# jingsenzhu/i2-sdf

Measured on AMD Instinct MI355X. Metric: ray-samples/sec (fwd+bwd), higher is better.
Workload: dtype f32 (bf16x3 split MFMA: fp32 operands as 3 bf16 terms, fp32 accumulate; the 256x256 weight-gradient GEMM blocks and the sampler's depth-choosing sdf-only passes: 2 bf16 terms per operand, 3 products, fp32 accumulate; the saved SDF tensors abar / G(hbar) / G(a) -- operands of those GEMMs and of the s

## Files before the change

### i2sdf_amd/csrc/pack.hip

```cpp
#include "plan.h"

using namespace i2sdf;

int i2sdf_hip_check(hipError_t e, const char* what);

namespace {

struct RowTab {
  int32_t n;
  int32_t rows[3 * I2SDF_MAX_LAYERS], cols[3 * I2SDF_MAX_LAYERS], scale_off[3 * I2SDF_MAX_LAYERS];
  int64_t off_v[3 * I2SDF_MAX_LAYERS], off_g[3 * I2SDF_MAX_LAYERS];
};

__global__ __launch_bounds__(256) void rowscale_kernel(RowTab tab, const float* __restrict__ params, float* __restrict__ scale,
                                                        int n_rows) {
  const int row = blockIdx.x * 4 + (threadIdx.x >> 6);
  const int lane = threadIdx.x & 63;
  if (row >= n_rows) return;
  int e = 0;
  while (e + 1 < tab.n && row >= tab.scale_off[e + 1]) ++e;
  const int r = row - tab.scale_off[e];
  const int cols = tab.cols[e];
  const float* v = params + tab.off_v[e] + (int64_t)r * cols;
  float s = 0.f;
  for (int c = lane; c < cols; c += 64) { float x = v[c]; s = fmaf(x, x, s); }
#pragma unroll
  for (int o = 32; o > 0; o >>= 1) s += __shfl_xor(s, o);
  if (lane == 0) scale[row] = params[tab.off_g[e] + r] / sqrtf(s);
}

__device__ __forceinline__ int map_col(const ColMap& cm, int kp) {
  if (kp < cm.split) return kp < cm.valid0 ? cm.base0 + kp : -1;
  const int j = kp - cm.split;
  return j < cm.valid1 ? cm.base1 + j : -1;
}

__global__ __launch_bounds__(256) void pack_kernel(const Seg* __restrict__ segs, int n_segs, const float* __restrict__ params,
                                                    const float* __restrict__ scale, float* __restrict__ chunks,
                                                    int64_t total_chunks) {
  const int64_t gid = (int64_t)blockIdx.x * 256 + threadIdx.x;
  const int64_t chunk = gid >> 6;
  const int lane = (int)(gid & 63);
  if (chunk >= total_chunks) return;
  int lo = 0, hi_ = n_segs - 1;
  while (lo < hi_) {
    const int mid = (lo + hi_ + 1) >> 1;
    if (segs[mid].chunk0 <= chunk) lo = mid; else hi_ = mid - 1;
  }
  const Seg s = segs[lo];
  const int c = (int)(chunk - s.chunk0);
  const int i32 = lane & 31, hi = lane >> 5;
  f32x4 out = {0.f, 0.f, 0.f, 0.f};
  if (c < s.used) {
    if (s.type == SEG_BIAS) {
      const int nt = c / 4, q = c % 4;
#pragma unroll
      for (int t = 0; t < 4; ++t) {
        const int r = 32 * nt + 8 * q + 4 * hi + t;
        out[t] = (r < s.nrows) ? params[s.off_bias + s.row_off + r] : 0.f;
      }
    } else if (s.type == SEG_WFWD) {
      const int nt = c / s.KC, kc = c % s.KC;
      const int r = 32 * nt + i32;
      if (r < s.nrows) {
        const int row = s.row_off + r;
        const float sc = scale[s.scale_off + row] * s.mult;
        const float* v = params + s.off_v + (int64_t)row * s.cols;
#pragma unroll
        for (int t = 0; t < 4; ++t) {
          const int col = map_col(s.cm, 8 * kc + 4 * hi + t);
          out[t] = col >= 0 ? v[col] * sc : 0.f;
        }
      }
    } else if (s.type == SEG_WFWD3) {
      const int G = s.NT / 2, w = c >> 1, e = c & 1;
      const int kc = w / (3 * G), g = (w / 3) % G, sp = w % 3;
      const int r = 32 * (2 * g + e) + i32;
      unsigned q[4] = {0u, 0u, 0u, 0u};
      if (r < s.nrows) {
        const int row = s.row_off + r;
        const float sc = scale[s.scale_off + row] * s.mult;
        const float* v = params + s.off_v + (int64_t)row * s.cols;
#pragma unroll
        for (int i = 0; i < 4; ++i) {
          float x[2];
#pragma unroll
          for (int h2 = 0; h2 < 2; ++h2) {
            const int j = 2 * i + h2;
            const int col = map_col(s.cm, 16 * kc + (j & 3) + 8 * (j >> 2) + 4 * hi);
            x[h2] = col >= 0 ? v[col] * sc : 0.f;
          }
          unsigned p0, p1, p2;
          split3_pair(x[0], x[1], p0, p1, p2);
          q[i] = sp == 0 ? p0 : (sp == 1 ? p1 : p2);
        }
      }
      out = __builtin_bit_cast(f32x4, u32x4{q[0], q[1], q[2], q[3]});
    } else if (s.type == SEG_WBWD3) {
      const int G = s.NT / 2, w = c >> 1, e = c & 1;
      const int kc = w / (3 * G), g = (w / 3) % G, sp = w % 3;
      const int col = map_col(s.cm, 32 * (2 * g + e) + i32);
      unsigned q[4] = {0u, 0u, 0u, 0u};
      if (col >= 0) {
#pragma unroll
        for (int i = 0; i < 4; ++i) {
          float x[2];
#pragma unroll
          for (int h2 = 0; h2 < 2; ++h2) {
            const int j = 2 * i + h2;
            const int r = 16 * kc + (j & 3) + 8 * (j >> 2) + 4 * hi;
            x[h2] = 0.f;
            if (r < s.nrows) {
              const int row = s.row_off + r;
              x[h2] = params[s.off_v + (int64_t)row * s.cols + col] * scale[s.scale_off + row] * s.mult;
            }
          }
          unsigned p0, p1, p2;
          split3_pair(x[0], x[1], p0, p1, p2);
          q[i] = sp == 0 ? p0 : (sp == 1 ? p1 : p2);
        }
      }
      out = __builtin_bit_cast(f32x4, u32x4{q[0], q[1], q[2], q[3]});
    } else if (s.type == SEG_BIAS_H) {
      const int kg = lane >> 4;
#pragma unroll
      for (int t = 0; t < 4; ++t) {
        const int r = 16 * c + 4 * kg + t;
        out[t] = (r < s.nrows) ? params[s.off_bias + s.row_off + r] : 0.f;
      }
    } else if (s.type == SEG_WFWD3H || s.type == SEG_WBWD3H || s.type == SEG_WFWD2H) {
      const int G = s.NT / 2, w = c >> 1, e = c & 1, PL = s.type == SEG_WFWD2H ? 2 : 3;
      const int kc = w / (PL * G), g = (w / PL) % G, sp = w % PL;
      const int i16 = lane & 15, kg = lane >> 4;
      const int arow = 16 * (2 * g + e) + i16;
      const bool fwd = s.type != SEG_WBWD3H;
      const int acol = fwd ? -1 : map_col(s.cm, arow);
      unsigned q[4] = {0u, 0u, 0u, 0u};
      if (fwd ? (arow < s.nrows) : (acol >= 0)) {
#pragma unroll
        for (int i = 0; i < 4; ++i) {
          float x[2];
#pragma unroll
          for (int h2 = 0; h2 < 2; ++h2) {
            const int j = 2 * i + h2;
            const int k = 32 * kc + 16 * (j >> 2) + 4 * kg + (j & 3);
            x[h2] = 0.f;
            if (fwd) {
              const int row = s.row_off + arow, col = map_col(s.cm, k);
              if (col >= 0) x[h2] = params[s.off_v + (int64_t)row * s.cols + col] * (scale[s.scale_off + row] * s.mult);
            } else if (k < s.nrows) {
              const int row = s.row_off + k;
              x[h2] = params[s.off_v + (int64_t)row * s.cols + acol] * scale[s.scale_off + row] * s.mult;
            }
          }
          unsigned p0, p1, p2;
          split3_pair(x[0], x[1], p0, p1, p2);
          q[i] = sp == 0 ? p0 : (sp == 1 ? p1 : p2);
        }
      }
      out = __builtin_bit_cast(f32x4, u32x4{q[0], q[1], q[2], q[3]});
    } else if (s.type == SEG_ROWVEC_H) {
      const int rr = c / s.KC, nt = c % s.KC, kg = lane >> 4;
      const int row = s.row_off + rr;
      const float sc = scale[s.scale_off + row] * s.mult;
#pragma unroll
      for (int t = 0; t < 4; ++t) {
        const int col = map_col(s.cm, 16 * nt + 4 * kg + t);
        out[t] = col >= 0 ? params[s.off_v + (int64_t)row * s.cols + col] * sc : 0.f;
      }
    } else if (s.type == SEG_WBWD) {
      const int kt = c / s.KC, nc = c % s.KC;
      const int col = map_col(s.cm, 32 * kt + i32);
      if (col >= 0) {
#pragma unroll
        for (int t = 0; t < 4; ++t) {
          const int r = 8 * nc + 4 * hi + t;
          if (r < s.nrows) {
            const int row = s.row_off + r;
            out[t] = params[s.off_v + (int64_t)row * s.cols + col] * scale[s.scale_off + row] * s.mult;
          }
        }
      }
    } else if (s.type == SEG_ROWVEC) {
      const int rr = c / s.KC, kc = c % s.KC;
      const int row = s.row_off + rr;
      const float sc = scale[s.scale_off + row] * s.mult;
#pragma unroll
      for (int t = 0; t < 4; ++t) {
        const int col = map_col(s.cm, 8 * kc + 4 * hi + t);
        out[t] = col >= 0 ? params[s.off_v + (int64_t)row * s.cols + col] * sc : 0.f;
      }
    } else if (s.type == SEG_SCALAR) {
#pragma unroll
      for (int t = 0; t < 4; ++t) out[t] = (t < s.nrows) ? params[s.off_bias + s.row_off + t] : 0.f;
    }
  }
  reinterpret_cast<f32x4*>(chunks)[chunk * 64 + lane] = out;
}

void fill_tab(RowTab& tab, const NetPlan& np) {
  for (int l = 0; l < np.d.n_lin; ++l) {
    const int e = tab.n++;
    tab.rows[e] = np.d.out_dim[l]; tab.cols[e] = np.d.in_dim[l]; tab.scale_off[e] = np.scale_off[l];
    tab.off_v[e] = np.d.off_v[l]; tab.off_g[e] = np.d.off_g[l];
  }
}

}

extern "C" int i2sdf_pack_weights(const i2sdf_plan* p, const float* params, float* packed, void* stream) {
  if (!p || !params || !packed) return I2SDF_EINVAL;
  if (!p->d_segs) return I2SDF_EHIP;
  hipStream_t st = (hipStream_t)stream;
  RowTab tab{};
  fill_tab(tab, p->sdf); fill_tab(tab, p->rgb);
  if (p->light.d.n_lin) fill_tab(tab, p->light);
  rowscale_kernel<<<cdiv(p->n_scale, 4), 256, 0, st>>>(tab, params, packed, p->n_scale);
  const int64_t threads = p->total_chunks * 64;
  pack_kernel<<<(unsigned)((threads + 255) / 256), 256, 0, st>>>(p->d_segs, p->n_segs, params, packed, packed + p->scale_floats,
                                                                 p->total_chunks);
  return i2sdf_hip_check(hipGetLastError(), "pack_weights launch");
}
```

### i2sdf_amd/csrc/plan.cpp

```cpp
#include <hip/hip_runtime.h>
#include <string.h>
#include <initializer_list>
#include <string>
#include "plan.h"
#include <stdlib.h>

using namespace i2sdf;

static thread_local std::string g_hip_err;

int i2sdf_hip_check(hipError_t e, const char* what) {
  if (e == hipSuccess) return I2SDF_OK;
  g_hip_err = std::string(what) + ": " + hipGetErrorString(e);
  return I2SDF_EHIP;
}

int i2sdf_refuse(const char* why) {
  g_hip_err = why;
  return I2SDF_EINVAL;
}

extern "C" int i2sdf_version(void) { return I2SDF_VERSION; }
extern "C" const char* i2sdf_last_hip_error(void) { return g_hip_err.c_str(); }
extern "C" const char* i2sdf_strerror(int code) {
  switch (code) {
    case I2SDF_OK: return "ok";
    case I2SDF_EINVAL: return "invalid argument or unsupported network shape";
    case I2SDF_EHIP: return "HIP runtime error";
    case I2SDF_ESPHERE: return "ray misses the scene bounding sphere";
    case I2SDF_EWORKSPACE: return "workspace too small";
    case I2SDF_ECOMM: return "RCCL error";
    default: return "unknown error";
  }
}

namespace {

constexpr int32_t HUGE_SPLIT = 1 << 30;
constexpr float RS2 = 0.70710678118654752440f;

struct Builder {
  std::vector<Seg>& segs;
  int64_t chunk;
  void add(Seg s) { s.chunk0 = chunk; chunk += s.nchunks; segs.push_back(s); }
  void pad_to_stage() {
    int64_t r = chunk % SC;
    if (r) { Seg z{}; z.type = SEG_ZERO; z.nchunks = (int32_t)(SC - r); add(z); }
  }
};

Seg base_seg(const NetPlan& np, int l, int type) {
  Seg s{};
  s.type = type;
  s.off_v = np.d.off_v[l]; s.off_bias = np.d.off_bias[l];
  s.scale_off = np.scale_off[l];
  s.rows = np.d.out_dim[l]; s.cols = np.d.in_dim[l];
  s.row_off = 0; s.nrows = s.rows;
  s.mult = 1.0f;
  s.cm = ColMap{HUGE_SPLIT, 0, s.cols, 0, 0};
  return s;
}

int pe_dim(const i2sdf_mlp_desc& d) { return side_dim(d); }
int pe_chunks(const i2sdf_mlp_desc& d) { return side_chunks(d); }

ColMap cols(int n) { return ColMap{HUGE_SPLIT, 0, n, 0, 0}; }

struct Family {
  int32_t bias_type, w_type, rowvec_type;
  int tile_rows;
  int k_width;
  int rv_width;
  int bias_chunks;
  int planes;
  bool fold_skip;
};
constexpr Family FP32{SEG_BIAS, SEG_WFWD, SEG_ROWVEC, 32, 8, 8, 4, 1, false};
constexpr Family X3{SEG_BIAS, SEG_WFWD3, SEG_ROWVEC, 32, 16, 8, 4, 3, true};
constexpr Family X3H{SEG_BIAS_H, SEG_WFWD3H, SEG_ROWVEC_H, 16, 32, 16, 1, 3, true};
constexpr Family X2H{SEG_BIAS_H, SEG_WFWD2H, SEG_ROWVEC_H, 16, 32, 16, 1, 2, true};

void emit_dense(Builder& b, const NetPlan& np, int l, const Family& f, int NT, int KC, ColMap cm, float mult, int row_off, int nrows) {
  Seg sb = base_seg(np, l, f.bias_type);
  sb.NT = NT; sb.KC = f.bias_chunks; sb.nchunks = sb.used = NT * f.bias_chunks; sb.row_off = row_off; sb.nrows = nrows;
  b.add(sb);
  Seg sw = base_seg(np, l, f.w_type);
  sw.NT = NT; sw.KC = KC; sw.used = NT * KC * f.planes; sw.cm = cm; sw.mult = mult; sw.row_off = row_off; sw.nrows = nrows;
  sw.nchunks = (f.w_type == SEG_WFWD ? op_chunks(NT, KC) : f.w_type == SEG_WFWD3 ? x3_op_chunks(NT, KC) : x3h_op_chunks(NT, KC, f.planes)) - sb.nchunks;
  b.add(sw);
}
void emit_dense_bwd(Builder& b, const NetPlan& np, int l, int type, int KT, int KC, ColMap cm, int row_off, int nrows, float mult = 1.0f) {
  Seg sw = base_seg(np, l, type);
  sw.NT = KT; sw.KC = KC; sw.used = KT * KC * (type == SEG_WBWD ? 1 : 3); sw.cm = cm; sw.mult = mult; sw.row_off = row_off; sw.nrows = nrows;
  sw.nchunks = type == SEG_WBWD ? bwd_op_chunks(KT, KC) : type == SEG_WBWD3 ? x3_bwd_chunks(KT, KC) : x3h_bwd_chunks(KT, KC);
  b.add(sw);
}
void emit_rowvec(Builder& b, const NetPlan& np, int l, const Family& f, int nrows) {
  const int KC = np.d.hidden / f.rv_width;
  Seg sw = base_seg(np, l, f.rowvec_type);
  sw.NT = nrows; sw.KC = KC; sw.used = nrows * KC; sw.nchunks = nrows * KC; sw.cm = cols(np.d.hidden); sw.nrows = nrows;
  b.add(sw);
  Seg sc = base_seg(np, l, SEG_SCALAR);
  sc.nchunks = (f.rowvec_type == SEG_ROWVEC ? rowvec_chunks(KC, nrows) : rowvec_h_chunks(KC, nrows)) - nrows * KC; sc.used = 1; sc.nrows = nrows;
  b.add(sc);
}
void emit_sdf_hidden(Builder& b, const NetPlan& np, const Family& f) {
  const i2sdf_mlp_desc& d = np.d;
  const int H = d.hidden, PED = pe_dim(d), PEK = cdiv(PED, f.k_width);
  for (int l = 0; l < d.n_lin - 1; ++l) {
    ColMap cm = cols(d.in_dim[l]);
    int KC = (l == 0) ? PEK : H / f.k_width;
    float mult = 1.0f;
    if (l == d.skip_layer) {
      cm = ColMap{H, 0, d.in_dim[l] - PED, d.in_dim[l] - PED, PED}; KC += PEK;
      if (f.fold_skip) mult = RS2;
    }
    emit_dense(b, np, l, f, H / f.tile_rows, KC, cm, mult, 0, d.out_dim[l]);
  }
}

int check_mlp(const i2sdf_mlp_desc& d) {
  if (d.n_lin < 2 || d.n_lin > I2SDF_MAX_LAYERS) return I2SDF_EINVAL;
  if (d.hidden % 32 || d.hidden < 32 || d.hidden > 256) return I2SDF_EINVAL;
  return I2SDF_OK;
}

void mark_here(NetPlan& np, const Builder& b, std::initializer_list<Mark> ms) {
  for (Mark k : ms) np.mark[k] = b.chunk;
}

int build_sdf(i2sdf_plan* p, Builder& b) {
  NetPlan& np = p->sdf;
  const i2sdf_mlp_desc& d = np.d;
  const int L = d.n_lin, H = d.hidden, PEC = pe_chunks(d), PED = pe_dim(d);
  const int F = d.d_out - 1;
  if (check_mlp(d)) return I2SDF_EINVAL;
  if (d.multires <= 0 || d.d_in != 3 || d.in0 != PED) return I2SDF_EINVAL;
  if (F < 0 || F % 32 || F > 256) return I2SDF_EINVAL;
  if (d.skip_layer == 0 || d.skip_layer >= L - 1) return I2SDF_EINVAL;
  for (int l = 0; l < L - 1; ++l) {
    const int want_out = (l + 1 == d.skip_layer) ? H - PED : H;
    const int want_in = (l == 0) ? PED : H;
    if (d.out_dim[l] != want_out || d.in_dim[l] != want_in) return I2SDF_EINVAL;
  }
  if (d.in_dim[L - 1] != H) return I2SDF_EINVAL;
  p->H = H; p->F = F;
  const bool even_tiles = (H / 32) % 2 == 0, wide = H == 256 && F == 256;
  const int PT = cdiv(PEC * 8, 32);
  mark_here(np, b, {FWD});
  emit_sdf_hidden(b, np, FP32);
  mark_here(np, b, {FWD_HIDDEN_END});
  emit_rowvec(b, np, L - 1, FP32, 1);
  mark_here(np, b, {FWD_SDF_END});
  if (F > 0) emit_dense(b, np, L - 1, FP32, F / 32, H / 8, cols(H), 1.0f, 1, F);
  mark_here(np, b, {FWD_END});
  mark_here(np, b, {REV});
  emit_rowvec(b, np, L - 1, FP32, 1);
  if (F > 0) emit_dense_bwd(b, np, L - 1, SEG_WBWD, H / 32, F / 8, cols(H), 1, F);
  mark_here(np, b, {REV_CHAIN});
  emit_rowvec(b, np, L - 1, FP32, 1);
  for (int l = L - 2; l >= 0; --l) {
    ColMap cm = cols(d.in_dim[l]);
    int KT = (l == 0) ? PT : H / 32;
    if (l == d.skip_layer) { cm = ColMap{H, 0, d.in_dim[l] - PED, d.in_dim[l] - PED, PED}; KT += PT; }
    if (l == 0) mark_here(np, b, {REV_W0});
    emit_dense_bwd(b, np, l, SEG_WBWD, KT, H / 8, cm, 0, d.out_dim[l]);
  }
  mark_here(np, b, {REV_END});
  mark_here(np, b, {FWD3, FWD3_HIDDEN_END, FWD3_END});
  if (even_tiles) {
    emit_sdf_hidden(b, np, X3);
    mark_here(np, b, {FWD3_HIDDEN_END});
    emit_rowvec(b, np, L - 1, X3, 1);
    mark_here(np, b, {FWD3_END});
  }
  mark_here(np, b, {REV3, REV3_CHAIN, REV3_W0, REV3_END});
  if (even_tiles) {
    emit_rowvec(b, np, L - 1, X3, 1);
    if (F > 0 && F % 16 == 0) emit_dense_bwd(b, np, L - 1, SEG_WBWD3, H / 32, F / 16, cols(H), 1, F);
    mark_here(np, b, {REV3_CHAIN});
    emit_rowvec(b, np, L - 1, X3, 1);
    for (int l = L - 2; l >= 0; --l) {
      if (l == 0) mark_here(np, b, {REV3_W0});
      if (l == d.skip_layer) {
        emit_dense_bwd(b, np, l, SEG_WBWD3, H / 32, H / 16, cols(d.in_dim[l] - PED), 0, d.out_dim[l], RS2);
        emit_dense_bwd(b, np, l, SEG_WBWD3, PT, H / 16, ColMap{HUGE_SPLIT, d.in_dim[l] - PED, PED, 0, 0}, 0, d.out_dim[l], RS2);
      } else {
        emit_dense_bwd(b, np, l, SEG_WBWD3, (l == 0) ? PT : H / 32, H / 16, cols(d.in_dim[l]), 0, d.out_dim[l]);
      }
    }
    mark_here(np, b, {REV3_END});
  }
  mark_here(np, b, {FWD3H, FWD3H_SDF_END, FWD3H_END});
  if (wide) {
    emit_sdf_hidden(b, np, X3H);
    emit_rowvec(b, np, L - 1, X3H, 1);
    mark_here(np, b, {FWD3H_SDF_END});
    emit_dense(b, np, L - 1, X3H, F / 16, H / 32, cols(H), 1.0f, 1, F);
    mark_here(np, b, {FWD3H_END});
  }
  mark_here(np, b, {FWD2H, FWD2H_END});
  if (wide) {
    emit_sdf_hidden(b, np, X2H);
    emit_rowvec(b, np, L - 1, X2H, 1);
    mark_here(np, b, {FWD2H_END});
  }
  return I2SDF_OK;
}

int build_rgb(i2sdf_plan* p, Builder& b) {
  NetPlan& np = p->rgb;
  const i2sdf_mlp_desc& d = np.d;
  const bool idr = rgb_idr(d);
  const int L = d.n_lin, H = d.hidden, PED = pe_dim(d), PEC = pe_chunks(d), F = p->F;
  if (check_mlp(d)) return I2SDF_EINVAL;
  if ((rgb_mode(d) != I2SDF_RGB_MODE_NERF && !idr) || (idr && d.d_in != 9)) return I2SDF_EINVAL;
  if (rgb_act(d) > I2SDF_RGB_ACT_SOFTPLUS || (d.reserved & 0xf0ff0000) || rgb_embed(d) > I2SDF_RGB_EMBED_FOURIER) return I2SDF_EINVAL;
  const ColMap rev0 = idr ? ColMap{F, PED, F, PED - 3, 3} : ColMap{HUGE_SPLIT, PED, F, 0, 0};
  if (d.skip_layer >= 0 || d.d_out != 3 || (d.multires <= 0 && !idr) || d.in0 != PED + F || F <= 0) return I2SDF_EINVAL;
  for (int l = 0; l < L - 1; ++l)
    if (d.out_dim[l] != H || d.in_dim[l] != (l == 0 ? PED + F : H)) return I2SDF_EINVAL;
  const bool wide = H == 256 && F == 256 && L >= 3;
  mark_here(np, b, {FWD});
  emit_dense(b, np, 0, FP32, H / 32, PEC + F / 8, ColMap{PEC * 8, 0, PED, PED, F}, 1.0f, 0, H);
  for (int l = 1; l < L - 1; ++l) emit_dense(b, np, l, FP32, H / 32, H / 8, cols(H), 1.0f, 0, H);
  emit_rowvec(b, np, L - 1, FP32, 3);
  mark_here(np, b, {FWD_END, REV});
  emit_rowvec(b, np, L - 1, FP32, 3);
  for (int l = L - 2; l >= 1; --l) emit_dense_bwd(b, np, l, SEG_WBWD, H / 32, H / 8, cols(H), 0, H);
  emit_dense_bwd(b, np, 0, SEG_WBWD, F / 32 + (idr ? 1 : 0), H / 8, rev0, 0, H);
  mark_here(np, b, {REV_END});
  mark_here(np, b, {FWD3H, FWD3H_END, REV3H, REV3H_END});
  if (wide) {
    const int PV32 = cdiv(PEC * 8, 32);
    emit_dense(b, np, 0, X3H, H / 16, PV32 + F / 32, ColMap{PV32 * 32, 0, PED, PED, F}, 1.0f, 0, H);
    for (int l = 1; l < L - 1; ++l) emit_dense(b, np, l, X3H, H / 16, H / 32, cols(H), 1.0f, 0, H);
    emit_rowvec(b, np, L - 1, X3H, 3);
    mark_here(np, b, {FWD3H_END, REV3H});
    emit_rowvec(b, np, L - 1, X3H, 3);
    for (int l = L - 2; l >= 1; --l) emit_dense_bwd(b, np, l, SEG_WBWD3H, H / 16, H / 32, cols(H), 0, H);
    emit_dense_bwd(b, np, 0, SEG_WBWD3H, F / 16 + (idr ? 2 : 0), H / 32, rev0, 0, H);
    mark_here(np, b, {REV3H_END});
  }
  return I2SDF_OK;
}

int build_light(i2sdf_plan* p, Builder& b) {
  NetPlan& np = p->light;
  const i2sdf_mlp_desc& d = np.d;
  if (d.n_lin == 0) return I2SDF_OK;
  const int H = d.hidden, F = p->F;
  if (d.n_lin != 2 || H % 32 || H > 256 || d.d_out != 1 || d.in0 != F || d.multires != 0) return I2SDF_EINVAL;
  if (d.out_dim[0] != H || d.in_dim[0] != F || d.in_dim[1] != H) return I2SDF_EINVAL;
  mark_here(np, b, {FWD});
  emit_dense(b, np, 0, FP32, H / 32, F / 8, cols(F), 1.0f, 0, H);
  emit_rowvec(b, np, 1, FP32, 1);
  mark_here(np, b, {FWD_END, REV});
  emit_rowvec(b, np, 1, FP32, 1);
  mark_here(np, b, {REV_END});
  mark_here(np, b, {FWD3H, FWD3H_END});
  if (H == 128 && F == 256) {
    emit_dense(b, np, 0, X3H, H / 16, F / 32, cols(F), 1.0f, 0, H);
    emit_rowvec(b, np, 1, X3H, 1);
    mark_here(np, b, {FWD3H_END});
  }
  return I2SDF_OK;
}

void assign_scales_and_wgrad(i2sdf_plan* p, NetPlan& np, int kind) {
  const i2sdf_mlp_desc& d = np.d;
  const int side = pe_dim(d), PEC8 = pe_chunks(d) * 8;
  for (int l = 0; l < d.n_lin; ++l) {
    np.scale_off[l] = p->n_scale;
    p->n_scale += d.out_dim[l];
    const bool last = (l == d.n_lin - 1);
    int rowsP = d.hidden, colsP = d.hidden;
    if (kind == 0) {
      if (l == 0) colsP = PEC8;
      else if (l == d.skip_layer) colsP = d.hidden + PEC8;
      if (last) rowsP = 32 + (d.d_out - 1);
    } else if (kind == 1) {
      if (l == 0) colsP = PEC8 + (d.in0 - side);
      if (last) rowsP = 32;
    } else {
      if (l == 0) colsP = d.in0;
      if (last) rowsP = 32;
    }
    np.wg_rows[l] = rowsP; np.wg_cols[l] = colsP;
    np.wgrad_off[l] = p->wgrad_floats;
    p->wgrad_floats += (int64_t)rowsP * colsP + rowsP;
  }
}

}

extern "C" int i2sdf_plan_create(const i2sdf_net_desc* desc, i2sdf_plan** out) {
  if (!desc || !out) return I2SDF_EINVAL;
  {
    if (rgb_act(desc->rgb) > I2SDF_RGB_ACT_SOFTPLUS || (desc->rgb.reserved & 0x00ff0000)) {
      g_hip_err = "i2sdf_plan_create: rgb.reserved " + std::to_string(desc->rgb.reserved) + ": output activation " + std::to_string(rgb_act(desc->rgb)) +
                  " of the radiance net is not one of I2SDF_RGB_ACT_SIGMOID (0), I2SDF_RGB_ACT_RELU (1), I2SDF_RGB_ACT_SOFTPLUS (2) in bits 8..15"
                  " (bits 16..23 must be zero)";
      return I2SDF_EINVAL;
    }
    const int emb = rgb_embed(desc->rgb), n_emb = desc->rgb.multires;
    if (emb > I2SDF_RGB_EMBED_FOURIER || (desc->rgb.reserved & 0xf0000000)) {
      g_hip_err = "i2sdf_plan_create: rgb.reserved " + std::to_string(desc->rgb.reserved) + ": view embedder " + std::to_string(emb) +
                  " of the radiance net is not one of I2SDF_RGB_EMBED_POSITIONAL (0), I2SDF_RGB_EMBED_SH (1), I2SDF_RGB_EMBED_FOURIER (2) in bits 24..27"
                  " (bits 28..31 must be zero)";
      return I2SDF_EINVAL;
    }
    if (emb == I2SDF_RGB_EMBED_SH && (n_emb < 1 || n_emb > 5)) {
      g_hip_err = "i2sdf_plan_create: spherical-harmonics view embedder of degree " + std::to_string(n_emb) +
                  " (rgb.multires): the reference's SHEncoder and the kernels have degrees 1..5";
      return I2SDF_EINVAL;
    }
    if (emb == I2SDF_RGB_EMBED_FOURIER && (n_emb < 1 || n_emb > I2SDF_RGB_EMBED_MAX_CHANNELS)) {
      g_hip_err = "i2sdf_plan_create: Fourier view embedder with " + std::to_string(n_emb) + " channels (rgb.multires): 1..12 fit the 27 view "
                  "columns of the radiance net's side row (width 2 c + 3); more need wider rows";
      return I2SDF_EINVAL;
    }
    const int H = desc->sdf.hidden, Hr = desc->rgb.hidden;
    int F = 0;
    if (desc->rgb.n_lin > 0) {
      if (emb != I2SDF_RGB_EMBED_POSITIONAL) {
        F = desc->sdf.d_out - 1;
        if (desc->rgb.in0 != side_dim(desc->rgb) + F) {
          g_hip_err = "i2sdf_plan_create: rgb.in0 " + std::to_string(desc->rgb.in0) + " disagrees with the view embedder: " +
                      (emb == I2SDF_RGB_EMBED_SH ? "spherical harmonics of degree " : "Fourier features with channels ") + std::to_string(n_emb) +
                      " are " + std::to_string(embed_dim(desc->rgb)) + " wide, the side row " + std::to_string(side_dim(desc->rgb)) +
                      ", so lin0 has " + std::to_string(side_dim(desc->rgb) + F) + " columns with feature size " + std::to_string(F);
          return I2SDF_EINVAL;
        }
      } else {
        F = desc->rgb.in0 - (rgb_idr(desc->rgb) ? side_dim(desc->rgb) : (desc->rgb.multires > 0 ? 3 + 6 * desc->rgb.multires : 3));
      }
    }
    const bool ok = (H == 256 && Hr == 256 && F == 256) || (H == 64 && Hr == 64 && F == 64);
    if (!ok || desc->sdf.multires != 6 || (emb == I2SDF_RGB_EMBED_POSITIONAL && desc->rgb.multires != 4 && desc->rgb.multires != 0)) {
      g_hip_err = "i2sdf_plan_create: SDF width " + std::to_string(H) + " / radiance width " + std::to_string(Hr) + " / feature size " + std::to_string(F) +
                  " / multires " + std::to_string(desc->sdf.multires) + "," + std::to_string(desc->rgb.multires) +
                  ": the MLP kernels are instantiated for 256/256/256 and 64/64/64 with multires 6 (points) and 4 (view directions) only";
      return I2SDF_EINVAL;
    }
    if (rgb_idr(desc->rgb) && desc->rgb.d_in != 9) {
      g_hip_err = "i2sdf_plan_create: the radiance net's 'idr' mode needs d_in 9 (points, view directions, normals)";
      return I2SDF_EINVAL;
    }
  }
  i2sdf_plan* p = new i2sdf_plan();
  p->desc = *desc;
  p->sdf.d = desc->sdf; p->rgb.d = desc->rgb; p->light.d = desc->light;
  assign_scales_and_wgrad(p, p->sdf, 0);
  assign_scales_and_wgrad(p, p->rgb, 1);
  if (desc->light.n_lin) assign_scales_and_wgrad(p, p->light, 2);
  p->scale_floats = round_up(p->n_scale, CHUNK_FLOATS);
  Builder b{p->segs, 0};
  int rc = build_sdf(p, b);
  if (!rc) rc = build_rgb(p, b);
  if (!rc) rc = build_light(p, b);
  if (rc) { delete p; return rc; }
  { Seg z{}; z.type = SEG_ZERO; z.nchunks = SC > SCH ? SC : SCH; b.add(z); }
  p->total_chunks = b.chunk;
  p->n_segs = (int32_t)p->segs.size();
  hipError_t e = hipMalloc((void**)&p->d_segs, sizeof(Seg) * p->segs.size());
  if (e == hipSuccess) e = hipMemcpy(p->d_segs, p->segs.data(), sizeof(Seg) * p->segs.size(), hipMemcpyHostToDevice);
  if (e != hipSuccess) {
    (void)i2sdf_hip_check(e, "plan table upload");
    if (p->d_segs) (void)hipFree(p->d_segs);
    p->d_segs = nullptr;
    (void)hipGetLastError();
  }
  {
    int dev = 0, n = 0;
    if (hipGetDevice(&dev) == hipSuccess && hipDeviceGetAttribute(&n, hipDeviceAttributeMultiprocessorCount, dev) == hipSuccess && n > 0) p->n_cu = n;
    else (void)hipGetLastError();
  }
  if (p->H == 256 && p->F == 256)
    for (int32_t opt : {I2SDF_OPT_SDF_FWD_BF16X3, I2SDF_OPT_WGRAD_BF16X3, I2SDF_OPT_TRAIN_FWD_BF16X3, I2SDF_OPT_SDF_BWD_BF16X3, I2SDF_OPT_RGB_BF16X3,
                        I2SDF_OPT_BLOCKED_SAVES, I2SDF_OPT_TAIL_OVERLAP})
      (void)i2sdf_plan_set_option(p, opt, 1);
  *out = p;
  return I2SDF_OK;
}

extern "C" void i2sdf_plan_destroy(i2sdf_plan* p) {
  if (!p) return;
  if (p->d_segs) (void)hipFree(p->d_segs);
  if (p->ev_fork) (void)hipEventDestroy(p->ev_fork);
  if (p->ev_join) (void)hipEventDestroy(p->ev_join);
  if (p->side) (void)hipStreamDestroy(p->side);
  for (hipEvent_t e : p->part_ev) if (e) (void)hipEventDestroy(e);
  for (hipStream_t s : p->part_st) if (s) (void)hipStreamDestroy(s);
  delete p;
}

hipStream_t i2sdf_tail_fork(const i2sdf_plan* p, hipStream_t st) {
  if (!p->tail_overlap) return st;
  if (!p->side) {
    if (hipStreamCreateWithFlags(&p->side, hipStreamNonBlocking) != hipSuccess) { p->side = nullptr; (void)hipGetLastError(); return st; }
    if (hipEventCreateWithFlags(&p->ev_fork, hipEventDisableTiming) != hipSuccess ||
        hipEventCreateWithFlags(&p->ev_join, hipEventDisableTiming) != hipSuccess) {
      (void)hipGetLastError();
      (void)hipStreamDestroy(p->side); p->side = nullptr;
      return st;
    }
  }
  if (hipEventRecord(p->ev_fork, st) != hipSuccess || hipStreamWaitEvent(p->side, p->ev_fork, 0) != hipSuccess) {
    (void)hipGetLastError();
    return st;
  }
  return p->side;
}

void i2sdf_tail_join(const i2sdf_plan* p, hipStream_t st, hipStream_t side) {
  if (side == st) return;
  (void)hipEventRecord(p->ev_join, side);
  (void)hipStreamWaitEvent(st, p->ev_join, 0);
}

namespace {
constexpr int64_t PART_ALIGN = I2SDF_WG_CH;

bool parts_resources(const i2sdf_plan* p) {
  for (int q = 0; q < I2SDF_MAX_PARTS; ++q)
    if (!p->part_ev[q] && hipEventCreateWithFlags(&p->part_ev[q], hipEventDisableTiming) != hipSuccess) { (void)hipGetLastError(); return false; }
  for (int q = 0; q + 1 < p->parts; ++q)
    if (!p->part_st[q] && hipStreamCreateWithFlags(&p->part_st[q], hipStreamNonBlocking) != hipSuccess) { (void)hipGetLastError(); return false; }
  return true;
}
void part_bounds(int64_t M, int n, int64_t (&b)[I2SDF_MAX_PARTS + 1]) {
  static double w[I2SDF_MAX_PARTS] = {0, 0, 0, 0};
  static int nw = -1;
  if (nw < 0) {
    nw = 0;
    if (const char* e = getenv("I2SDF_PART_WEIGHTS")) {
      while (*e && nw < I2SDF_MAX_PARTS) {
        char* end = nullptr;
        const double v = strtod(e, &end);
        if (end == e) break;
        w[nw++] = v > 0 ? v : 0;
        e = (*end == ',') ? end + 1 : end;
      }
    }
  }
  const int64_t nch = (M + PART_ALIGN - 1) / PART_ALIGN;
  double tot = 0, acc = 0;
  for (int q = 0; q < n; ++q) tot += (nw == n) ? w[q] : 1.0;
  b[0] = 0;
  for (int q = 1; q <= n; ++q) {
    acc += (nw == n) ? w[q - 1] : 1.0;
    int64_t c = tot > 0 ? (int64_t)(nch * (acc / tot) + 0.5) : nch * q / n;
    if (c < b[q - 1] / PART_ALIGN) c = b[q - 1] / PART_ALIGN;
    b[q] = (c > nch ? nch : c) * PART_ALIGN;
  }
  b[n] = nch * PART_ALIGN;
}
}

void i2sdf_parts_fence(const i2sdf_plan* p, hipStream_t st) {
  (void)hipEventRecord(p->part_ev[0], st);
  for (int q = 0; q + 1 < p->parts; ++q) (void)hipStreamWaitEvent(p->part_st[q], p->part_ev[0], 0);
}
void i2sdf_parts_join_all(const i2sdf_plan* p, hipStream_t st) {
  for (int q = 0; q + 1 < p->parts; ++q) {
    if (!p->part_st[q] || !p->part_ev[q + 1]) continue;
    (void)hipEventRecord(p->part_ev[q + 1], p->part_st[q]);
    (void)hipStreamWaitEvent(st, p->part_ev[q + 1], 0);
  }
}
bool i2sdf_parts_begin(const i2sdf_plan* p, hipStream_t st, int64_t M, PartRun* pr) {
  pr->n = 1; pr->st[0] = st; pr->lo[0] = 0; pr->hi[0] = M; pr->own = false;
  if (!i2sdf_parts_on(p) || M <= 0) return false;
  const bool chain = p->chain_active != 0;
  const int64_t Mref = chain ? (p->chain_M > M ? p->chain_M : M) : M;
  if ((Mref + PART_ALIGN - 1) / PART_ALIGN < p->parts) return false;
  if (!parts_resources(p)) return false;
  int64_t b[I2SDF_MAX_PARTS + 1];
  part_bounds(Mref, p->parts, b);
  pr->n = p->parts;
  for (int q = 0; q < pr->n; ++q) {
    pr->st[q] = q == 0 ? st : p->part_st[q - 1];
    pr->lo[q] = b[q] < M ? b[q] : M;
    pr->hi[q] = b[q + 1] < M ? b[q + 1] : M;
  }
  if (!chain) { i2sdf_parts_fence(p, st); pr->own = true; }
  return true;
}
void i2sdf_parts_end(const i2sdf_plan* p, hipStream_t st, PartRun* pr) {
  if (pr->own) i2sdf_parts_join_all(p, st);
  pr->own = false;
}

extern "C" int i2sdf_chain_begin(const i2sdf_plan* p, int64_t M, void* stream) {
  if (!p || M < 0) return I2SDF_EINVAL;
  if (!i2sdf_parts_on(p) || M == 0) return I2SDF_OK;
  if (p->chain_active) return I2SDF_EINVAL;
  if (!parts_resources(p)) return i2sdf_hip_check(hipErrorOutOfMemory, "chain_begin: streams / events");
  i2sdf_parts_fence(p, (hipStream_t)stream);
  p->chain_active = 1;
  p->chain_M = M;
  return i2sdf_hip_check(hipGetLastError(), "chain_begin");
}
extern "C" int i2sdf_chain_fence(const i2sdf_plan* p, void* stream) {
  if (!p) return I2SDF_EINVAL;
  if (!p->chain_active) return I2SDF_OK;
  i2sdf_parts_fence(p, (hipStream_t)stream);
  return i2sdf_hip_check(hipGetLastError(), "chain_fence");
}
extern "C" int i2sdf_chain_end(const i2sdf_plan* p, void* stream) {
  if (!p) return I2SDF_EINVAL;
  if (!p->chain_active) return I2SDF_OK;
  i2sdf_parts_join_all(p, (hipStream_t)stream);
  p->chain_active = 0;
  p->chain_M = 0;
  return i2sdf_hip_check(hipGetLastError(), "chain_end");
}

extern "C" int i2sdf_plan_set_option(i2sdf_plan* p, int32_t option, int32_t value) {
  if (!p) return I2SDF_EINVAL;
  if (option == I2SDF_OPT_PARTS) {
    if (value < 0 || value > I2SDF_MAX_PARTS || p->chain_active) return I2SDF_EINVAL;
    p->parts = value >= 2 ? value : 0;
    return I2SDF_OK;
  }
  if (option == I2SDF_OPT_SDF_FWD_BF16X3) {
    const bool runs = (p->H == 256 && p->F == 256 && span_chunks(p->sdf, SPAN_FWD3H) > 0) || (p->H == 64 && p->F == 64 && span_chunks(p->sdf, SPAN_FWD3) > 0);
    if (value && !runs) return I2SDF_EINVAL;
    p->sdf_fwd_bf16x3 = value ? 1 : 0;
    return I2SDF_OK;
  }
  if (option == I2SDF_OPT_SAMPLER_BF16X2) {
    if (value && (span_chunks(p->sdf, SPAN_FWD2H) == 0 || p->H != 256 || p->F != 256)) return I2SDF_EINVAL;
    p->sampler_bf16x2 = value ? 1 : 0;
    return I2SDF_OK;
  }
  if (option == I2SDF_OPT_TRAIN_FWD_BF16X3) {
    if (value && (span_chunks(p->sdf, SPAN_REV3_CHAIN) == 0 || span_chunks(p->sdf, SPAN_FWD3H) == 0 || p->H != 256 || p->F != 256)) return I2SDF_EINVAL;
    p->train_fwd_bf16x3 = value ? 1 : 0;
    return I2SDF_OK;
  }
  if (option == I2SDF_OPT_SDF_BWD_BF16X3) {
    if (value && (span_chunks(p->sdf, SPAN_REV3_CHAIN) == 0 || p->H != 256 || p->F != 256)) return I2SDF_EINVAL;
    p->sdf_bwd_bf16x3 = value ? 1 : 0;
    return I2SDF_OK;
  }
  if (option == I2SDF_OPT_RGB_BF16X3) {
    if (value && (span_chunks(p->rgb, SPAN_REV3H) == 0 || p->rgb.d.hidden != 256 || p->F != 256 || p->rgb.d.n_lin < 3)) return I2SDF_EINVAL;
    p->rgb_bf16x3 = value ? 1 : 0;
    return I2SDF_OK;
  }
  if (option == I2SDF_OPT_WGRAD_BF16X3) {
    p->wgrad_bf16x3 = value ? 1 : 0;
    return I2SDF_OK;
  }
  if (option == I2SDF_OPT_WGRAD_BF16X2) {
    p->wgrad_bf16x2 = value ? 1 : 0;
    return I2SDF_OK;
  }
  if (option == I2SDF_OPT_BLOCKED_SAVES) {
    p->blocked_saves = value ? 1 : 0;
    return I2SDF_OK;
  }
  if (option == I2SDF_OPT_SAVES24) {
    if (value && (p->H != 256 || p->F != 256 || span_chunks(p->sdf, SPAN_REV3_CHAIN) == 0)) return I2SDF_EINVAL;
    if (p->chain_active) return I2SDF_EINVAL;
    p->saves24 = value ? 1 : 0;
    return I2SDF_OK;
  }
  if (option == I2SDF_OPT_TAIL_OVERLAP) {
    p->tail_overlap = value ? 1 : 0;
    return I2SDF_OK;
  }
  return I2SDF_EINVAL;
}

extern "C" int i2sdf_plan_set_view_embed(i2sdf_plan* p, const float* B_host, int32_t rows, int32_t cols) {
  if (!p) return I2SDF_EINVAL;
  const auto refuse = [](const std::string& why) { g_hip_err = "i2sdf_plan_set_view_embed: " + why; return I2SDF_EINVAL; };
  if (rgb_embed(p->rgb.d) != I2SDF_RGB_EMBED_FOURIER) return refuse("the plan's radiance net has no Fourier view embedder (rgb.reserved bits 24..27)");
  if (!B_host) return refuse("B_host is NULL");
  if (rows != 3 || cols != p->rgb.d.multires)
    return refuse("B is (" + std::to_string(rows) + ", " + std::to_string(cols) + "), the plan's embedder takes (3, " + std::to_string(p->rgb.d.multires) + ")");
  for (int i = 0; i < 3 * cols; ++i)
    if (!(B_host[i] - B_host[i] == 0.0f)) return refuse("B[" + std::to_string(i / cols) + "][" + std::to_string(i % cols) + "] is not finite");
  for (int r = 0; r < 3; ++r)
    for (int c = 0; c < I2SDF_RGB_EMBED_MAX_CHANNELS; ++c) p->view_B[r * I2SDF_RGB_EMBED_MAX_CHANNELS + c] = c < cols ? B_host[r * cols + c] : 0.0f;
  p->view_B_set = 1;
  return I2SDF_OK;
}

extern "C" int i2sdf_plan_set_exchange(i2sdf_plan* p, const i2sdf_exchange* ex, int32_t flags) {
  if (!p || (flags & ~I2SDF_DP_GLOBAL_SAMPLER) || (ex && !ex->allreduce)) return I2SDF_EINVAL;
  p->exchange = ex ? *ex : i2sdf_exchange{nullptr, nullptr};
  p->dp_flags = ex ? flags : 0;
  return I2SDF_OK;
}

extern "C" int64_t i2sdf_plan_pack_floats(const i2sdf_plan* p) {
  return p ? p->scale_floats + p->total_chunks * CHUNK_FLOATS : 0;
}
extern "C" int64_t i2sdf_plan_wgrad_floats(const i2sdf_plan* p) { return p ? p->wgrad_floats : 0; }
```

### i2sdf_amd/csrc/plan.h

```cpp
#pragma once
#include <stdint.h>
#include <vector>
#include "../../include/i2sdf.h"
#include "x3h.h"

namespace i2sdf {

enum SegType : int32_t { SEG_ZERO = 0, SEG_BIAS = 1, SEG_WFWD = 2, SEG_WBWD = 3, SEG_ROWVEC = 4, SEG_SCALAR = 5,
                         SEG_WFWD3 = 6 ,
                         SEG_WBWD3 = 7 ,
                         SEG_BIAS_H = 8, SEG_WFWD3H = 9, SEG_WBWD3H = 10, SEG_ROWVEC_H = 11,
                         SEG_WFWD2H = 12  };

struct ColMap { int32_t split, base0, valid0, base1, valid1; };

struct Seg {
  int64_t chunk0;
  int32_t nchunks;
  int32_t type;
  int64_t off_v, off_bias;
  int32_t scale_off;
  int32_t rows, cols;
  int32_t row_off;
  int32_t nrows;
  int32_t NT, KC;
  int32_t used;
  ColMap cm;
  float mult;
};

enum Mark : int {
  FWD, FWD_HIDDEN_END, FWD_SDF_END, FWD_END,
  REV, REV_CHAIN, REV_W0, REV_END,
  FWD3, FWD3_HIDDEN_END, FWD3_END,
  REV3, REV3_CHAIN, REV3_W0, REV3_END,
  FWD3H, FWD3H_SDF_END, FWD3H_END,
  REV3H, REV3H_END,
  FWD2H, FWD2H_END,
  N_MARKS
};
struct SpanId { Mark from, to; int stage_chunks; };
constexpr SpanId SPAN_FWD_HIDDEN{FWD, FWD_HIDDEN_END, SC};
constexpr SpanId SPAN_FWD_SDF{FWD, FWD_SDF_END, SC};
constexpr SpanId SPAN_FWD{FWD, FWD_END, SC};
constexpr SpanId SPAN_REV_SWEEP2{REV, REV_W0, SC};
constexpr SpanId SPAN_REV_CHAIN{REV_CHAIN, REV_END, SC};
constexpr SpanId SPAN_REV{REV, REV_END, SC};
constexpr SpanId SPAN_FWD3_HIDDEN{FWD3, FWD3_HIDDEN_END, SC};
constexpr SpanId SPAN_FWD3{FWD3, FWD3_END, SC};
constexpr SpanId SPAN_REV3_SWEEP2{REV3, REV3_W0, SC};
constexpr SpanId SPAN_REV3_CHAIN{REV3_CHAIN, REV3_END, SC};
constexpr SpanId SPAN_FWD3H_SDF{FWD3H, FWD3H_SDF_END, SCH};
constexpr SpanId SPAN_FWD3H{FWD3H, FWD3H_END, SCH};
constexpr SpanId SPAN_REV3H{REV3H, REV3H_END, SCH};
constexpr SpanId SPAN_FWD2H{FWD2H, FWD2H_END, SCH};

inline int rgb_mode(const i2sdf_mlp_desc& d) { return d.reserved & 0xff; }
inline int rgb_act(const i2sdf_mlp_desc& d) { return (d.reserved >> 8) & 0xff; }
inline int rgb_embed(const i2sdf_mlp_desc& d) { return (d.reserved >> 24) & 0xf; }
inline bool rgb_idr(const i2sdf_mlp_desc& d) { return rgb_mode(d) == I2SDF_RGB_MODE_IDR; }
inline int embed_dim(const i2sdf_mlp_desc& d) { return rgb_embed(d) == I2SDF_RGB_EMBED_SH ? d.multires * d.multires : 2 * d.multires + 3; }
inline int side_dim(const i2sdf_mlp_desc& d) {
  if (rgb_embed(d) != I2SDF_RGB_EMBED_POSITIONAL) return embed_dim(d) + (rgb_idr(d) ? 6 : 0);
  const int raw = rgb_idr(d) ? 3 : d.d_in;
  return (d.multires > 0 ? raw + 2 * raw * d.multires : raw) + (rgb_idr(d) ? 6 : 0);
}
inline int side_chunks(const i2sdf_mlp_desc& d) {
  if (rgb_embed(d) != I2SDF_RGB_EMBED_POSITIONAL) return rgb_idr(d) ? 5 : 4;
  return (side_dim(d) + 7) / 8;
}

struct NetPlan {
  i2sdf_mlp_desc d;
  int32_t scale_off[I2SDF_MAX_LAYERS];
  int64_t mark[N_MARKS] = {};
  int64_t wgrad_off[I2SDF_MAX_LAYERS];
  int32_t wg_rows[I2SDF_MAX_LAYERS], wg_cols[I2SDF_MAX_LAYERS];
};

}

struct i2sdf_plan {
  i2sdf_net_desc desc;
  i2sdf::NetPlan sdf, rgb, light;
  std::vector<i2sdf::Seg> segs;
  i2sdf::Seg* d_segs = nullptr;
  int32_t n_segs = 0;
  int32_t n_scale = 0;
  int64_t scale_floats = 0;
  int64_t total_chunks = 0;
  int64_t wgrad_floats = 0;
  int32_t H = 0, F = 0;
  int32_t n_cu = 256;
  int32_t rgb_bf16x3 = 0;
  int32_t sdf_bwd_bf16x3 = 0;
  int32_t train_fwd_bf16x3 = 0;
  int32_t wgrad_bf16x3 = 0;
  int32_t sdf_fwd_bf16x3 = 0;
  int32_t sampler_bf16x2 = 0;
  i2sdf_exchange exchange{nullptr, nullptr};
  int32_t dp_flags = 0;
  int32_t wgrad_bf16x2 = 0;
  int32_t blocked_saves = 0;
  int32_t saves24 = 0;
  int32_t tail_overlap = 0;
  mutable hipStream_t side = nullptr;
  mutable hipEvent_t ev_fork = nullptr, ev_join = nullptr;
  int32_t parts = 0;
  mutable hipStream_t part_st[I2SDF_MAX_PARTS - 1] = {nullptr, nullptr, nullptr};
  mutable hipEvent_t part_ev[I2SDF_MAX_PARTS] = {nullptr, nullptr, nullptr, nullptr};
  mutable int32_t chain_active = 0;
  float view_B[3 * I2SDF_RGB_EMBED_MAX_CHANNELS] = {};
  int32_t view_B_set = 0;
  mutable int64_t chain_M = 0;
};

int i2sdf_refuse(const char* why);
int i2sdf_hip_check(hipError_t e, const char* what);

namespace i2sdf {
struct Span { const float* w = nullptr; int n_stages = 0; };
inline int64_t span_chunks(const NetPlan& np, SpanId id) { return np.mark[id.to] - np.mark[id.from]; }
inline Span span(const i2sdf_plan* p, const float* packed, const NetPlan& np, SpanId id) {
  const int64_t n = span_chunks(np, id);
  if (n <= 0 || n % id.stage_chunks) return Span{};
  return Span{packed + p->scale_floats + np.mark[id.from] * CHUNK_FLOATS, (int)(n / id.stage_chunks)};
}
}

struct PartRun {
  int n = 1;
  hipStream_t st[I2SDF_MAX_PARTS];
  int64_t lo[I2SDF_MAX_PARTS], hi[I2SDF_MAX_PARTS];
  bool own = false;
};
bool i2sdf_parts_begin(const i2sdf_plan* p, hipStream_t st, int64_t M, PartRun* pr);
void i2sdf_parts_end(const i2sdf_plan* p, hipStream_t st, PartRun* pr);
void i2sdf_parts_join_all(const i2sdf_plan* p, hipStream_t st);
void i2sdf_parts_fence(const i2sdf_plan* p, hipStream_t st);
#ifndef I2SDF_WG_CH
#define I2SDF_WG_CH 2048
#endif
inline bool i2sdf_parts_on(const i2sdf_plan* p) { return p->parts >= 2; }
struct ChainGuard {
  const i2sdf_plan* p; hipStream_t st; bool on;
  ChainGuard(const i2sdf_plan* p_, hipStream_t st_, bool ranged) : p(p_), st(st_), on(!ranged && p_->chain_active != 0) {
    if (on) i2sdf_parts_join_all(p, st);
  }
  ~ChainGuard() { if (on) i2sdf_parts_fence(p, st); }
};

hipStream_t i2sdf_tail_fork(const i2sdf_plan* p, hipStream_t st);
void i2sdf_tail_join(const i2sdf_plan* p, hipStream_t st, hipStream_t side);

inline int64_t split_bulk_points(int64_t M, int n_cu) {
  const int64_t n_wg = (M + i2sdf::PTS_PER_WG - 1) / i2sdf::PTS_PER_WG;
  const int64_t full = (n_wg / n_cu) * n_cu, rem = n_wg - full;
  if (full == 0 || rem == 0 || rem * 4 > n_cu) return 0;
  if ((full * i2sdf::PTS_PER_WG) % I2SDF_WG_CH != 0) return 0;
  return full * i2sdf::PTS_PER_WG;
}

enum TailOrder { TAIL_FORKED, TAIL_BEHIND };
template <class Full, class Tail>
inline void i2sdf_dispatch_points(const i2sdf_plan* p, hipStream_t st, int64_t M, bool ranged, bool may_split, TailOrder order, Full full, Tail tail) {
  constexpr int64_t WG = i2sdf::PTS_PER_WG;
  if (ranged) {
    PartRun pr;
    i2sdf_parts_begin(p, st, M, &pr);
    for (int q = 0; q < pr.n; ++q)
      if (pr.hi[q] > pr.lo[q]) full(pr.st[q], (int)(pr.lo[q] / WG), (unsigned)((pr.hi[q] - pr.lo[q] + WG - 1) / WG), M);
    i2sdf_parts_end(p, st, &pr);
    return;
  }
  const int64_t bulk = may_split ? split_bulk_points(M, p->n_cu) : 0;
  if (bulk == 0) {
    full(st, 0, (unsigned)((M + WG - 1) / WG), M);
  } else if (order == TAIL_FORKED) {
    hipStream_t ts = i2sdf_tail_fork(p, st);
    tail(ts, bulk);
    full(st, 0, (unsigned)(bulk / WG), bulk);
    i2sdf_tail_join(p, st, ts);
  } else {
    full(st, 0, (unsigned)(bulk / WG), bulk);
    tail(st, bulk);
  }
}
```

### i2sdf_amd/csrc/sampler.hip

```cpp
#include "mlp_args.h"

using namespace i2sdf;

namespace {

constexpr int NMAX = 640;
constexpr int NNEW = 128;
constexpr int EMAX = NMAX / 64;

enum { ST_DONE = 0, ST_ITERS = 1, ST_FLAG0 = 2 , ST_CNT0 = 16 , ST_WORDS = 32 };

#ifndef SAMPLER_DPP
#define SAMPLER_DPP 1
#endif
template <int CTRL, int ROW_MASK>
__device__ __forceinline__ float dpp_mov(float old, float v) {
  return __builtin_bit_cast(float, __builtin_amdgcn_update_dpp(__builtin_bit_cast(int, old), __builtin_bit_cast(int, v), CTRL, ROW_MASK, 0xf, false));
}
constexpr int DPP_ROW_SHR1 = 0x111, DPP_ROW_SHR2 = 0x112, DPP_ROW_SHR4 = 0x114, DPP_ROW_SHR8 = 0x118, DPP_ROW_BCAST15 = 0x142, DPP_ROW_BCAST31 = 0x143;
__device__ __forceinline__ float wscan_incl(float v, int lane) {
#if SAMPLER_DPP
  (void)lane;
  v += dpp_mov<DPP_ROW_SHR1, 0xf>(0.f, v);
  v += dpp_mov<DPP_ROW_SHR2, 0xf>(0.f, v);
  v += dpp_mov<DPP_ROW_SHR4, 0xf>(0.f, v);
  v += dpp_mov<DPP_ROW_SHR8, 0xf>(0.f, v);
  v += dpp_mov<DPP_ROW_BCAST15, 0xa>(0.f, v);
  v += dpp_mov<DPP_ROW_BCAST31, 0xc>(0.f, v);
  return v;
#else
#pragma unroll
  for (int o = 1; o < 64; o <<= 1) {
    const float t = __shfl_up(v, o);
    if (lane >= o) v += t;
  }
  return v;
#endif
}
__device__ __forceinline__ float wsum(float v) {
#if SAMPLER_DPP
  return __builtin_bit_cast(float, __builtin_amdgcn_readlane(__builtin_bit_cast(int, wscan_incl(v, 0)), 63));
#else
#pragma unroll
  for (int o = 32; o > 0; o >>= 1) v += __shfl_xor(v, o);
  return v;
#endif
}
__device__ __forceinline__ float wmax(float v) {
#if SAMPLER_DPP
  const float lo = -3.4028234663852886e38f;
  v = fmaxf(v, dpp_mov<DPP_ROW_SHR1, 0xf>(lo, v));
  v = fmaxf(v, dpp_mov<DPP_ROW_SHR2, 0xf>(lo, v));
  v = fmaxf(v, dpp_mov<DPP_ROW_SHR4, 0xf>(lo, v));
  v = fmaxf(v, dpp_mov<DPP_ROW_SHR8, 0xf>(lo, v));
  v = fmaxf(v, dpp_mov<DPP_ROW_BCAST15, 0xa>(lo, v));
  v = fmaxf(v, dpp_mov<DPP_ROW_BCAST31, 0xc>(lo, v));
  return __builtin_bit_cast(float, __builtin_amdgcn_readlane(__builtin_bit_cast(int, v), 63));
#else
#pragma unroll
  for (int o = 32; o > 0; o >>= 1) v = fmaxf(v, __shfl_xor(v, o));
  return v;
#endif
}
template <int E>
__device__ __forceinline__ void row_scan_incl(float (&v)[E], int lane) {
#pragma unroll
  for (int e = 1; e < E; ++e) v[e] += v[e - 1];
  const float tot = v[E - 1];
  const float pre = wscan_incl(tot, lane) - tot;
#pragma unroll
  for (int e = 0; e < E; ++e) v[e] += pre;
}

__device__ __forceinline__ float laplace_density(float s, float inv_beta) {
  const float e = expm1f(-fabsf(s) * inv_beta);
  const float sg = (s > 0.f) ? 1.f : ((s < 0.f) ? -1.f : 0.f);
  return inv_beta * (0.5f + 0.5f * sg * e);
}

template <int E>
struct Row {
  float z[E], s[E];
  float a[E], ds[E];
  int n;
};

template <int E>
__device__ __forceinline__ void row_intervals(Row<E>& r, int lane) {
  const float zn_next = __shfl_down(r.z[0], 1), sn_next = __shfl_down(r.s[0], 1);
#pragma unroll
  for (int e = 0; e < E; ++e) {
    const int j = lane * E + e;
    const float z1 = (e + 1 < E) ? r.z[(e + 1 < E) ? e + 1 : e] : zn_next;
    const float s1 = (e + 1 < E) ? r.s[(e + 1 < E) ? e + 1 : e] : sn_next;
    float a = 0.f, d = 0.f;
    if (j < r.n - 1) {
      a = z1 - r.z[e];
      const float b = fabsf(r.s[e]), c = fabsf(s1);
      const bool first = a * a + b * b <= c * c;
      const bool second = a * a + c * c <= b * b;
      const float sp = (a + b + c) / 2.0f;
      const float area = sp * (sp - a) * (sp - b) * (sp - c);
      const bool mask = !first && !second && (b + c - a > 0.f);
      float h = (2.0f * sqrtf(area)) / a;
      if (!(h == h)) h = 0.f;
      else if (h > 3.4028234663852886e38f) h = 3.4028234663852886e38f;
      else if (h < -3.4028234663852886e38f) h = -3.4028234663852886e38f;
      d = ((first && !second) ? b : 0.f) + (second ? c : 0.f) + (mask ? h : 0.f);
      const float sg0 = (r.s[e] > 0.f) ? 1.f : ((r.s[e] < 0.f) ? -1.f : 0.f);
      const float sg1 = (s1 > 0.f) ? 1.f : ((s1 < 0.f) ? -1.f : 0.f);
      if (!(sg0 * sg1 == 1.f)) d = 0.f;
    }
    r.a[e] = a; r.ds[e] = d;
  }
}

template <int E>
__device__ __forceinline__ float row_error_bound(const Row<E>& r, float beta, int lane) {
  const float ib = 1.0f / beta;
  float fe[E], er[E];
#pragma unroll
  for (int e = 0; e < E; ++e) {
    const int j = lane * E + e;
    const bool ok = j < r.n - 1;
    fe[e] = ok ? r.a[e] * laplace_density(r.s[e], ib) : 0.f;
    er[e] = ok ? expf(-r.ds[e] / beta) * (r.a[e] * r.a[e]) / (4.0f * beta * beta) : 0.f;
  }
  float fi[E], ei[E];
#pragma unroll
  for (int e = 0; e < E; ++e) { fi[e] = fe[e]; ei[e] = er[e]; }
  row_scan_incl<E>(fi, lane);
  row_scan_incl<E>(ei, lane);
  float mx = -3.4e38f;
#pragma unroll
  for (int e = 0; e < E; ++e) {
    const int j = lane * E + e;
    if (j < r.n - 1) {
      const float integ = fi[e] - fe[e];
      const float bo = (fminf(expf(ei[e]), 1.0e6f) - 1.0f) * expf(-integ);
      mx = fmaxf(mx, bo);
    }
  }
  return wmax(mx);
}

struct SamplerArgs {
  int64_t B;
  int it, n, n_new;
  int N_eval, N_final, max_iters, beta_iters, force_iters;
  float eps, add_tiny, near, far;
  const float* beta_param; float beta_min;
  int* state;
  float* z_cur; float* z_nxt;
  float* sdf_prev; float* sdf_cur;
  const int* idx;
  int* idx_nxt;
  const float* sdf_new;
  float* samples;
  float* beta;
  const float* u_more; const float* u_final; int64_t ldu_final;
};

template <int E>
__device__ __forceinline__ void load_row(Row<E>& r, const float* z, const float* s, int n, int lane) {
  r.n = n;
#pragma unroll
  for (int e = 0; e < E; ++e) {
    const int j = lane * E + e;
    r.z[e] = (j < n) ? z[j] : 3.0e38f;
    r.s[e] = (j < n) ? s[j] : 0.f;
  }
}

template <int E>
__device__ __forceinline__ float beta_step(const SamplerArgs& a, Row<E>& r, int64_t rc, bool active, int lane) {
  const float beta0 = fabsf(a.beta_param[0]) + a.beta_min;
  const int n = a.n;
  float* sc = a.sdf_cur + rc * NMAX;
  const float* zc = a.z_cur + rc * NMAX;
  r.n = n;
  {
    const int n_old = n - a.n_new;
    const int* ix = a.idx + rc * NMAX;
    const float* sp = a.sdf_prev + rc * NMAX;
    const float* sn = a.sdf_new + rc * a.n_new;
#pragma unroll
    for (int e = 0; e < E; ++e) {
      const int j = lane * E + e;
      float sv = 0.f, zv = 3.0e38f;
      if (j < n) {
        zv = zc[j];
        if (a.it == 0) sv = sn[j];
        else { const int k = ix[j]; sv = (k < n_old) ? sp[k] : sn[k - n_old]; }
        if (active) sc[j] = sv;
      }
      r.z[e] = zv; r.s[e] = sv;
    }
  }
  row_intervals<E>(r, lane);
  float beta = a.beta[rc];
  const float err0 = row_error_bound<E>(r, beta0, lane);
  if (err0 <= a.eps) beta = beta0;
  float bmin = beta0, bmax = beta;
  for (int k = 0; k < a.beta_iters; ++k) {
    const float bmid = (bmin + bmax) / 2.0f;
    const float err = row_error_bound<E>(r, bmid, lane);
    if (err <= a.eps) bmax = bmid; else bmin = bmid;
  }
  return bmax;
}
template <int E>
__global__ __launch_bounds__(256) void sampler_beta_kernel(SamplerArgs a) {
  if (a.state[ST_DONE]) return;
  const int lane = threadIdx.x & 63;
  const int64_t ray = (int64_t)blockIdx.x * 4 + (threadIdx.x >> 6);
  if (ray >= a.B) return;
  Row<E> r;
  const float beta = beta_step<E>(a, r, ray, true, lane);
  if (lane == 0) {
    a.beta[ray] = beta;
    if (beta > fabsf(a.beta_param[0]) + a.beta_min) atomicOr(&a.state[ST_FLAG0 + a.it], 1);
  }
}

template <int E>
__device__ __forceinline__ void resample_step(const SamplerArgs& a, const Row<E>& r, float beta, bool more, int64_t ray, int64_t rc, bool active,
                                              float (&s_cdf)[4][NMAX + 1], float (&s_z)[4][NMAX], float (&s_new)[4][NNEW], int lane, int wv) {
  const int n = a.n;
  const float ib = 1.0f / beta;
  float fe[E], cum[E];
#pragma unroll
  for (int e = 0; e < E; ++e) {
    const int j = lane * E + e;
    const float dist = (j < n - 1) ? r.a[e] : 1.0e10f;
    fe[e] = (j < n) ? dist * laplace_density(r.s[e], ib) : 0.f;
    cum[e] = (j < n - 1) ? fe[e] : 0.f;
  }
  row_scan_incl<E>(cum, lane);
  float pdf[E];
  if (more) {
    float er[E];
#pragma unroll
    for (int e = 0; e < E; ++e) {
      const int j = lane * E + e;
      er[e] = (j < n - 1) ? expf(-r.ds[e] / beta) * (r.a[e] * r.a[e]) / (4.0f * beta * beta) : 0.f;
    }
    row_scan_incl<E>(er, lane);
#pragma unroll
    for (int e = 0; e < E; ++e) {
      const int j = lane * E + e;
      const float T = expf(-(cum[e] - ((j < n - 1) ? fe[e] : 0.f)));
      pdf[e] = (j < n - 1) ? (fminf(expf(er[e]), 1.0e6f) - 1.0f) * T + a.add_tiny : 0.f;
    }
  } else {
#pragma unroll
    for (int e = 0; e < E; ++e) {
      const int j = lane * E + e;
      const float T = expf(-(cum[e] - ((j < n - 1) ? fe[e] : 0.f)));
      const float w = (1.0f - expf(-fe[e])) * T;
      pdf[e] = (j < n - 1) ? w + 1e-5f : 0.f;
    }
  }
  float tot = 0.f;
#pragma unroll
  for (int e = 0; e < E; ++e) tot += pdf[e];
  tot = wsum(tot);
  float cd[E];
#pragma unroll
  for (int e = 0; e < E; ++e) { pdf[e] = pdf[e] / tot; cd[e] = pdf[e]; }
  row_scan_incl<E>(cd, lane);
#pragma unroll
  for (int e = 0; e < E; ++e) {
    const int j = lane * E + e;
    if (j < n) { s_cdf[wv][j] = cd[e] - pdf[e]; s_z[wv][j] = r.z[e]; }
  }
  __syncthreads();
  const int N = more ? a.N_eval : a.N_final;
  for (int k = lane; k < N; k += 64) {
    float u;
    if (more) u = a.u_more[k];
    else u = a.u_final[rc * a.ldu_final + k];
    int lo = 0, hi = n;
    while (lo < hi) {
      const int mid = (lo + hi) >> 1;
      if (s_cdf[wv][mid] <= u) lo = mid + 1; else hi = mid;
    }
    const int below = (lo - 1 > 0) ? lo - 1 : 0;
    const int above = (lo < n - 1) ? lo : n - 1;
    const float c0 = s_cdf[wv][below], c1 = s_cdf[wv][above];
    const float b0 = s_z[wv][below], b1 = s_z[wv][above];
    float denom = c1 - c0;
    if (denom < 1e-5f) denom = 1.0f;
    const float t = (u - c0) / denom;
    const float smp = b0 + t * (b1 - b0);
    s_new[wv][k] = smp;
    if (active) a.samples[ray * NNEW + k] = smp;
  }
  __syncthreads();
  if (!more) return;
  if (active) {
    float* zn = a.z_nxt + ray * NMAX;
    int* ixn = a.idx_nxt + ray * NMAX;
    for (int j = lane; j < n; j += 64) {
      const float v = s_z[wv][j];
      int lo = 0, hi = N;
      while (lo < hi) { const int mid = (lo + hi) >> 1; if (s_new[wv][mid] < v) lo = mid + 1; else hi = mid; }
      zn[j + lo] = v; ixn[j + lo] = j;
    }
    for (int k = lane; k < N; k += 64) {
      const float v = s_new[wv][k];
      int lo = 0, hi = n;
      while (lo < hi) { const int mid = (lo + hi) >> 1; if (s_z[wv][mid] <= v) lo = mid + 1; else hi = mid; }
      zn[k + lo] = v; ixn[k + lo] = n + k;
    }
  }
}

__device__ __forceinline__ void iteration_done(const SamplerArgs& a, bool more) {
  __syncthreads();
  if (threadIdx.x == 0) {
    __threadfence();
    const int c = atomicAdd(&a.state[ST_CNT0 + a.it], 1);
    if (c == (int)gridDim.x - 1 && !more) { a.state[ST_ITERS] = a.it + 1; __threadfence(); a.state[ST_DONE] = 1; }
  }
}

template <int E>
__global__ __launch_bounds__(256) void sampler_resample_kernel(SamplerArgs a) {
  __shared__ float s_cdf[4][NMAX + 1];
  __shared__ float s_z[4][NMAX];
  __shared__ float s_new[4][NNEW];
  if (a.state[ST_DONE]) return;
  const int lane = threadIdx.x & 63, wv = threadIdx.x >> 6;
  const int64_t ray = (int64_t)blockIdx.x * 4 + wv;
  const bool active = ray < a.B;
  const int64_t rc = active ? ray : a.B - 1;
  bool not_conv = a.state[ST_FLAG0 + a.it] != 0;
  if (a.force_iters > 0) not_conv = (a.it + 1) < a.force_iters;
  const bool more = not_conv && (a.it + 1 < a.max_iters);
  Row<E> r;
  load_row<E>(r, a.z_cur + rc * NMAX, a.sdf_cur + rc * NMAX, a.n, lane);
  row_intervals<E>(r, lane);
  resample_step<E>(a, r, a.beta[rc], more, ray, rc, active, s_cdf, s_z, s_new, lane, wv);
  iteration_done(a, more);
}

template <int E>
__global__ __launch_bounds__(256) void sampler_iter_fixed_kernel(SamplerArgs a) {
  __shared__ float s_cdf[4][NMAX + 1];
  __shared__ float s_z[4][NMAX];
  __shared__ float s_new[4][NNEW];
  const int lane = threadIdx.x & 63, wv = threadIdx.x >> 6;
  const int64_t ray = (int64_t)blockIdx.x * 4 + wv;
  const bool active = ray < a.B;
  const int64_t rc = active ? ray : a.B - 1;
  const bool more = ((a.it + 1) < a.force_iters) && (a.it + 1 < a.max_iters);
  Row<E> r;
  const float beta = beta_step<E>(a, r, rc, active, lane);
  if (active && lane == 0) a.beta[ray] = beta;
  resample_step<E>(a, r, beta, more, ray, rc, active, s_cdf, s_z, s_new, lane, wv);
  iteration_done(a, more);
}

__global__ __launch_bounds__(256) void sampler_init_kernel(int64_t B, int N, const float* __restrict__ t_lin, const float* __restrict__ strat_u,
                                                            float near, float far, float eps, float* __restrict__ z_cur,
                                                            float* __restrict__ samples, float* __restrict__ beta, int* __restrict__ state) {
  const int lane = threadIdx.x & 63;
  const int64_t ray = (int64_t)blockIdx.x * 4 + (threadIdx.x >> 6);
  if (blockIdx.x == 0 && threadIdx.x < ST_WORDS) state[threadIdx.x] = 0;
  if (ray >= B) return;
  float acc = 0.f, carry = 0.f;
  for (int base = 0; base < N; base += 64) {
    const int j = base + lane;
    float z = 0.f;
    if (j < N) {
      const float t = t_lin[j];
      z = near * (1.0f - t) + far * t;
      if (strat_u) {
        const float tm = t_lin[j > 0 ? j - 1 : 0], tp = t_lin[j < N - 1 ? j + 1 : N - 1];
        const float zm = near * (1.0f - tm) + far * tm, zq = near * (1.0f - tp) + far * tp;
        const float lower = (j > 0) ? 0.5f * (z + zm) : z;
        const float upper = (j < N - 1) ? 0.5f * (zq + z) : z;
        z = lower + (upper - lower) * strat_u[ray * N + j];
      }
      z_cur[ray * NMAX + j] = z;
      samples[ray * NNEW + j] = z;
    }
    float zp = __shfl_up(z, 1);
    if (lane == 0) zp = carry;
    if (j < N && j > 0) { const float d = z - zp; acc = fmaf(d, d, acc); }
    carry = __shfl(z, 63);
  }
  acc = wsum(acc);
  if (lane == 0) beta[ray] = sqrtf((1.0f / (4.0f * logf(eps + 1.0f))) * acc);
}

__global__ __launch_bounds__(256) void sampler_final_kernel(int64_t B, const int* __restrict__ state, int N_eval, const float* z_a,
                                                             const float* z_b, const float* __restrict__ samples, int N_final, int N_extra,
                                                             const int* __restrict__ extra_idx, const int* __restrict__ extra_tab,
                                                             float near, float far, const int* __restrict__ eik_idx, float* __restrict__ z_out,
                                                             int64_t ldz, float* __restrict__ z_eik, int* __restrict__ iters_out) {
  __shared__ float buf[4][256];
  const int lane = threadIdx.x & 63, wv = threadIdx.x >> 6;
  const int64_t ray = (int64_t)blockIdx.x * 4 + wv;
  const bool active = ray < B;
  const int64_t rc = active ? ray : B - 1;
  const int iters = state[ST_ITERS];
  if (iters_out != nullptr && blockIdx.x == 0 && threadIdx.x == 0) iters_out[0] = iters;
  const int n_row = N_eval * iters;
  const float* zr = ((iters & 1) ? z_a : z_b) + rc * NMAX;
  const int total = N_final + 2 + N_extra;
  for (int k = lane; k < 256; k += 64) {
    float v = 3.0e38f;
    if (k < N_final) v = samples[rc * NNEW + k];
    else if (k == N_final) v = near;
    else if (k == N_final + 1) v = far;
    else if (k < total) {
      const int e = k - N_final - 2;
      int id;
      if (extra_idx) id = extra_idx[(iters - 1) * N_extra + e];
      else id = extra_tab[(iters - 1) * N_extra + e];
      id = id < 0 ? 0 : (id > n_row - 1 ? n_row - 1 : id);
      v = zr[id];
    }
    buf[wv][k] = v;
  }
  __syncthreads();
  for (int k = 2; k <= 256; k <<= 1) {
    for (int j = k >> 1; j > 0; j >>= 1) {
      for (int i = lane; i < 256; i += 64) {
        const int l = i ^ j;
        if (l > i) {
          const float x = buf[wv][i], y = buf[wv][l];
          const bool up = (i & k) == 0;
          if ((x > y) == up) { buf[wv][i] = y; buf[wv][l] = x; }
        }
      }
      __syncthreads();
    }
  }
  if (active) {
    for (int k = lane; k < total; k += 64) z_out[ray * ldz + k] = buf[wv][k];
    if (lane == 0 && z_eik) {
      int id = eik_idx ? eik_idx[ray] : 0;
      id = id < 0 ? 0 : (id > total - 1 ? total - 1 : id);
      z_eik[ray] = buf[wv][id];
    }
  }
}

template <int E>
__global__ __launch_bounds__(256) void error_bound_kernel(int64_t B, int n, const float* __restrict__ z, const float* __restrict__ sdf,
                                                           const float* __restrict__ beta, int64_t ldbeta, const float* __restrict__ d_star_in,
                                                           float* __restrict__ d_star_out, float* __restrict__ bound) {
  const int lane = threadIdx.x & 63;
  const int64_t ray = (int64_t)blockIdx.x * 4 + (threadIdx.x >> 6);
  if (ray >= B) return;
  Row<E> r;
  load_row<E>(r, z + ray * n, sdf + ray * n, n, lane);
  row_intervals<E>(r, lane);
#pragma unroll
  for (int e = 0; e < E; ++e) {
    const int j = lane * E + e;
    if (j < n - 1) {
      if (d_star_in) r.ds[e] = d_star_in[ray * (n - 1) + j];
      if (d_star_out) d_star_out[ray * (n - 1) + j] = r.ds[e];
    }
  }
  if (bound) {
    const float eb = row_error_bound<E>(r, beta[ray * ldbeta], lane);
    if (lane == 0) bound[ray] = eb;
  }
}

template <int E>
int launch_iter(const SamplerArgs& a, hipStream_t st, const i2sdf_exchange* ex) {
  const unsigned grid = (unsigned)((a.B + 3) / 4);
  if (a.force_iters > 0 && !ex) {
    sampler_iter_fixed_kernel<E><<<grid, 256, 0, st>>>(a);
    return I2SDF_OK;
  }
  sampler_beta_kernel<E><<<grid, 256, 0, st>>>(a);
  if (ex) {
    const int rc = ex->allreduce(ex->ctx, a.state + ST_FLAG0 + a.it, 1, I2SDF_XCHG_I32, I2SDF_XCHG_MAX, (void*)st);
    if (rc) return rc;
  }
  sampler_resample_kernel<E><<<grid, 256, 0, st>>>(a);
  return I2SDF_OK;
}

}

extern "C" int64_t i2sdf_sampler_workspace_floats(int64_t B) {
  return B * (int64_t)(NMAX * 6 + NNEW * 2 + 1) + ST_WORDS + 64;
}

extern "C" int i2sdf_error_bound(const float* z, const float* sdf, int64_t B, int32_t n, const float* beta, int64_t ldbeta,
                                 const float* d_star_in, float* d_star_out, float* bound, void* stream) {
  if (B == 0) return I2SDF_OK;
  if (!z || !sdf || B < 0 || n < 2 || n > NMAX || (bound && !beta) || (!bound && !d_star_out) || (ldbeta != 0 && ldbeta != 1)) return I2SDF_EINVAL;
  hipStream_t st = (hipStream_t)stream;
  const unsigned grid = (unsigned)((B + 3) / 4);
#define I2SDF_EB(E_) error_bound_kernel<E_><<<grid, 256, 0, st>>>(B, n, z, sdf, beta, ldbeta, d_star_in, d_star_out, bound)
  switch (cdiv(n, 64)) {
    case 1: I2SDF_EB(1); break;
    case 2: I2SDF_EB(2); break;
    case 3: I2SDF_EB(3); break;
    case 4: I2SDF_EB(4); break;
    case 5: I2SDF_EB(5); break;
    case 6: I2SDF_EB(6); break;
    case 7: I2SDF_EB(7); break;
    case 8: I2SDF_EB(8); break;
    case 9: I2SDF_EB(9); break;
    default: I2SDF_EB(10); break;
  }
#undef I2SDF_EB
  return i2sdf_hip_check(hipGetLastError(), "error_bound launch");
}


extern "C" int i2sdf_sample_rays(const i2sdf_plan* p, const float* packed, const float* params, const i2sdf_sampler_cfg* sc,
                                 const float* cam, const float* dirs, int64_t B, int32_t training, const float* t_lin, const float* u_more,
                                 const float* u_final, int64_t ldu_final, const int32_t* extra_tab, const float* strat_u,
                                 const int32_t* extra_idx, const int32_t* eik_idx, int32_t force_iters, float* workspace, float* z_out,
                                 int64_t ldz, float* z_eik, int32_t* iters_out, void* stream) {
  if (B == 0) return I2SDF_OK;
  if (!p || !packed || !params || !sc || !cam || !dirs || !t_lin || !u_more || !u_final || !workspace || !z_out || B < 0) return I2SDF_EINVAL;
  if (sc->N_samples_eval > NNEW || sc->N_samples > NNEW || sc->N_samples_eval * sc->max_total_iters > NMAX || sc->max_total_iters > 12)
    return I2SDF_EINVAL;
  if (sc->N_samples + 2 + sc->N_samples_extra > 256 || ldz < sc->N_samples + 2 + sc->N_samples_extra) return I2SDF_EINVAL;
  if (training && (!strat_u || (sc->N_samples_extra > 0 && !extra_idx))) return I2SDF_EINVAL;
  if (!training && sc->N_samples_extra > 0 && !extra_tab) return I2SDF_EINVAL;
  hipStream_t st = (hipStream_t)stream;
  float* w = workspace;
  float* zA = w; w += B * NMAX;
  float* zB = w; w += B * NMAX;
  float* sA = w; w += B * NMAX;
  float* sB = w; w += B * NMAX;
  int* iA = (int*)w; w += B * NMAX;
  int* iB = (int*)w; w += B * NMAX;
  float* samples = w; w += B * NNEW;
  float* sdf_new = w; w += B * NNEW;
  float* beta = w; w += B;
  int* state = (int*)w;
  const float near = sc->near, far = 2.0f * p->desc.scene_bounding_sphere;
  const unsigned grid = (unsigned)((B + 3) / 4);
  const i2sdf_exchange* gcomm = (training && p->exchange.allreduce && (p->dp_flags & I2SDF_DP_GLOBAL_SAMPLER) && force_iters <= 0) ? &p->exchange : nullptr;
  sampler_init_kernel<<<grid, 256, 0, st>>>(B, sc->N_samples_eval, t_lin, training ? strat_u : nullptr, near, far, sc->eps, zA, samples, beta, state);
  const int n_it = (force_iters > 0 && force_iters < sc->max_total_iters) ? force_iters : sc->max_total_iters;
  for (int it = 0; it < n_it; ++it) {
    const int n_new = sc->N_samples_eval;
    int rc = i2sdf_sdf_forward_rays_flagged(p, packed, cam, dirs, samples, NNEW, n_new, B, sdf_new, state + ST_DONE, true, stream);
    if (rc) return rc;
    SamplerArgs a{};
    a.B = B; a.it = it; a.n = sc->N_samples_eval * (it + 1); a.n_new = n_new;
    a.N_eval = sc->N_samples_eval; a.N_final = sc->N_samples; a.max_iters = sc->max_total_iters; a.beta_iters = sc->beta_iters;
    a.force_iters = force_iters;
    a.eps = sc->eps; a.add_tiny = sc->add_tiny; a.near = near; a.far = far;
    a.beta_param = params + p->desc.off_beta; a.beta_min = p->desc.beta_min;
    a.state = state;
    const bool even = (it & 1) == 0;
    a.z_cur = even ? zA : zB; a.z_nxt = even ? zB : zA;
    a.sdf_cur = even ? sA : sB; a.sdf_prev = even ? sB : sA;
    a.idx = even ? iB : iA; a.idx_nxt = even ? iA : iB;
    a.sdf_new = sdf_new; a.samples = samples; a.beta = beta;
    a.u_more = u_more; a.u_final = u_final; a.ldu_final = ldu_final;
    const int E = cdiv(a.n, 64);
    int xrc = I2SDF_OK;
    switch (E) {
      case 1: xrc = launch_iter<1>(a, st, gcomm); break;
      case 2: xrc = launch_iter<2>(a, st, gcomm); break;
      case 3: xrc = launch_iter<3>(a, st, gcomm); break;
      case 4: xrc = launch_iter<4>(a, st, gcomm); break;
      case 5: xrc = launch_iter<5>(a, st, gcomm); break;
      case 6: xrc = launch_iter<6>(a, st, gcomm); break;
      case 7: xrc = launch_iter<7>(a, st, gcomm); break;
      case 8: xrc = launch_iter<8>(a, st, gcomm); break;
      case 9: xrc = launch_iter<9>(a, st, gcomm); break;
      default: xrc = launch_iter<10>(a, st, gcomm); break;
    }
    if (xrc) return xrc;
  }
  sampler_final_kernel<<<grid, 256, 0, st>>>(B, state, sc->N_samples_eval, zA, zB, samples, sc->N_samples, sc->N_samples_extra,
                                             training ? (const int*)extra_idx : nullptr, (const int*)extra_tab, near, far, (const int*)eik_idx, z_out, ldz,
                                             z_eik, iters_out);
  return i2sdf_hip_check(hipGetLastError(), "sample_rays launch");
}
```

### i2sdf_amd/engine.py

```python
from __future__ import annotations

import ctypes as C
from typing import Optional

import os

import torch

from . import lib as L
from .config import NetConfig
from .params import ParamLayout


class RenderEngine:
    def __init__(self, cfg: NetConfig, device="cuda"):
        self.cfg = cfg
        self.layout = ParamLayout(cfg)
        self.device = torch.device(device)
        self._lib = L.load()
        self._desc = self.layout.net_desc()
        plan = C.c_void_p()
        L.check(self._lib.i2sdf_plan_create(C.byref(self._desc), C.byref(plan)), "i2sdf_plan_create")
        self._plan = plan
        self.pack_floats = int(self._lib.i2sdf_plan_pack_floats(plan))
        self.wgrad_floats = int(self._lib.i2sdf_plan_wgrad_floats(plan))
        self.packed = torch.zeros(self.pack_floats, dtype=torch.float32, device=self.device)
        self._pack_stream, self._pack_event, self._pack_readers = None, None, {}
        self.F = cfg.feature_size
        wide = cfg.sdf.hidden == 256 and cfg.feature_size == 256
        self.set_sdf_forward_bf16x3(bool(cfg.bf16x3 and cfg.sdf.hidden % 64 == 0))
        self.set_wgrad_bf16x3(bool(cfg.bf16x3))
        self.set_train_forward_bf16x3(bool(cfg.bf16x3 and wide))
        self.set_sdf_backward_bf16x3(bool(cfg.bf16x3 and wide))
        self.set_rgb_bf16x3(bool(cfg.bf16x3 and cfg.rgb.hidden == 256 and cfg.feature_size == 256 and cfg.rgb.n_lin >= 3))
        self.wgrad_bf16x2 = False
        x2 = os.environ.get("I2SDF_WGRAD_BF16X2", "")
        self.set_wgrad_bf16x2(bool(cfg.bf16x3 and ((x2 != "0") if x2 != "" else cfg.wgrad_bf16x2)))
        self.sampler_bf16x2 = False
        sx2 = os.environ.get("I2SDF_SAMPLER_BF16X2", "")
        if wide:
            self.set_sampler_bf16x2(bool(self.sdf_forward_bf16x3 and ((sx2 != "0") if sx2 != "" else getattr(cfg, "sampler_bf16x2", False))))
        self.set_blocked_saves(bool(cfg.bf16x3 and os.environ.get("I2SDF_BLOCKED_SAVES", "1") != "0"))
        self.saves24 = False
        s24 = os.environ.get("I2SDF_SAVES24", "")
        if wide:
            self.set_saves24(bool(cfg.bf16x3 and ((s24 != "0") if s24 != "" else getattr(cfg, "saves24", True))))
        self.set_tail_overlap(os.environ.get("I2SDF_TAIL_OVERLAP", "1") != "0")
        self.parts = 0
        n_parts = int(os.environ.get("I2SDF_PARTS", "2"))
        self._parts_wanted = n_parts if (cfg.bf16x3 and n_parts >= 2) else 0
        self._sync_parts()
        sc = cfg.sampler
        self._scfg = L.SamplerCfg(near=sc.near, eps=sc.eps, add_tiny=sc.add_tiny, N_samples=sc.N_samples, N_samples_eval=sc.N_samples_eval,
                                  N_samples_extra=sc.N_samples_extra, beta_iters=sc.beta_iters, max_total_iters=sc.max_total_iters)
        dev = self.device
        self.t_lin = torch.linspace(0.0, 1.0, steps=sc.N_samples_eval, device=dev)
        self.u_more = torch.linspace(0.0, 1.0, steps=sc.N_samples_eval, device=dev)
        self.u_final = torch.linspace(0.0, 1.0, steps=sc.N_samples, device=dev)
        if sc.N_samples_extra > 0:
            self.extra_tab = torch.stack([torch.linspace(0, sc.N_samples_eval * (it + 1) - 1, sc.N_samples_extra).long()
                                          for it in range(sc.max_total_iters)]).to(torch.int32).to(dev).contiguous()
        else:
            self.extra_tab = None
        self.n_z = sc.N_samples + sc.N_samples_extra + 2

    def start_timing(self):
        self._timing = []
        eng = self

        class _Timed:
            def __init__(self, fn, name):
                self.fn, self.name = fn, name

            def __call__(self, *a):
                e0, e1 = torch.cuda.Event(enable_timing=True), torch.cuda.Event(enable_timing=True)
                e0.record()
                rc = self.fn(*a)
                e1.record()
                eng._timing.append((self.name, e0, e1))
                return rc

        self._timed_lib = type("TimedLib", (), {})()
        for name in L.SIGNATURES:
            fn = getattr(self._lib, name)
            if name in ("i2sdf_sdf_forward", "i2sdf_sdf_forward_grad", "i2sdf_rgb_forward", "i2sdf_rgb_backward", "i2sdf_rgb_forward_idr", "i2sdf_rgb_backward_idr",
                        "i2sdf_sdf_backward",
                        "i2sdf_weight_grads", "i2sdf_sample_rays", "i2sdf_composite_forward", "i2sdf_composite_backward", "i2sdf_pack_weights",
                        "i2sdf_ray_setup", "i2sdf_light_forward", "i2sdf_light_backward"):
                fn = _Timed(fn, name)
            setattr(self._timed_lib, name, fn)
        self._real_lib, self._lib = self._lib, self._timed_lib

    def stop_timing(self):
        self._lib = self._real_lib
        out = {}
        for name, e0, e1 in self._timing:
            tot, cnt = out.get(name, (0.0, 0))
            out[name] = (tot + e0.elapsed_time(e1), cnt + 1)
        self._timing = []
        return out

    def __del__(self):
        try:
            if getattr(self, "_plan", None):
                self._lib.i2sdf_plan_destroy(self._plan)
                self._plan = None
        except Exception:
            pass

    def pack(self, flat_params: torch.Tensor):
        assert flat_params.is_cuda and flat_params.dtype == torch.float32 and flat_params.numel() == self.layout.n_params
        if os.environ.get("I2SDF_PACK_ASYNC", "1") == "0":
            L.check(self._lib.i2sdf_pack_weights(self._plan, L.ptr(flat_params), L.ptr(self.packed), L.stream_ptr()), "i2sdf_pack_weights")
            return
        dev = flat_params.device
        side = self._pack_stream
        if side is None:
            side = self._pack_stream = torch.cuda.Stream(device=dev)
        cur = torch.cuda.current_stream(dev)
        side.wait_stream(cur)
        for st in getattr(self, "_pack_readers", {}):
            if st != cur:
                side.wait_stream(st)
        with torch.cuda.stream(side):
            L.check(self._lib.i2sdf_pack_weights(self._plan, L.ptr(flat_params), L.ptr(self.packed), L.stream_ptr()), "i2sdf_pack_weights")
            self._pack_event = side.record_event()
        flat_params.record_stream(side)
        self._pack_readers = {}

    def _pk(self):
        ev = self._pack_event
        if ev is not None:
            cur = torch.cuda.current_stream(self.packed.device)
            readers = self.__dict__.setdefault("_pack_readers", {})
            if cur not in readers:
                cur.wait_event(ev)
                readers[cur] = True
        return L.ptr(self.packed)

    def set_sdf_forward_bf16x3(self, on: bool):
        L.check(self._lib.i2sdf_plan_set_option(self._plan, L.OPT_SDF_FWD_BF16X3, int(bool(on))), "i2sdf_plan_set_option")
        self.sdf_forward_bf16x3 = bool(on)

    def set_train_forward_bf16x3(self, on: bool):
        L.check(self._lib.i2sdf_plan_set_option(self._plan, L.OPT_TRAIN_FWD_BF16X3, int(bool(on))), "i2sdf_plan_set_option")
        self.train_forward_bf16x3 = bool(on)
        if hasattr(self, "_parts_wanted"):
            self._sync_parts()

    def set_sdf_backward_bf16x3(self, on: bool):
        L.check(self._lib.i2sdf_plan_set_option(self._plan, L.OPT_SDF_BWD_BF16X3, int(bool(on))), "i2sdf_plan_set_option")
        self.sdf_backward_bf16x3 = bool(on)
        if hasattr(self, "_parts_wanted"):
            self._sync_parts()

    def set_rgb_bf16x3(self, on: bool):
        L.check(self._lib.i2sdf_plan_set_option(self._plan, L.OPT_RGB_BF16X3, int(bool(on))), "i2sdf_plan_set_option")
        self.rgb_bf16x3 = bool(on)
        if hasattr(self, "_parts_wanted"):
            self._sync_parts()

    def set_wgrad_bf16x2(self, on: bool):
        L.check(self._lib.i2sdf_plan_set_option(self._plan, L.OPT_WGRAD_BF16X2, int(bool(on))), "i2sdf_plan_set_option")
        self.wgrad_bf16x2 = bool(on)

    def set_sampler_bf16x2(self, on: bool):
        rc = self._lib.i2sdf_plan_set_option(self._plan, L.OPT_SAMPLER_BF16X2, int(bool(on)))
        if on or rc == 0:
            L.check(rc, "i2sdf_plan_set_option")
        self.sampler_bf16x2 = bool(on) and rc == 0

    def set_blocked_saves(self, on: bool):
        L.check(self._lib.i2sdf_plan_set_option(self._plan, L.OPT_BLOCKED_SAVES, int(bool(on))), "i2sdf_plan_set_option")
        self.blocked_saves = bool(on)

    def set_saves24(self, on: bool):
        rc = self._lib.i2sdf_plan_set_option(self._plan, L.OPT_SAVES24, int(bool(on)))
        if on or rc == 0:
            L.check(rc, "i2sdf_plan_set_option")
        self.saves24 = bool(on) and rc == 0

    def blocked_points(self, which: int, M: int, Mp: int, has_feat: bool = True) -> int:
        return int(self._lib.i2sdf_blocked_points(self._plan, which, M, Mp, int(has_feat)))

    def saves24_points(self, M: int, Mp: int, has_feat: bool = True) -> int:
        return int(self._lib.i2sdf_blocked_points(self._plan, 2, M, Mp, int(has_feat))) if self.saves24 else 0

    @staticmethod
    def saved_to_point_major(t: torch.Tensor, n_blocked: int, p24_layers=None) -> torch.Tensor:
        if n_blocked <= 0:
            return t.clone()
        Lr, Mp, H = t.shape
        assert H == 256 and n_blocked % 32 == 0
        out = t.clone()
        out[:, :n_blocked] = t[:, :n_blocked].reshape(Lr, n_blocked // 32, 16, 32, 16).permute(0, 1, 3, 2, 4).reshape(Lr, n_blocked, 256)
        if p24_layers is not None and any(p24_layers):
            assert n_blocked == Mp, "packed records: every point is blocked"
            nb = Mp // 32
            for l in range(Lr):
                if not p24_layers[l]:
                    continue
                raw = t[l].reshape(-1)[: nb * 6144].view(torch.int32).reshape(nb, 16, 384)
                hi16 = raw[:, :, :256].contiguous().view(torch.int16).reshape(nb, 16, 32, 2, 8).to(torch.int32) & 0xFFFF
                mid = raw[:, :, 256:].contiguous().view(torch.uint8).reshape(nb, 16, 32, 2, 8).to(torch.int32)
                val = ((hi16 << 16) | (mid << 8)).view(torch.float32)
                v = val.reshape(nb, 16, 32, 2, 2, 4).permute(0, 2, 1, 4, 3, 5)
                out[l] = v.reshape(Mp, 256)
        return out

    def saved_pm(self, name: str, t: torch.Tensor, M: int, has_feat: bool = True) -> torch.Tensor:
        Mp = t.shape[1]
        if name in ("rs", "gar"):
            return self.saved_to_point_major(t, self.blocked_points(1, M, Mp))[:, :M]
        nb = self.blocked_points(0, M, Mp, has_feat)
        p24 = None
        if name in ("abars", "gus", "gas") and self.saves24_points(M, Mp, has_feat) == Mp:
            p24 = [True] * t.shape[0]
            if name == "gus":
                p24[-1] = False
                p24[0] = False
        return self.saved_to_point_major(t, nb, p24)[:, :M]

    def set_tail_overlap(self, on: bool):
        L.check(self._lib.i2sdf_plan_set_option(self._plan, L.OPT_TAIL_OVERLAP, int(bool(on))), "i2sdf_plan_set_option")
        self.tail_overlap = bool(on)

    def _sync_parts(self):
        want = self._parts_wanted if (self.train_forward_bf16x3 and self.sdf_backward_bf16x3 and self.rgb_bf16x3) else 0
        if want != self.parts:
            n = int(want) if int(want) >= 2 else 0
            L.check(self._lib.i2sdf_plan_set_option(self._plan, L.OPT_PARTS, n), "i2sdf_plan_set_option")
            self.parts = n

    def set_parts(self, n: int):
        self._parts_wanted = int(n) if int(n) >= 2 else 0
        self._sync_parts()

    def chain(self, M: int):
        eng = self
        if not getattr(self, "use_chain", True) or not self.parts:
            import contextlib
            return contextlib.nullcontext()

        class _Chain:
            def __enter__(self_):
                L.check(eng._lib.i2sdf_chain_begin(eng._plan, int(M), L.stream_ptr()), "i2sdf_chain_begin")
                return self_

            def __exit__(self_, *exc):
                L.check(eng._lib.i2sdf_chain_end(eng._plan, L.stream_ptr()), "i2sdf_chain_end")
                return False

            def fence(self_):
                L.check(eng._lib.i2sdf_chain_fence(eng._plan, L.stream_ptr()), "i2sdf_chain_fence")

        return _Chain()

    def set_exchange(self, ex, flags: int = 0):
        self._exchange = ex
        L.check(self._lib.i2sdf_plan_set_exchange(self._plan, C.byref(ex) if ex is not None else None, int(flags)), "i2sdf_plan_set_exchange")

    def set_wgrad_bf16x3(self, on: bool):
        L.check(self._lib.i2sdf_plan_set_option(self._plan, L.OPT_WGRAD_BF16X3, int(bool(on))), "i2sdf_plan_set_option")
        self.wgrad_bf16x3 = bool(on)

    def sdf_forward(self, points: torch.Tensor, want_features: bool = False):
        pts = points.detach().to(torch.float32).contiguous()
        M = pts.shape[0]
        sdf = torch.empty(M, 1, dtype=torch.float32, device=pts.device)
        feat = torch.empty(M, self.F, dtype=torch.float32, device=pts.device) if want_features else None
        L.check(self._lib.i2sdf_sdf_forward(self._plan, self._pk(), L.ptr(pts), M, L.ptr(sdf), L.ptr(feat), self.F,
                                            L.stream_ptr()), "i2sdf_sdf_forward")
        return (sdf, feat) if want_features else sdf

    @staticmethod
    def pad_rows(M: int) -> int:
        return (M + 127) // 128 * 128

    def _ws(self, *shape, device=None):
        return torch.empty(*shape, dtype=torch.float32, device=device)

    def sdf_forward_grad(self, points=None, rays=None, want_grad=True, save=True, want_feat=True):
        cfgs = self.cfg.sdf
        H, NL = cfgs.hidden, cfgs.n_lin
        pts = cam = dirs = z = None
        n_ray, ldz, npr = 0, 0, 1
        if rays is not None:
            cam, dirs, z = (t.detach().to(torch.float32).contiguous() for t in rays[:3])
            npr = rays[3] if len(rays) > 3 else z.shape[1]
            n_ray, ldz = z.shape[0] * npr, z.shape[1]
            dev = z.device
        if points is not None:
            pts = points.detach().to(torch.float32).contiguous()
            dev = pts.device
        M = n_ray + (pts.shape[0] if pts is not None else 0)
        Mp = self.pad_rows(M)
        out = {"Mp": Mp, "M": M, "n_ray_pts": n_ray, "pts": pts, "rays": (cam, dirs, z, npr), "sdf": torch.empty(M, 1, dtype=torch.float32, device=dev),
               "blk": self.blocked_points(0, M, Mp, want_feat)}
        out["feat"] = self._ws(Mp, self.F, device=dev) if want_feat else None
        out["grad"] = torch.empty(M, 3, dtype=torch.float32, device=dev) if want_grad else None
        out["hs"] = self._ws(NL - 1, Mp, H, device=dev) if (save or want_grad) else None
        out["abars"] = self._ws(NL - 1, Mp, H, device=dev) if (save and want_grad) else None
        out["pe"] = self._ws(Mp, 40, device=dev) if save else None
        L.check(self._lib.i2sdf_sdf_forward_grad(self._plan, self._pk(), L.ptr(pts), L.ptr(cam), L.ptr(dirs), L.ptr(z),
                                                  ldz, npr, n_ray, M, Mp, L.ptr(out["sdf"]), L.ptr(out["feat"]), L.ptr(out["grad"]),
                                                  L.ptr(out["hs"]), L.ptr(out["abars"]), L.ptr(out["pe"]), L.stream_ptr()),
                 "i2sdf_sdf_forward_grad")
        return out

    @property
    def idr(self) -> bool:
        return self.cfg.rgb_mode == "idr"

    @property
    def rgb_act(self) -> str:
        return self.cfg.rgb_act

    def set_view_embed(self, B: torch.Tensor):
        B = B.detach().to("cpu", torch.float32).contiguous()
        if B.dim() != 2:
            raise ValueError(f"set_view_embed: B must be (3, channels); got {tuple(B.shape)}")
        L.check(self._lib.i2sdf_plan_set_view_embed(self._plan, C.c_void_p(B.data_ptr()), B.shape[0], B.shape[1]), "i2sdf_plan_set_view_embed")
        self.view_embed_B = B

    def rgb_forward(self, dirs, n_per_ray, feat, M, save=True, fw=None, points=None, normals=None):
        Mp = feat.shape[0]
        rgb = torch.empty(M, 3, dtype=torch.float32, device=feat.device)
        Lr, Hr = self.cfg.rgb.n_lin, self.cfg.rgb.hidden
        rs = self._ws(Lr - 1, Mp, Hr, device=feat.device) if save else None
        side = (40 if self.idr else 32) if self.cfg.rgb.embed != "positional" else ((self.cfg.rgb.pe_dim + 7) // 8 * 8 if self.idr else 32)
        pev = self._ws(Mp, side, device=feat.device) if save else None
        no_B = self.cfg.rgb.embed == "fourier" and getattr(self, "view_embed_B", None) is None
        if self.idr:
            cam = z = pts = None
            ldz = 0
            if points is not None:
                pts = points.detach().to(torch.float32).contiguous()
                if pts.shape[0] < M:
                    raise ValueError(f"rgb_forward: {pts.shape[0]} points for {M} radiance samples")
            else:
                if fw is None or fw["rays"][2] is None or fw["n_ray_pts"] < M or fw["rays"][3] != n_per_ray:
                    raise ValueError("rgb_forward ('idr' mode): needs the sdf_forward_grad result whose leading ray samples are the M points, or `points`")
                cam, _, z, _ = fw["rays"]
                ldz = z.shape[1]
            nrm = normals if normals is not None else (fw["grad"] if fw is not None else None)
            if nrm is None or nrm.shape[0] < M:
                raise ValueError("rgb_forward ('idr' mode): needs the normals (d sdf/dx) of the M points")
            nrm = nrm.detach().to(torch.float32).contiguous()
            dirs = dirs.contiguous()
            if dirs.shape[0] * n_per_ray < M:
                raise ValueError(f"rgb_forward: {dirs.shape[0]} view directions x {n_per_ray} samples for {M} points")
            L.check(self._lib.i2sdf_rgb_forward_idr(self._plan, self._pk(), L.ptr(pts), L.ptr(cam), L.ptr(dirs), L.ptr(z), ldz, n_per_ray,
                                                    L.ptr(nrm), L.ptr(feat), M, Mp, L.ptr(rgb), L.ptr(rs), L.ptr(pev), L.stream_ptr()),
                    "i2sdf_rgb_forward_idr", reason=no_B)
            return rgb, rs, pev
        L.check(self._lib.i2sdf_rgb_forward(self._plan, self._pk(), L.ptr(dirs.contiguous()), n_per_ray, L.ptr(feat), M, Mp,
                                             L.ptr(rgb), L.ptr(rs), L.ptr(pev), L.stream_ptr()), "i2sdf_rgb_forward", reason=no_B)
        return rgb, rs, pev

    def rgb_backward(self, rgb, rgb_bar, rs, M, nbar=None, accumulate=True):
        Mp, dev = rs.shape[1], rs.device
        Lr, Hr = self.cfg.rgb.n_lin, self.cfg.rgb.hidden
        gar = self._ws(Lr - 1, Mp, Hr, device=dev)
        ga_last = self._ws(Mp, 4, device=dev)
        fbar = self._ws(Mp, self.F, device=dev)
        if self.idr:
            if nbar is None or nbar.shape[0] < M or nbar.dtype != torch.float32 or not nbar.is_contiguous():
                raise ValueError("rgb_backward ('idr' mode): needs a contiguous fp32 `nbar` of at least M rows")
            L.check(self._lib.i2sdf_rgb_backward_idr(self._plan, self._pk(), L.ptr(rgb), L.ptr(rgb_bar.contiguous()), L.ptr(rs), M, Mp,
                                                     L.ptr(gar), L.ptr(ga_last), L.ptr(fbar), L.ptr(nbar), int(bool(accumulate)), L.stream_ptr()),
                    "i2sdf_rgb_backward_idr")
            return gar, ga_last, fbar
        L.check(self._lib.i2sdf_rgb_backward(self._plan, self._pk(), L.ptr(rgb), L.ptr(rgb_bar.contiguous()), L.ptr(rs), M, Mp,
                                              L.ptr(gar), L.ptr(ga_last), L.ptr(fbar), L.stream_ptr()), "i2sdf_rgb_backward")
        return gar, ga_last, fbar

    def sdf_backward(self, fw, sbar=None, fbar=None, m_fbar=0, nbar=None):
        cfgs = self.cfg.sdf
        H, NL = cfgs.hidden, cfgs.n_lin
        Mp, M, dev = fw["Mp"], fw["M"], fw["hs"].device
        cam, dirs, z, npr = fw["rays"]
        o = {"gus": self._ws(NL, Mp, H, device=dev), "gpbar": self._ws(Mp, 40, device=dev), "gas": self._ws(NL - 1, Mp, H, device=dev),
             "ga_last4": self._ws(Mp, 4, device=dev), "ones4": self._ws(Mp, 4, device=dev)}
        c = lambda t: None if t is None else t.contiguous()
        L.check(self._lib.i2sdf_sdf_backward(self._plan, self._pk(), L.ptr(fw["pts"]), L.ptr(cam), L.ptr(dirs), L.ptr(z),
                                              z.shape[1] if z is not None else 0, npr, fw["n_ray_pts"], M, Mp,
                                              L.ptr(fw["hs"]), L.ptr(fw["abars"]), L.ptr(c(sbar)), L.ptr(c(fbar)), m_fbar, L.ptr(c(nbar)),
                                              L.ptr(o["gus"]), L.ptr(o["gpbar"]), L.ptr(o["gas"]), L.ptr(o["ga_last4"]), L.ptr(o["ones4"]),
                                              L.stream_ptr()), "i2sdf_sdf_backward")
        return o

    def weight_grads(self, flat_params, grad_flat, fw, bw, M_main=0, fbar=None, rgb_fw=None, rgb_bw=None, light=None):
        tb = L.TrainBuffers()
        tb.M_sdf, tb.M_main, tb.Mp = fw["M"], M_main, fw["Mp"]
        P = lambda t: None if t is None else t.data_ptr()
        tb.pe, tb.hs, tb.abars = P(fw["pe"]), P(fw["hs"]), P(fw["abars"])
        tb.gus, tb.gpbar, tb.gas, tb.ga_last4, tb.ones4 = P(bw["gus"]), P(bw["gpbar"]), P(bw["gas"]), P(bw["ga_last4"]), P(bw["ones4"])
        tb.fbar = P(fbar)
        tb.feat = P(fw["feat"])
        if rgb_fw is not None:
            tb.pev, tb.rs = P(rgb_fw["pev"]), P(rgb_fw["rs"])
            tb.gar, tb.ga_last_rgb = P(rgb_bw["gar"]), P(rgb_bw["ga_last"])
        if light is not None:
            tb.hl, tb.gal0, tb.gal_last = P(light["hl"]), P(light["gal0"]), P(light["gal_last"])
        ch = int(self._lib.i2sdf_wgrad_chunk_points())
        n_chunks = (fw["M"] + ch - 1) // ch
        partials = torch.empty(n_chunks * self.wgrad_floats, dtype=torch.float32, device=flat_params.device)
        L.check(self._lib.i2sdf_weight_grads(self._plan, C.byref(tb), L.ptr(flat_params), L.ptr(partials), n_chunks, L.ptr(grad_flat),
                                              L.stream_ptr()), "i2sdf_weight_grads")
        return partials

    def ray_setup(self, uv, pose, intrinsics):
        uv, pose, intrinsics = (t.detach().to(torch.float32).contiguous() for t in (uv, pose, intrinsics))
        quat = pose.dim() == 2 and pose.shape[1] == 7
        if not quat and tuple(pose.shape[1:]) != (4, 4):
            raise ValueError(f"pose must be (batch,4,4) or (batch,7), got {tuple(pose.shape)}")
        batch, pixels = uv.shape[0], uv.shape[1]
        N = batch * pixels
        cam = torch.empty(N, 3, dtype=torch.float32, device=uv.device)
        dirs = torch.empty_like(cam)
        dnorm = torch.empty(N, dtype=torch.float32, device=uv.device)
        L.check(self._lib.i2sdf_ray_setup_ex(L.ptr(uv), L.ptr(pose), int(quat), L.ptr(intrinsics), batch, pixels, L.ptr(cam),
                                              L.ptr(dirs), L.ptr(dnorm), L.stream_ptr()), "i2sdf_ray_setup_ex")
        return cam, dirs, dnorm

    def sphere_intersections(self, cam_loc, dirs, radius):
        cam_loc, dirs = cam_loc.detach().float().contiguous(), dirs.detach().float().contiguous()
        N = cam_loc.shape[0]
        out = torch.empty(N, 2, dtype=torch.float32, device=cam_loc.device)
        miss = torch.zeros(1, dtype=torch.int32, device=cam_loc.device)
        L.check(self._lib.i2sdf_sphere_intersections(L.ptr(cam_loc), L.ptr(dirs), N, float(radius), L.ptr(out), L.ptr(miss),
                                                      L.stream_ptr()), "i2sdf_sphere_intersections")
        if int(miss.item()) > 0:
            raise ValueError(f"BOUNDING SPHERE PROBLEM: {int(miss.item())} rays do not intersect the sphere of radius {radius}")
        return out

    def composite_forward(self, beta_param, z_all, sdf, rgb, grad, lmask, dnorm, want_normal, save=True, eik_grad=None):
        B, n = z_all.shape[0], z_all.shape[1] - 1
        dev = z_all.device
        o = {"rgb": torch.empty(B, 3, device=dev), "depth": torch.empty(B, device=dev), "wsum": torch.empty(B, 1, device=dev)}
        o["normal"] = torch.empty(B, 3, device=dev) if want_normal else None
        o["lmask"] = torch.empty(B, 1, device=dev) if lmask is not None else None
        o["w"] = torch.empty(B, n, device=dev) if save else None
        o["nsum"] = torch.empty(B, 3, device=dev) if (save and want_normal) else None
        if eik_grad is not None and eik_grad.shape[0] == 3 * B and B > 0:
            o["grad_theta"], o["diff_norm"] = torch.empty(2 * B, 3, device=dev), torch.empty(B, device=dev)
            L.check(self._lib.i2sdf_composite_forward_eik(L.ptr(beta_param), self.cfg.beta_min, L.ptr(z_all), z_all.shape[1], L.ptr(sdf),
                                                           L.ptr(rgb), L.ptr(grad) if want_normal else None, L.ptr(lmask), L.ptr(dnorm), B, n,
                                                           L.ptr(o["rgb"]), L.ptr(o["depth"]), L.ptr(o["wsum"]), L.ptr(o["normal"]),
                                                           L.ptr(o["lmask"]), L.ptr(o["w"]), L.ptr(o["nsum"]), L.ptr(eik_grad.contiguous()),
                                                           L.ptr(o["grad_theta"]), L.ptr(o["diff_norm"]), L.stream_ptr()), "i2sdf_composite_forward_eik")
            return o
        L.check(self._lib.i2sdf_composite_forward(L.ptr(beta_param), self.cfg.beta_min, L.ptr(z_all), z_all.shape[1], L.ptr(sdf),
                                                   L.ptr(rgb), L.ptr(grad) if want_normal else None, L.ptr(lmask), L.ptr(dnorm), B, n,
                                                   L.ptr(o["rgb"]), L.ptr(o["depth"]), L.ptr(o["wsum"]), L.ptr(o["normal"]),
                                                   L.ptr(o["lmask"]), L.ptr(o["w"]), L.ptr(o["nsum"]), L.stream_ptr()),
                 "i2sdf_composite_forward")
        return o

    def composite_backward(self, beta_param, z_all, sdf, rgb, grad, dnorm, nsum, g_rgb, g_depth, g_wsum, g_normal, g_lmask,
                           beta_grad_accum=None, sdf_bar_out=None, grad_bar_out=None):
        B, n = z_all.shape[0], z_all.shape[1] - 1
        dev = z_all.device
        M = B * n
        o = {"sdf_bar": sdf_bar_out if sdf_bar_out is not None else torch.empty(M, device=dev), "rgb_bar": torch.empty(M, 3, device=dev)}
        o["grad_bar"] = grad_bar_out if grad_bar_out is not None else (torch.empty(M, 3, device=dev) if g_normal is not None else None)
        o["lmask_bar"] = torch.empty(M, device=dev) if g_lmask is not None else None
        part = torch.empty(B, device=dev)
        c = lambda t: None if t is None else t.contiguous()
        L.check(self._lib.i2sdf_composite_backward(L.ptr(beta_param), self.cfg.beta_min, L.ptr(z_all), z_all.shape[1], L.ptr(sdf),
                                                    L.ptr(rgb), L.ptr(grad), L.ptr(dnorm), L.ptr(nsum), B, n, L.ptr(c(g_rgb)),
                                                    L.ptr(c(g_depth)), L.ptr(c(g_wsum)), L.ptr(c(g_normal)), L.ptr(c(g_lmask)),
                                                    L.ptr(o["sdf_bar"]), L.ptr(o["rgb_bar"]), L.ptr(o["grad_bar"]), L.ptr(o["lmask_bar"]),
                                                    L.ptr(part), L.ptr(beta_grad_accum), L.stream_ptr()), "i2sdf_composite_backward")
        o["beta_partial"] = part
        return o

    def training_draws(self, B: int, seed: int, device, eik_radius: float = 0.0, want_eik: bool = True):
        sc = self.cfg.sampler
        e = lambda *s, dt=torch.float32: torch.empty(*s, dtype=dt, device=device)
        d = {"strat_u": e(B, sc.N_samples_eval), "cdf_u": e(B, sc.N_samples),
             "extra_idx": e(sc.max_total_iters, sc.N_samples_extra, dt=torch.int32) if sc.N_samples_extra > 0 else None,
             "eik_idx": e(B, dt=torch.int32), "eik_pts": e(B, 3) if want_eik else None, "nbr_off": e(B, 3) if want_eik else None}
        L.check(self._lib.i2sdf_training_draws(int(seed) & (2 ** 64 - 1), B, sc.N_samples_eval, sc.N_samples, sc.N_samples_extra, sc.max_total_iters,
                                               self.n_z, float(eik_radius), 0.005, L.ptr(d["strat_u"]), L.ptr(d["cdf_u"]), L.ptr(d["extra_idx"]),
                                               L.ptr(d["eik_idx"]), L.ptr(d["eik_pts"]), L.ptr(d["nbr_off"]), L.stream_ptr()), "i2sdf_training_draws")
        return d

    def sample_rays(self, flat_params, cam, dirs, training=False, strat_u=None, cdf_u=None, extra_idx=None, eik_idx=None, force_iters=0,
                    workspace=None):
        B, dev = cam.shape[0], cam.device
        n_ws = int(self._lib.i2sdf_sampler_workspace_floats(B))
        if workspace is None:
            ws = torch.empty(n_ws, dtype=torch.float32, device=dev)
        else:
            ws = workspace
            if not (ws.is_cuda and ws.device == dev and ws.dtype == torch.float32 and ws.is_contiguous() and ws.numel() >= n_ws):
                raise ValueError(f"workspace must be a contiguous fp32 tensor of at least {n_ws} elements on {dev}")
        z_out = torch.empty(B, self.n_z, dtype=torch.float32, device=dev)
        z_eik = torch.empty(B, 1, dtype=torch.float32, device=dev)
        iters = torch.empty(1, dtype=torch.int32, device=dev) if B > 0 else torch.zeros(1, dtype=torch.int32, device=dev)
        i32 = lambda t: None if t is None else t.to(torch.int32).contiguous()
        if training:
            u_final, ldu = cdf_u.contiguous(), cdf_u.shape[1]
        else:
            u_final, ldu = self.u_final, 0
        ex, ek = i32(extra_idx), i32(eik_idx)
        su = None if strat_u is None else strat_u.contiguous()
        L.check(self._lib.i2sdf_sample_rays(self._plan, self._pk(), L.ptr(flat_params), C.byref(self._scfg), L.ptr(cam.contiguous()),
                                             L.ptr(dirs.contiguous()), B, 1 if training else 0, L.ptr(self.t_lin), L.ptr(self.u_more),
                                             L.ptr(u_final), ldu, L.ptr(self.extra_tab), L.ptr(su), L.ptr(ex), L.ptr(ek), force_iters,
                                             L.ptr(ws), L.ptr(z_out), self.n_z, L.ptr(z_eik), L.ptr(iters), L.stream_ptr()),
                 "i2sdf_sample_rays")
        self._last_sampler_ws = ws
        return z_out, z_eik, iters

    def trace_rays(self, cam_loc, dirs, t_min=None, t_max=None, *, eps=1e-4, max_steps=64, step_scale=1.0, route="auto", return_f=False,
                   workspace=None, out=None):
        from . import trace as T
        cfg = T.check_trace_cfg(eps, max_steps, step_scale, route)
        cam, dirs, t0, t1 = T.check_trace_rays(cam_loc, dirs, self.cfg.sampler.near if t_min is None else t_min,
                                               2.0 * self.cfg.scene_bounding_sphere if t_max is None else t_max)
        N, dev = cam.shape[0], cam.device
        if dev.type != self.device.type or (self.device.index is not None and dev.index != self.device.index):
            raise ValueError(f"trace_rays: the rays are on {dev}, the engine on {self.device}")
        out = dict(out or {})
        shapes = {"t": ((N,), torch.float32), "status": ((N,), torch.int32), "steps": ((N,), torch.int32), "f_trace": ((max_steps, N), torch.float32)}
        for k, b in out.items():
            if k not in shapes:
                raise ValueError(f"trace_rays: out has no entry {k!r}")
            shp, dt = shapes[k]
            if not (isinstance(b, torch.Tensor) and tuple(b.shape) == shp and b.dtype == dt and b.device == dev and b.is_contiguous()):
                raise ValueError(f"trace_rays: out[{k!r}] must be a contiguous {dt} tensor {shp} on {dev}")
        t = out["t"] if "t" in out else torch.empty(N, dtype=torch.float32, device=dev)
        status = out["status"] if "status" in out else torch.empty(N, dtype=torch.int32, device=dev)
        steps = out["steps"] if "steps" in out else torch.empty(N, dtype=torch.int32, device=dev)
        f_trace = None
        if return_f:
            f_trace = out["f_trace"] if "f_trace" in out else torch.full((max_steps, N), float("nan"), dtype=torch.float32, device=dev)
        n_ws = int(self._lib.i2sdf_trace_workspace_floats(N))
        if workspace is None:
            ws = torch.empty(max(n_ws, 1), dtype=torch.float32, device=dev)
        else:
            ws = workspace
            if not (ws.device == dev and ws.dtype == torch.float32 and ws.is_contiguous() and ws.numel() >= n_ws):
                raise ValueError(f"trace_rays: workspace must be a contiguous fp32 tensor of at least {n_ws} elements on {dev}")
        if N > 0:
            L.check(self._lib.i2sdf_trace_rays(self._plan, self._pk(), C.byref(cfg), L.ptr(cam), L.ptr(dirs), L.ptr(t0), L.ptr(t1), N, L.ptr(t),
                                               L.ptr(status), L.ptr(steps), L.ptr(f_trace), L.ptr(ws), L.stream_ptr()), "i2sdf_trace_rays", reason=True)
        elif cfg.route == L.TRACE_ROUTES["fused"]:
            L.check(self._lib.i2sdf_trace_rays(self._plan, None, C.byref(cfg), None, None, None, None, 0, None, None, None, None, None, None),
                    "i2sdf_trace_rays", reason=True)
        return T.TraceResultF(t, status, steps, f_trace) if return_f else T.TraceResult(t, status, steps)

    def error_bound(self, z, sdf, beta, d_star=None, want_d_star=False):
        z, sdf = z.detach().float().contiguous(), sdf.detach().float().reshape(z.shape).contiguous()
        B, n = z.shape
        beta = beta.detach().float().reshape(-1).contiguous().to(z.device)
        if beta.numel() not in (1, B):
            raise ValueError("beta must be a scalar or one value per ray")
        bound = torch.empty(B, dtype=torch.float32, device=z.device)
        ds_out = torch.empty(B, n - 1, dtype=torch.float32, device=z.device) if want_d_star else None
        ds_in = None if d_star is None else d_star.detach().float().contiguous()
        L.check(self._lib.i2sdf_error_bound(L.ptr(z), L.ptr(sdf), B, n, L.ptr(beta), 0 if beta.numel() == 1 else 1, L.ptr(ds_in),
                                            L.ptr(ds_out), L.ptr(bound), L.stream_ptr()), "i2sdf_error_bound")
        return (bound, ds_out) if want_d_star else bound

    def render_image(self, flat_params, uv, pose, intrinsics, chunk, want_normal=True, want_z=False, out=None):
        uv = uv.detach().to(torch.float32).reshape(-1, 2).contiguous()
        pose = pose.detach().to(torch.float32).contiguous()
        intrinsics = intrinsics.detach().to(torch.float32).reshape(4, 4).contiguous()
        quat = pose.numel() == 7
        if not quat and pose.numel() != 16:
            raise ValueError(f"one view: pose must be (4,4) or (7,), got {tuple(pose.shape)}")
        P, dev = uv.shape[0], uv.device
        chunk = int(max(1, min(chunk, max(P, 1))))
        n_ws = int(self._lib.i2sdf_render_image_workspace_floats(self._plan, C.byref(self._scfg), chunk))
        ws = getattr(self, "_img_ws", None)
        if ws is None or ws.numel() < n_ws or ws.device != dev:
            ws = torch.empty(n_ws, dtype=torch.float32, device=dev)
            self._img_ws = ws
        e = lambda *s: torch.empty(*s, dtype=torch.float32, device=dev)
        o = {"rgb": e(P, 3), "depth": e(P), "wsum": e(P, 1), "normal": e(P, 3) if want_normal else None,
             "lmask": e(P, 1) if self.cfg.light is not None else None, "z": e(P, self.n_z) if want_z else None,
             "iters": torch.zeros((P + chunk - 1) // chunk, dtype=torch.int32, device=dev)}
        for k, t in (out or {}).items():
            if o.get(k) is None or t.shape != o[k].shape or t.dtype != o[k].dtype or t.device != dev or not t.is_contiguous():
                raise ValueError(f"render_image: out[{k!r}] does not fit (want {None if o.get(k) is None else tuple(o[k].shape)})")
            o[k] = t.zero_() if k == "iters" else t
        L.check(self._lib.i2sdf_render_image(self._plan, self._pk(), L.ptr(flat_params), C.byref(self._scfg), L.ptr(uv), L.ptr(pose),
                                             int(quat), L.ptr(intrinsics), P, chunk, L.ptr(self.t_lin), L.ptr(self.u_more), L.ptr(self.u_final),
                                             L.ptr(self.extra_tab), L.ptr(ws), L.ptr(o["rgb"]), L.ptr(o["depth"]), L.ptr(o["wsum"]),
                                             L.ptr(o["normal"]), L.ptr(o["lmask"]), L.ptr(o["z"]), L.ptr(o["iters"]), L.stream_ptr()),
                "i2sdf_render_image")
        return o

    def sdf_grid(self, x, y, z, rot=None, trans=None, order: int = L.GRID_ORDER_VOLUME, first: int = 0, count: Optional[int] = None,
                 chunk: int = 1 << 21):
        x, y, z = (t.detach().to(torch.float32).contiguous() for t in (x, y, z))
        dev = x.device
        nx, ny, nz = x.numel(), y.numel(), z.numel()
        total = nx * ny * nz
        count = total - first if count is None else count
        chunk = int(max(128, min(chunk, max(count, 128))))
        ws = getattr(self, "_grid_ws", None)
        n_ws = int(self._lib.i2sdf_sdf_grid_workspace_floats(chunk))
        if ws is None or ws.numel() < n_ws or ws.device != dev:
            ws = torch.empty(n_ws, dtype=torch.float32, device=dev)
            self._grid_ws = ws
        out = torch.empty(count, dtype=torch.float32, device=dev)
        host = lambda v, n: None if v is None else (C.c_float * n)(*[float(a) for a in torch.as_tensor(v, dtype=torch.float32).reshape(-1).tolist()])
        r, t = host(rot, 9), host(trans, 3)
        L.check(self._lib.i2sdf_sdf_grid(self._plan, self._pk(), L.ptr(x), L.ptr(y), L.ptr(z), nx, ny, nz, int(order),
                                         C.cast(r, C.c_void_p) if r is not None else None, C.cast(t, C.c_void_p) if t is not None else None,
                                         int(first), int(count), L.ptr(out), L.ptr(ws), chunk, L.stream_ptr()), "i2sdf_sdf_grid")
        return out

    def light_forward(self, feat, M, save=True):
        Mp, dev = feat.shape[0], feat.device
        HL = self.cfg.light.hidden
        lm = torch.empty(M, dtype=torch.float32, device=dev)
        hl = self._ws(Mp, HL, device=dev) if save else None
        L.check(self._lib.i2sdf_light_forward(self._plan, self._pk(), L.ptr(feat), M, Mp, L.ptr(lm), L.ptr(hl), L.stream_ptr()),
                 "i2sdf_light_forward")
        return lm, hl

    def light_backward(self, lm, lm_bar, hl, M):
        Mp, dev = hl.shape[0], hl.device
        gal0 = self._ws(Mp, hl.shape[1], device=dev)
        gal_last = self._ws(Mp, 4, device=dev)
        L.check(self._lib.i2sdf_light_backward(self._plan, self._pk(), L.ptr(lm), L.ptr(lm_bar.contiguous()), L.ptr(hl), M, Mp,
                                                L.ptr(gal0), L.ptr(gal_last), L.stream_ptr()), "i2sdf_light_backward")
        return gal0, gal_last
```

### i2sdf_amd/lib.py

```python
from __future__ import annotations

import ctypes as C
import os

MAX_LAYERS = 12
_HERE = os.path.dirname(os.path.abspath(__file__))
LIB_PATH = os.environ.get("I2SDF_LIB_PATH") or os.path.join(_HERE, "lib", "libi2sdf_hip.so")


class MlpDesc(C.Structure):
    _fields_ = [("n_lin", C.c_int32), ("hidden", C.c_int32), ("d_in", C.c_int32), ("in0", C.c_int32), ("d_out", C.c_int32),
                ("multires", C.c_int32), ("skip_layer", C.c_int32), ("reserved", C.c_int32),
                ("out_dim", C.c_int32 * MAX_LAYERS), ("in_dim", C.c_int32 * MAX_LAYERS),
                ("off_bias", C.c_int64 * MAX_LAYERS), ("off_g", C.c_int64 * MAX_LAYERS), ("off_v", C.c_int64 * MAX_LAYERS)]


class NetDesc(C.Structure):
    _fields_ = [("sdf", MlpDesc), ("rgb", MlpDesc), ("light", MlpDesc), ("off_beta", C.c_int64), ("n_params", C.c_int64),
                ("beta_min", C.c_float), ("scene_bounding_sphere", C.c_float)]


class TrainBuffers(C.Structure):
    _fields_ = [("M_sdf", C.c_int64), ("M_main", C.c_int64), ("Mp", C.c_int64)] + [(n, C.c_void_p) for n in (
        "pe", "hs", "abars", "gus", "gpbar", "gas", "ga_last4", "ones4", "fbar", "pev", "feat", "rs", "gar", "ga_last_rgb",
        "hl", "gal0", "gal_last")]


class SamplerCfg(C.Structure):
    _fields_ = [("near", C.c_float), ("eps", C.c_float), ("add_tiny", C.c_float), ("N_samples", C.c_int32), ("N_samples_eval", C.c_int32),
                ("N_samples_extra", C.c_int32), ("beta_iters", C.c_int32), ("max_total_iters", C.c_int32)]


EXCHANGE_FN = C.CFUNCTYPE(C.c_int, C.c_void_p, C.c_void_p, C.c_int64, C.c_int32, C.c_int32, C.c_void_p)


class Exchange(C.Structure):
    _fields_ = [("allreduce", EXCHANGE_FN), ("ctx", C.c_void_p)]


class TraceCfg(C.Structure):
    _fields_ = [("eps", C.c_float), ("step_scale", C.c_float), ("max_steps", C.c_int32), ("route", C.c_int32)]


class LossCfg(C.Structure):
    _fields_ = [(n, C.c_float) for n in ("eikonal_w", "smooth_w", "mask_w", "depth_w", "normal_w", "angular_w", "bubble_w", "light_w")] + \
               [("smooth_on", C.c_int32), ("reserved", C.c_int32), ("exchange", C.POINTER(Exchange))]


XCHG_F32, XCHG_I32 = 0, 1
XCHG_SUM, XCHG_AVG, XCHG_MAX = 0, 1, 2
DP_GLOBAL_SAMPLER = 1
COMM_UNIQUE_ID_BYTES = 128


class RayTables(C.Structure):
    _fields_ = [("intrinsics", C.c_void_p), ("pose", C.c_void_p), ("pose_is_quat", C.c_int32), ("n_images", C.c_int32),
                ("height", C.c_int32), ("width", C.c_int32)] + \
               [(n, C.c_void_p) for n in ("rgb", "depth", "normal", "mask", "light_mask", "depth_mask", "normal_mask")]


class RayBatch(C.Structure):
    _fields_ = [(n, C.c_void_p) for n in ("image_idx", "uv", "cam_loc", "dirs", "dnorm", "rgb", "depth", "normal", "mask", "light_mask",
                                          "depth_mask", "normal_mask", "n_bad")]


OPT_SDF_FWD_BF16X3 = 1
OPT_WGRAD_BF16X3 = 2
OPT_TRAIN_FWD_BF16X3 = 4
OPT_SDF_BWD_BF16X3 = 8
OPT_RGB_BF16X3 = 16
OPT_TAIL_OVERLAP = 32
OPT_BLOCKED_SAVES = 128
OPT_WGRAD_BF16X2 = 256
OPT_PARTS = 512
OPT_SAMPLER_BF16X2 = 1024
OPT_SAVES24 = 2048
MAX_PARTS = 4
GRID_ORDER_MESHGRID, GRID_ORDER_VOLUME = 0, 1
RGB_MODE_NERF, RGB_MODE_IDR = 0, 1
RGB_ACTS = {"sigmoid": 0, "relu": 1, "softplus": 2}
RGB_EMBEDS = {"positional": 0, "spherical_harmonics": 1, "fourier": 2}
RGB_EMBED_MAX_CHANNELS = 12
RASTER_SMALL_MAX = 64
TSDF_MAX_CELLS = 1 << 24
IMAGE_STATS = 8
SSIM_TILE_X, SSIM_TILE_Y = 32, 16
BUBBLE_MAX_K = 4096
BUBBLE_WS_PASSES_OFFSET = 24
KMEANS_MAX_K = 256
DBSCAN_NONFINITE, DBSCAN_CELLS = 1, 2
TRACE_HIT, TRACE_MISS, TRACE_UNRESOLVED, TRACE_INSIDE = 1, 2, 3, 4
TRACE_ROUTES = {"auto": 0, "stepwise": 1, "fused": 2}
TRACE_MAX_STEPS = 1024


class I2SDFError(RuntimeError):
    pass


_lib = None

_P, _I64, _I32, _F, _D = C.c_void_p, C.c_int64, C.c_int32, C.c_float, C.c_double
SIGNATURES = {
    "i2sdf_version": (C.c_int, []),
    "i2sdf_strerror": (C.c_char_p, [C.c_int]),
    "i2sdf_last_hip_error": (C.c_char_p, []),
    "i2sdf_plan_create": (C.c_int, [C.POINTER(NetDesc), C.POINTER(_P)]),
    "i2sdf_plan_destroy": (None, [_P]),
    "i2sdf_plan_set_option": (C.c_int, [_P, _I32, _I32]),
    "i2sdf_chain_begin": (C.c_int, [_P, _I64, _P]),
    "i2sdf_chain_fence": (C.c_int, [_P, _P]),
    "i2sdf_chain_end": (C.c_int, [_P, _P]),
    "i2sdf_blocked_points": (_I64, [_P, _I32, _I64, _I64, _I32]),
    "i2sdf_plan_pack_floats": (_I64, [_P]),
    "i2sdf_plan_wgrad_floats": (_I64, [_P]),
    "i2sdf_pack_weights": (C.c_int, [_P, _P, _P, _P]),
    "i2sdf_sdf_forward": (C.c_int, [_P, _P, _P, _I64, _P, _P, _I64, _P]),
    "i2sdf_sdf_forward_grad": (C.c_int, [_P] * 6 + [_I64, _I32, _I64, _I64, _I64] + [_P] * 7),
    "i2sdf_plan_set_view_embed": (C.c_int, [_P, _P, _I32, _I32]),
    "i2sdf_rgb_forward": (C.c_int, [_P, _P, _P, _I32, _P, _I64, _I64, _P, _P, _P, _P]),
    "i2sdf_rgb_backward": (C.c_int, [_P] * 5 + [_I64, _I64] + [_P] * 4),
    "i2sdf_rgb_forward_idr": (C.c_int, [_P] * 6 + [_I64, _I32, _P, _P, _I64, _I64] + [_P] * 4),
    "i2sdf_rgb_backward_idr": (C.c_int, [_P] * 5 + [_I64, _I64] + [_P] * 4 + [_I32, _P]),
    "i2sdf_sdf_backward": (C.c_int, [_P] * 6 + [_I64, _I32, _I64, _I64, _I64] + [_P] * 4 + [_I64] + [_P] * 7),
    "i2sdf_wgrad_chunk_points": (_I64, []),
    "i2sdf_weight_grads": (C.c_int, [_P, C.POINTER(TrainBuffers), _P, _P, _I64, _P, _P]),
    "i2sdf_comm_available": (_I32, []),
    "i2sdf_comm_unique_id": (C.c_int, [_P, _I64]),
    "i2sdf_comm_init_rank": (C.c_int, [_P, _I32, _I32, C.POINTER(_P)]),
    "i2sdf_comm_destroy": (None, [_P]),
    "i2sdf_comm_size": (_I32, [_P]),
    "i2sdf_comm_rank": (_I32, [_P]),
    "i2sdf_last_comm_error": (C.c_char_p, []),
    "i2sdf_allreduce_grads": (C.c_int, [_P, _I64, _P, _P]),
    "i2sdf_allreduce_max_i32": (C.c_int, [_P, _I64, _P, _P]),
    "i2sdf_broadcast": (C.c_int, [_P, _I64, _I32, _P, _P]),
    "i2sdf_comm_as_exchange": (C.c_int, [_P, C.POINTER(Exchange)]),
    "i2sdf_plan_set_exchange": (C.c_int, [_P, C.POINTER(Exchange), _I32]),
    "i2sdf_adam_step": (C.c_int, [_P, _P, _P, _P, _I64, _D, _D, _D, _D, _D, _I64, _D, _P]),
    "i2sdf_error_bound": (C.c_int, [_P, _P, _I64, _I32, _P, _I64, _P, _P, _P, _P]),
    "i2sdf_sampler_workspace_floats": (_I64, [_I64]),
    "i2sdf_sample_rays": (C.c_int, [_P, _P, _P, C.POINTER(SamplerCfg), _P, _P, _I64, _I32, _P, _P, _P, _I64, _P, _P, _P, _P, _I32, _P, _P,
                                    _I64, _P, _P, _P]),
    "i2sdf_render_image_workspace_floats": (_I64, [_P, C.POINTER(SamplerCfg), _I64]),
    "i2sdf_render_image": (C.c_int, [_P, _P, _P, C.POINTER(SamplerCfg), _P, _P, _I32, _P, _I64, _I64] + [_P] * 13),
    "i2sdf_sdf_grid_workspace_floats": (_I64, [_I64]),
    "i2sdf_sdf_grid": (C.c_int, [_P, _P, _P, _P, _P, _I32, _I32, _I32, _I32, _P, _P, _I64, _I64, _P, _P, _I64, _P]),
    "i2sdf_marching_cubes_workspace_bytes": (_I64, [_I32, _I32, _I32]),
    "i2sdf_marching_cubes_count": (C.c_int, [_P, _I32, _I32, _I32, _F, _P, _P, _P]),
    "i2sdf_marching_cubes_emit": (C.c_int, [_P, _I32, _I32, _I32, _F, _P, _P, _P, _P, _P, _P, _I64, _I64, _P]),
    "i2sdf_mesh_scan_workspace_bytes": (_I64, [_I64]),
    "i2sdf_mesh_status": (C.c_int, [_P, _P]),
    "i2sdf_mesh_edge_keys": (C.c_int, [_P, _I64, _I64, _P, _P, _P]),
    "i2sdf_mesh_face_components": (C.c_int, [_P, _P, _I64, _P, _P]),
    "i2sdf_mesh_face_areas": (C.c_int, [_P, _I64, _P, _I64, _P, _P, _P]),
    "i2sdf_mesh_cumsum_f64": (C.c_int, [_P, _I64, _P, _I64, _P, _P, _P]),
    "i2sdf_mesh_largest_label": (C.c_int, [_P, _P, _I64, _P, _P]),
    "i2sdf_mesh_compact_mark": (C.c_int, [_P, _P, _I64, _I64, _P, _P, _P, _P]),
    "i2sdf_mesh_compact_gather": (C.c_int, [_P, _P, _I64, _P, _I64, _P, _P, _P, _P, _P, _P, _P, _I64, _I64, _P]),
    "i2sdf_mesh_sample_surface": (C.c_int, [_P, _I64, _P, _I64, _P, _P, _P, _I64, _P, _P, _P, _P]),
    "i2sdf_points_bounds": (C.c_int, [_P, _I64, _P, _P, _P]),
    "i2sdf_points_voxel_keys": (C.c_int, [_P, _I64, _P, _D, _P, _P, _P]),
    "i2sdf_points_voxel_heads": (C.c_int, [_P, _I64, _P, _P]),
    "i2sdf_points_voxel_mean": (C.c_int, [_P, _I64, _P, _P, _P, _P, _P, _I64, _P]),
    "i2sdf_points_grid_workspace_bytes": (_I64, [_I64]),
    "i2sdf_points_grid_keys": (C.c_int, [_P, _I64, _P, _P, _P, _P]),
    "i2sdf_points_grid_build": (C.c_int, [_P, _I64, _P, _P, _P, _P, _P]),
    "i2sdf_points_nn_query": (C.c_int, [_P, _I64, _P, _I64, _P, _I32, _P, _P, _P, _P, _P]),
    "i2sdf_points_nn_fallback": (C.c_int, [_P, _I64, _P, _I64, _P, _P, _P, _P, _P]),
    "i2sdf_points_reduce_workspace_bytes": (_I64, [_I64]),
    "i2sdf_points_threshold_reduce": (C.c_int, [_P, _I64, _D, _P, _P, _P]),
    "i2sdf_raster_workspace_bytes": (_I64, [_I64, _I64, _I32]),
    "i2sdf_raster_depth": (C.c_int, [_P, _I64, _P, _I64, _P, _I32, _P, _I32, _I32, _F, _F, _I32, _P, _P, _P, _P, _P]),
    "i2sdf_tsdf_table_cells": (_I64, [_P]),
    "i2sdf_tsdf_extract_workspace_bytes": (_I64, [_I64]),
    "i2sdf_tsdf_bounds": (C.c_int, [_P, _I32, _I32, _I32, _P, _P, _F, _F, _F, _F, _I32, _P, _P]),
    "i2sdf_tsdf_mark": (C.c_int, [_P, _I32, _I32, _I32, _I32, _P, _P, _F, _F, _F, _F, _I32, _P, _P, _I64, _P, _P, _P, _P, _P]),
    "i2sdf_tsdf_integrate": (C.c_int, [_P, _I32, _I32, _I32, _I32, _P, _P, _F, _F, _F, _F, _P, _P, _I64, _P, _P, _P, _P, _P]),
    "i2sdf_tsdf_count": (C.c_int, [_P, _P, _P, _I64, _P, _P, _P, _P, _P]),
    "i2sdf_tsdf_emit": (C.c_int, [_P, _F, _F, _P, _P, _I64, _P, _P, _P, _P, _P, _P, _P, _I64, _I64, _P]),
    "i2sdf_image_workspace_bytes": (_I64, [_I32, _I32, _I32]),
    "i2sdf_image_stats": (C.c_int, [_P, _P, _P, _I32, _I32, _I32, _P, _P, _P]),
    "i2sdf_image_ssim": (C.c_int, [_P, _P, _I32, _I32, _I32, _F, _P, _P, _P, _P, _P]),
    "i2sdf_image_frames": (C.c_int, [_P] * 6 + [_I32, _I32, _I32] + [_P] * 6),
    "i2sdf_linear_to_srgb": (C.c_int, [_P, _P, _I64, _I32, _P]),
    "i2sdf_pdf_update": (C.c_int, [_P, _P, _I32, _P, _I64, _I64, _P, _I64, C.c_double, C.c_double, _P, _I64, _P, _P]),
    "i2sdf_training_draws": (C.c_int, [C.c_uint64, _I64, _I32, _I32, _I32, _I32, _I32, C.c_float, C.c_float, _P, _P, _P, _P, _P, _P, _P]),
    "i2sdf_bubble_sample_workspace_bytes": (_I64, [_I64]),
    "i2sdf_bubble_sample": (C.c_int, [_P, _I64, _P, _I64, C.c_uint64, C.c_uint32, _P, _P, _P, _P, _P, _P]),
    "i2sdf_bubble_keys": (C.c_int, [_P, _I64, C.c_uint64, C.c_uint32, _P, _P]),
    "i2sdf_depth_unproject_workspace_bytes": (_I64, [_I64, _I32, _I32]),
    "i2sdf_depth_unproject_count": (C.c_int, [_P, _I64, _I32, _I32, _F, _F, _P, _P, C.POINTER(_I64), _P]),
    "i2sdf_depth_unproject_write": (C.c_int, [_P, _P, _P, _I64, _I32, _I32, _F, _F, _P, _I64, _P, _P, _P, _P]),
    "i2sdf_shade_draws": (C.c_int, [C.c_uint64, _I64, _I32, _P, _P]),
    "i2sdf_shade_sample": (C.c_int, [_P] * 7 + [C.POINTER(C.c_uint64), _I64, _I32] + [_P] * 4),
    "i2sdf_shade_reduce": (C.c_int, [_P] * 6 + [C.POINTER(C.c_uint64), _P, _P, _I64, _I32] + [_P] * 3),
    "i2sdf_shade_backward_workspace_bytes": (_I64, [_I64, _I32]),
    "i2sdf_shade_backward": (C.c_int, [_P] * 6 + [C.POINTER(C.c_uint64)] + [_P] * 6 + [_I64, _I32] + [_P] * 7),
    "i2sdf_kmeans_workspace_bytes": (_I64, [_I64, _I64]),
    "i2sdf_kmeans_pp": (C.c_int, [_P, _I64, _I64, C.c_uint64, _P, _P, _P, _P]),
    "i2sdf_kmeans_fit": (C.c_int, [_P, _I64, _I64, _P, _I32, _D, _P, _P, _P, _P]),
    "i2sdf_kmeans_assign": (C.c_int, [_P, _I64, _P, _I64, _P, _P, _P]),
    "i2sdf_dbscan_workspace_bytes": (_I64, [_I64]),
    "i2sdf_dbscan_cell_keys": (C.c_int, [_P, _I64, _D, _P, _P, _P, _P]),
    "i2sdf_dbscan_label": (C.c_int, [_P, _I64, _D, _I32, _P, _P, _P, _P, _P, _P, _P, _P]),
    "i2sdf_trace_workspace_floats": (_I64, [_I64]),
    "i2sdf_trace_rays": (C.c_int, [_P, _P, C.POINTER(TraceCfg)] + [_P] * 4 + [_I64] + [_P] * 6),
    "i2sdf_light_forward": (C.c_int, [_P, _P, _P, _I64, _I64, _P, _P, _P]),
    "i2sdf_light_backward": (C.c_int, [_P, _P, _P, _P, _P, _I64, _I64, _P, _P, _P]),
    "i2sdf_loss_scratch_floats": (_I64, []),
    "i2sdf_loss_forward_backward": (C.c_int, [C.POINTER(LossCfg), _I64, _I64] + [_P] * 27),
    "i2sdf_eikonal_outputs_forward": (C.c_int, [_P, _I64, _P, _P, _P]),
    "i2sdf_extra_points": (C.c_int, [_P, _P, _P, _P, _P, _I64, _P, _P]),
    "i2sdf_render_loss_scratch_floats": (_I64, [_I64]),
    "i2sdf_render_loss_backward": (C.c_int, [C.POINTER(LossCfg), _I64, _I32, _I64, _I64, _I64, _I64, _P, C.c_float, _P, _I64] + [_P] * 5 + [_P] * 8 + [_P] * 7 +
                                   [_P] * 3 + [_P] * 8 + [_P, _P, _P, _I32, _P, _P, _P]),
    "i2sdf_scale_seeds": (C.c_int, [_P, _P, _I64, _P, _I64, _P, _I64, _P, _I64, _P, _P, _P]),
    "i2sdf_backward_seeds": (C.c_int, [_P, _I64, _P, _P, _I64, _I64, _P, _I64, _P, _I64, C.c_int32, _P]),
    "i2sdf_eikonal_outputs_backward": (C.c_int, [_P, _P, _P, _I64, _P, _P]),
    "i2sdf_ray_setup": (C.c_int, [_P, _P, _P, _I64, _I32, _P, _P, _P, _P]),
    "i2sdf_ray_setup_ex": (C.c_int, [_P, _P, _I32, _P, _I64, _I32, _P, _P, _P, _P]),
    "i2sdf_ray_batch": (C.c_int, [C.POINTER(RayTables), _P, _I64, C.POINTER(RayBatch), _P]),
    "i2sdf_sphere_intersections": (C.c_int, [_P, _P, _I64, _F, _P, _P, _P]),
    "i2sdf_composite_forward": (C.c_int, [_P, _F, _P, _I64, _P, _P, _P, _P, _P, _I64, _I32] + [_P] * 8),
    "i2sdf_composite_forward_eik": (C.c_int, [_P, _F, _P, _I64, _P, _P, _P, _P, _P, _I64, _I32] + [_P] * 11),
    "i2sdf_composite_backward": (C.c_int, [_P, _F, _P, _I64] + [_P] * 5 + [_I64, _I32] + [_P] * 12),
}


def load():
    global _lib
    if _lib is not None:
        return _lib
    import torch
    if not os.path.exists(LIB_PATH):
        raise I2SDFError(f"{LIB_PATH} not found: build it with `python -c 'import __graft_entry__ as g; g.build()'` "
                         "(hipcc --offload-arch=gfx950). There is no CPU fallback.")
    lib = C.CDLL(LIB_PATH)
    for name, (res, args) in SIGNATURES.items():
        fn = getattr(lib, name)
        fn.restype, fn.argtypes = res, args
    _lib = lib
    return lib


def check(rc: int, what: str = "", reason: bool = False):
    if rc != 0:
        lib = load()
        msg = lib.i2sdf_strerror(rc).decode()
        if rc == -2 or (rc == -1 and (reason or what in ("i2sdf_plan_create", "i2sdf_plan_set_view_embed"))):
            msg += ": " + lib.i2sdf_last_hip_error().decode()
        if rc == -5:
            msg += ": " + lib.i2sdf_last_comm_error().decode()
        raise I2SDFError(f"{what} failed ({rc}): {msg}")


def ptr(t):
    if t is None:
        return None
    assert t.is_contiguous(), "C ABI needs contiguous tensors"
    return C.c_void_p(t.data_ptr())


def stream_ptr():
    import torch
    return C.c_void_p(torch.cuda.current_stream().cuda_stream)
```

### include/i2sdf.h

```cpp
#ifndef I2SDF_H
#define I2SDF_H

#include <stddef.h>
#include <stdint.h>

#ifdef __cplusplus
extern "C" {
#endif

#define I2SDF_VERSION 100
#define I2SDF_MAX_LAYERS 12
#define I2SDF_MAX_PARTS 4

#define I2SDF_OK 0
#define I2SDF_EINVAL (-1)
#define I2SDF_EHIP (-2)
#define I2SDF_ESPHERE (-3)
#define I2SDF_EWORKSPACE (-4)
#define I2SDF_ECOMM (-5)

typedef struct i2sdf_mlp_desc {
  int32_t n_lin;
  int32_t hidden;
  int32_t d_in;
  int32_t in0;
  int32_t d_out;
  int32_t multires;
  int32_t skip_layer;
  int32_t reserved;
  int32_t out_dim[I2SDF_MAX_LAYERS];
  int32_t in_dim[I2SDF_MAX_LAYERS];
  int64_t off_bias[I2SDF_MAX_LAYERS];
  int64_t off_g[I2SDF_MAX_LAYERS];
  int64_t off_v[I2SDF_MAX_LAYERS];
} i2sdf_mlp_desc;

#define I2SDF_RGB_MODE_NERF 0
#define I2SDF_RGB_MODE_IDR 1
#define I2SDF_RGB_ACT_SIGMOID 0
#define I2SDF_RGB_ACT_RELU 1
#define I2SDF_RGB_ACT_SOFTPLUS 2
#define I2SDF_RGB_EMBED_POSITIONAL 0
#define I2SDF_RGB_EMBED_SH 1
#define I2SDF_RGB_EMBED_FOURIER 2
#define I2SDF_RGB_EMBED_MAX_CHANNELS 12

typedef struct i2sdf_net_desc {
  i2sdf_mlp_desc sdf;
  i2sdf_mlp_desc rgb;
  i2sdf_mlp_desc light;
  int64_t off_beta;
  int64_t n_params;
  float beta_min;
  float scene_bounding_sphere;
} i2sdf_net_desc;

typedef struct i2sdf_plan i2sdf_plan;

int i2sdf_version(void);
const char* i2sdf_strerror(int code);
const char* i2sdf_last_hip_error(void);

int i2sdf_plan_create(const i2sdf_net_desc* desc, i2sdf_plan** out);
void i2sdf_plan_destroy(i2sdf_plan* plan);
#define I2SDF_OPT_SDF_FWD_BF16X3 1
#define I2SDF_OPT_WGRAD_BF16X3 2
#define I2SDF_OPT_TRAIN_FWD_BF16X3 4
#define I2SDF_OPT_SDF_BWD_BF16X3 8
#define I2SDF_OPT_RGB_BF16X3 16
#define I2SDF_OPT_TAIL_OVERLAP 32
#define I2SDF_OPT_BLOCKED_SAVES 128
#define I2SDF_OPT_WGRAD_BF16X2 256
#define I2SDF_OPT_PARTS 512
#define I2SDF_OPT_SAMPLER_BF16X2 1024
#define I2SDF_OPT_SAVES24 2048
int64_t i2sdf_blocked_points(const i2sdf_plan* plan, int32_t which, int64_t M, int64_t Mp, int32_t has_feat);
int i2sdf_plan_set_option(i2sdf_plan* plan, int32_t option, int32_t value);
int i2sdf_chain_begin(const i2sdf_plan* plan, int64_t M, void* stream);
int i2sdf_chain_fence(const i2sdf_plan* plan, void* stream);
int i2sdf_chain_end(const i2sdf_plan* plan, void* stream);
int64_t i2sdf_plan_pack_floats(const i2sdf_plan* plan);
int64_t i2sdf_plan_wgrad_floats(const i2sdf_plan* plan);

int i2sdf_pack_weights(const i2sdf_plan* plan, const float* params, float* packed, void* stream);

int i2sdf_sdf_forward(const i2sdf_plan* plan, const float* packed, const float* points, int64_t M,
                      float* sdf_out, float* feat_out, int64_t ld_feat, void* stream);


int i2sdf_sdf_forward_grad(const i2sdf_plan* plan, const float* packed, const float* points, const float* cam,
                           const float* dirs, const float* z, int64_t ldz, int32_t n_per_ray, int64_t n_ray_pts, int64_t M,
                           int64_t Mp, float* sdf, float* feat, float* grad, float* hs, float* abars, float* pe_save,
                           void* stream);

int i2sdf_plan_set_view_embed(i2sdf_plan* plan, const float* B_host, int32_t rows, int32_t cols);

int i2sdf_rgb_forward(const i2sdf_plan* plan, const float* packed, const float* dirs, int32_t n_per_ray, const float* feat,
                      int64_t M, int64_t Mp, float* rgb, float* rs, float* pev_save, void* stream);

int i2sdf_rgb_forward_idr(const i2sdf_plan* plan, const float* packed, const float* points, const float* cam, const float* dirs,
                          const float* z, int64_t ldz, int32_t n_per_ray, const float* normals, const float* feat, int64_t M, int64_t Mp,
                          float* rgb, float* rs, float* pev_save, void* stream);

int i2sdf_rgb_backward(const i2sdf_plan* plan, const float* packed, const float* rgb, const float* rgb_bar, const float* rs,
                       int64_t M, int64_t Mp, float* gar, float* ga_last, float* fbar, void* stream);

int i2sdf_rgb_backward_idr(const i2sdf_plan* plan, const float* packed, const float* rgb, const float* rgb_bar, const float* rs,
                           int64_t M, int64_t Mp, float* gar, float* ga_last, float* fbar, float* nbar, int32_t accumulate, void* stream);

int i2sdf_sdf_backward(const i2sdf_plan* plan, const float* packed, const float* points, const float* cam, const float* dirs,
                       const float* z, int64_t ldz, int32_t n_per_ray, int64_t n_ray_pts, int64_t M, int64_t Mp,
                       const float* hs, const float* abars, const float* sbar, const float* fbar, int64_t m_fbar,
                       const float* nbar, float* gus, float* gpbar, float* gas, float* ga_last4, float* ones4, void* stream);

int i2sdf_ray_setup(const float* uv, const float* pose, const float* intrinsics, int64_t batch, int32_t pixels,
                    float* cam_loc, float* dirs, float* dnorm, void* stream);
int i2sdf_ray_setup_ex(const float* uv, const float* pose, int32_t pose_is_quat, const float* intrinsics, int64_t batch,
                       int32_t pixels, float* cam_loc, float* dirs, float* dnorm, void* stream);

typedef struct i2sdf_ray_tables {
  const float* intrinsics;
  const float* pose;
  int32_t pose_is_quat;
  int32_t n_images, height, width;
  const float* rgb;
  const float* depth;
  const float* normal;
  const float* mask;
  const float* light_mask;
  const uint8_t* depth_mask;
  const uint8_t* normal_mask;
} i2sdf_ray_tables;

typedef struct i2sdf_ray_batch_out {
  int64_t* image_idx;
  float* uv;
  float* cam_loc;
  float* dirs;
  float* dnorm;
  float* rgb;
  float* depth;
  float* normal;
  float* mask;
  float* light_mask;
  uint8_t* depth_mask;
  uint8_t* normal_mask;
  int32_t* n_bad;
} i2sdf_ray_batch_out;

int i2sdf_ray_batch(const i2sdf_ray_tables* tables, const int64_t* tidx, int64_t n_rays, const i2sdf_ray_batch_out* out, void* stream);

int i2sdf_sphere_intersections(const float* cam_loc, const float* dirs, int64_t n_rays, float radius, float* t_near_far,
                               int32_t* n_miss, void* stream);

int i2sdf_composite_forward(const float* beta_param, float beta_min, const float* z, int64_t ldz, const float* sdf,
                            const float* rgb, const float* grad, const float* lmask, const float* dnorm, int64_t B, int32_t n,
                            float* o_rgb, float* o_depth, float* o_wsum, float* o_normal, float* o_lmask, float* w_save,
                            float* nsum_save, void* stream);

int i2sdf_composite_forward_eik(const float* beta_param, float beta_min, const float* z, int64_t ldz, const float* sdf,
                                const float* rgb, const float* grad, const float* lmask, const float* dnorm, int64_t B, int32_t n,
                                float* o_rgb, float* o_depth, float* o_wsum, float* o_normal, float* o_lmask, float* w_save,
                                float* nsum_save, const float* grad_all, float* grad_theta, float* diff_norm, void* stream);

int i2sdf_composite_backward(const float* beta_param, float beta_min, const float* z, int64_t ldz, const float* sdf,
                             const float* rgb, const float* grad, const float* dnorm, const float* nsum_save, int64_t B, int32_t n,
                             const float* g_rgb, const float* g_depth, const float* g_wsum, const float* g_normal,
                             const float* g_lmask, float* sdf_bar, float* rgb_bar, float* grad_bar, float* lmask_bar,
                             float* beta_partial, float* beta_grad_accum, void* stream);


typedef struct i2sdf_train_buffers {
  int64_t M_sdf;
  int64_t M_main;
  int64_t Mp;
  const float *pe, *hs, *abars, *gus, *gpbar, *gas, *ga_last4, *ones4, *fbar;
  const float *pev, *feat, *rs, *gar, *ga_last_rgb;
  const float *hl, *gal0, *gal_last;
} i2sdf_train_buffers;

int64_t i2sdf_wgrad_chunk_points(void);
int i2sdf_weight_grads(const i2sdf_plan* plan, const i2sdf_train_buffers* bufs, const float* params, float* partials,
                       int64_t n_chunks_cap, float* grad_flat, void* stream);


typedef struct i2sdf_comm i2sdf_comm;
#define I2SDF_COMM_UNIQUE_ID_BYTES 128
#define I2SDF_DP_GLOBAL_SAMPLER 1
#define I2SDF_XCHG_F32 0
#define I2SDF_XCHG_I32 1
#define I2SDF_XCHG_SUM 0
#define I2SDF_XCHG_AVG 1
#define I2SDF_XCHG_MAX 2
typedef struct i2sdf_exchange {
  int (*allreduce)(void* ctx, void* buf, int64_t n, int32_t dtype, int32_t op, void* stream);
  void* ctx;
} i2sdf_exchange;
int32_t i2sdf_comm_available(void);
int i2sdf_comm_unique_id(void* out, int64_t out_bytes);
int i2sdf_comm_init_rank(const void* unique_id, int32_t nranks, int32_t rank, i2sdf_comm** out);
void i2sdf_comm_destroy(i2sdf_comm* comm);
int32_t i2sdf_comm_size(const i2sdf_comm* comm);
int32_t i2sdf_comm_rank(const i2sdf_comm* comm);
const char* i2sdf_last_comm_error(void);
int i2sdf_allreduce_grads(float* flat, int64_t n, const i2sdf_comm* comm, void* stream);
int i2sdf_allreduce_max_i32(int32_t* flags, int64_t n, const i2sdf_comm* comm, void* stream);
int i2sdf_broadcast(void* buf, int64_t bytes, int32_t root, const i2sdf_comm* comm, void* stream);
int i2sdf_comm_as_exchange(const i2sdf_comm* comm, i2sdf_exchange* out);
int i2sdf_plan_set_exchange(i2sdf_plan* plan, const i2sdf_exchange* ex, int32_t flags);

int i2sdf_adam_step(float* params, const float* grads, float* exp_avg, float* exp_avg_sq, int64_t n, double lr, double beta1,
                    double beta2, double eps, double weight_decay, int64_t step, double grad_scale, void* stream);

typedef struct i2sdf_sampler_cfg {
  float near, eps, add_tiny;
  int32_t N_samples, N_samples_eval, N_samples_extra, beta_iters, max_total_iters;
} i2sdf_sampler_cfg;

int i2sdf_error_bound(const float* z, const float* sdf, int64_t B, int32_t n, const float* beta, int64_t ldbeta,
                      const float* d_star_in, float* d_star_out, float* bound, void* stream);

int64_t i2sdf_sampler_workspace_floats(int64_t B);
int i2sdf_sample_rays(const i2sdf_plan* plan, const float* packed, const float* params, const i2sdf_sampler_cfg* cfg,
                      const float* cam, const float* dirs, int64_t B, int32_t training, const float* t_lin, const float* u_more,
                      const float* u_final, int64_t ldu_final, const int32_t* extra_tab, const float* strat_u,
                      const int32_t* extra_idx, const int32_t* eik_idx, int32_t force_iters, float* workspace, float* z_out,
                      int64_t ldz, float* z_eik, int32_t* iters_out, void* stream);


int i2sdf_light_forward(const i2sdf_plan* plan, const float* packed, const float* feat, int64_t M, int64_t Mp, float* lm, float* hl,
                        void* stream);
int i2sdf_light_backward(const i2sdf_plan* plan, const float* packed, const float* lm, const float* lm_bar, const float* hl, int64_t M,
                         int64_t Mp, float* gal0, float* gal_last, void* stream);


typedef struct i2sdf_loss_cfg {
  float eikonal_w, smooth_w, mask_w, depth_w, normal_w, angular_w, bubble_w, light_w;
  int32_t smooth_on;
  int32_t reserved;
  const i2sdf_exchange* exchange;
} i2sdf_loss_cfg;

int64_t i2sdf_loss_scratch_floats(void);
int i2sdf_loss_forward_backward(const i2sdf_loss_cfg* cfg, int64_t B, int64_t n_pc, const float* rgb, const float* depth,
                                const float* wsum, const float* normal, const float* grad_theta, const float* diff_norm,
                                const float* surface, const float* lmask, const float* gt_rgb, const float* gt_depth,
                                const uint8_t* depth_mask, const float* gt_normal, const uint8_t* normal_mask, const float* gt_mask,
                                const float* gt_lmask, float* scratch, float* losses, float* loss_value, float* g_rgb, float* g_depth, float* g_wsum,
                                float* g_normal, float* g_grad_theta, float* g_diff_norm, float* g_surface, float* g_lmask,
                                void* stream);

int i2sdf_eikonal_outputs_forward(const float* grad_all, int64_t B, float* grad_theta, float* diff_norm, void* stream);
int i2sdf_eikonal_outputs_backward(const float* grad_all, const float* grad_theta_bar, const float* diff_norm_bar, int64_t B,
                                   float* grad_all_bar, void* stream);

int i2sdf_extra_points(const float* cam, const float* dirs, const float* z_eik, const float* eik_pts, const float* nbr_off, int64_t B,
                       float* out, void* stream);

int i2sdf_backward_seeds(float* beta_grad, int64_t n_beta, float* sdf_bar, float* grad_bar, int64_t M_main, int64_t M_sdf,
                         const float* g_eik, int64_t n_eik, const float* g_surf, int64_t n_pc, int32_t zero_main_grad, void* stream);

int64_t i2sdf_render_loss_scratch_floats(int64_t B);
int i2sdf_render_loss_backward(const i2sdf_loss_cfg* cfg, int64_t B, int32_t n, int64_t n_pc, int64_t M_main, int64_t M_sdf, int64_t n_eik,
                               const float* beta_param, float beta_min, const float* z, int64_t ldz, const float* sdf, const float* rgb_pts,
                               const float* grad_pts, const float* dnorm, const float* nsum_save,
                               const float* rgb, const float* depth, const float* wsum, const float* normal, const float* grad_theta,
                               const float* diff_norm, const float* surface, const float* lmask,
                               const float* gt_rgb, const float* gt_depth, const uint8_t* depth_mask, const float* gt_normal,
                               const uint8_t* normal_mask, const float* gt_mask, const float* gt_lmask,
                               float* scratch, float* losses, float* loss_value,
                               float* g_rgb, float* g_depth, float* g_wsum, float* g_normal, float* g_grad_theta, float* g_diff_norm,
                               float* g_surface, float* g_lmask,
                               float* sdf_bar, float* rgb_bar, float* grad_bar, int32_t normal_term, float* lmask_bar, float* beta_grad,
                               void* stream);
int i2sdf_scale_seeds(const float* g, float* sdf_bar, int64_t n_sdf, float* grad_bar, int64_t n_grad, float* rgb_bar, int64_t n_rgb,
                      float* lmask_bar, int64_t n_lmask, const float* beta_in, float* beta_out, void* stream);

int64_t i2sdf_render_image_workspace_floats(const i2sdf_plan* plan, const i2sdf_sampler_cfg* cfg, int64_t chunk);
int i2sdf_render_image(const i2sdf_plan* plan, const float* packed, const float* params, const i2sdf_sampler_cfg* cfg,
                       const float* uv, const float* pose, int32_t pose_is_quat, const float* intrinsics, int64_t P, int64_t chunk,
                       const float* t_lin, const float* u_more, const float* u_final, const int32_t* extra_tab, float* workspace,
                       float* o_rgb, float* o_depth, float* o_wsum, float* o_normal, float* o_lmask, float* o_z, int32_t* o_iters,
                       void* stream);

#define I2SDF_GRID_ORDER_MESHGRID 0
#define I2SDF_GRID_ORDER_VOLUME 1
int64_t i2sdf_sdf_grid_workspace_floats(int64_t chunk_points);
int i2sdf_sdf_grid(const i2sdf_plan* plan, const float* packed, const float* x, const float* y, const float* z, int32_t nx,
                   int32_t ny, int32_t nz, int32_t order, const float* rot, const float* trans, int64_t first, int64_t count,
                   float* sdf_out, float* workspace, int64_t chunk_points, void* stream);

int64_t i2sdf_marching_cubes_workspace_bytes(int32_t nx, int32_t ny, int32_t nz);
int i2sdf_marching_cubes_count(const float* vol, int32_t nx, int32_t ny, int32_t nz, float level, void* workspace, int64_t* counts_out,
                               void* stream);
int i2sdf_marching_cubes_emit(const float* vol, int32_t nx, int32_t ny, int32_t nz, float level, const float* spacing,
                              const float* origin, void* workspace, float* verts, float* normals, int32_t* faces, int64_t cap_v,
                              int64_t cap_f, void* stream);

int64_t i2sdf_mesh_scan_workspace_bytes(int64_t n);
int i2sdf_mesh_status(const int32_t* status, void* stream);
int i2sdf_mesh_edge_keys(const int32_t* faces, int64_t F, int64_t n_verts, int64_t* keys, int32_t* status, void* stream);
int i2sdf_mesh_face_components(const int64_t* sorted_keys, const int64_t* perm, int64_t F, int32_t* labels, void* stream);
int i2sdf_mesh_face_areas(const float* verts, int64_t n_verts, const int32_t* faces, int64_t F, float* area, int32_t* status,
                          void* stream);
int i2sdf_mesh_cumsum_f64(const float* x, int64_t n_x, const int64_t* order, int64_t n, double* cdf, void* workspace, void* stream);
int i2sdf_mesh_largest_label(const int32_t* sorted_labels, const double* cdf, int64_t F, int64_t* best, void* stream);
int i2sdf_mesh_compact_mark(const int32_t* faces, const uint8_t* mask, int64_t F, int64_t n_verts, int32_t* fkeep, int32_t* vflag,
                            int32_t* status, void* stream);
int i2sdf_mesh_compact_gather(const float* verts, const float* normals, int64_t n_verts, const int32_t* faces, int64_t F,
                              const int32_t* fkeep, const int32_t* fscan, const int32_t* vflag, const int32_t* vscan,
                              float* out_verts, float* out_normals, int32_t* out_faces, int64_t cap_v, int64_t cap_f, void* stream);
int i2sdf_mesh_sample_surface(const float* verts, int64_t n_verts, const int32_t* faces, int64_t F, const double* cdf,
                              const float* u_face, const float* u_bary, int64_t count, float* points, int32_t* face_index,
                              int32_t* status, void* stream);

int i2sdf_points_bounds(const float* points, int64_t n, int32_t* bounds, int32_t* status, void* stream);
int i2sdf_points_voxel_keys(const float* points, int64_t n, const int32_t* bounds, double voxel_size, int64_t* keys, int32_t* status,
                            void* stream);
int i2sdf_points_voxel_heads(const int64_t* sorted_keys, int64_t n, int32_t* heads, void* stream);
int i2sdf_points_voxel_mean(const float* points, int64_t n, const int64_t* sorted_keys, const int64_t* perm, const int32_t* head_scan,
                            float* out_points, int32_t* out_counts, int64_t cap_m, void* stream);
int64_t i2sdf_points_grid_workspace_bytes(int64_t n_ref);
int i2sdf_points_grid_keys(const float* ref, int64_t n_ref, void* workspace, int64_t* keys, int32_t* status, void* stream);
int i2sdf_points_grid_build(const float* ref, int64_t n_ref, const int64_t* sorted_keys, const int64_t* perm, void* workspace,
                            float* sorted_ref, void* stream);
int i2sdf_points_nn_query(const float* query, int64_t n_query, const float* sorted_ref, int64_t n_ref, const void* workspace,
                          int32_t max_ring, float* dist, int32_t* index, int32_t* fallback_list, int32_t* status, void* stream);
int i2sdf_points_nn_fallback(const float* query, int64_t n_query, const float* ref, int64_t n_ref, const int32_t* fallback_list,
                             const int32_t* status, float* dist, int32_t* index, void* stream);
int64_t i2sdf_points_reduce_workspace_bytes(int64_t n);
int i2sdf_points_threshold_reduce(const float* dist, int64_t n, double threshold, void* workspace, double* out, void* stream);

#define I2SDF_RASTER_SMALL_MAX 64
int64_t i2sdf_raster_workspace_bytes(int64_t n_verts, int64_t F, int32_t n_cam);
int i2sdf_raster_depth(const float* verts, int64_t n_verts, const int32_t* faces, int64_t F, const float* w2c, int32_t n_cam,
                       const float* K4, int32_t H, int32_t W, float znear, float zfar, int32_t cull, void* workspace, float* depth,
                       int32_t* counters, int32_t* status, void* stream);

#define I2SDF_TSDF_MAX_CELLS (1 << 24)
int64_t i2sdf_tsdf_table_cells(const int32_t* grid6);
int64_t i2sdf_tsdf_extract_workspace_bytes(int64_t n_units);
int i2sdf_tsdf_bounds(const float* depths, int32_t n_cam, int32_t H, int32_t W, const float* c2w, const float* K4, float voxel_length,
                      float unit_length, float sdf_trunc, float depth_trunc, int32_t stride, int32_t* bounds, void* stream);
int i2sdf_tsdf_mark(const float* depths, int32_t n_cam, int32_t cam, int32_t H, int32_t W, const float* c2w, const float* K4,
                    float voxel_length, float unit_length, float sdf_trunc, float depth_trunc, int32_t stride, const int32_t* grid6,
                    const int32_t* slot, int64_t n_units, int32_t* stamp, int32_t* list, int32_t* list_count, int32_t* flag, void* stream);
int i2sdf_tsdf_integrate(const float* depths, int32_t n_cam, int32_t cam, int32_t H, int32_t W, const float* w2c, const float* K4,
                         float voxel_length, float unit_length, float sdf_trunc, float depth_trunc, const int32_t* grid6,
                         const int32_t* unit_cell, int64_t n_units, const int32_t* list, const int32_t* list_count, float* tsdf,
                         float* weight, void* stream);
int i2sdf_tsdf_count(const int32_t* grid6, const int32_t* slot, const int32_t* unit_cell, int64_t n_units, const float* tsdf,
                     const float* weight, void* workspace, int64_t* blocks, void* stream);
int i2sdf_tsdf_emit(const int32_t* grid6, float voxel_length, float unit_length, const int32_t* slot, const int32_t* unit_cell,
                    int64_t n_units, const float* tsdf, const float* weight, void* workspace, const int64_t* blocks_excl, float* verts,
                    float* normals, int32_t* faces, int64_t cap_v, int64_t cap_f, void* stream);

#define I2SDF_IMAGE_STATS 8
#define I2SDF_SSIM_TILE_X 32
#define I2SDF_SSIM_TILE_Y 16
int64_t i2sdf_image_workspace_bytes(int32_t n_views, int32_t H, int32_t W);
int i2sdf_image_stats(const float* pred, const float* gt, const float* depth, int32_t n_views, int32_t H, int32_t W, void* workspace,
                      double* stats, void* stream);
int i2sdf_image_ssim(const float* pred, const float* gt, int32_t n_views, int32_t H, int32_t W, float data_range, const double* stats,
                     void* workspace, double* ssim, float* map, void* stream);
int i2sdf_image_frames(const float* rgb, const float* normal, const float* depth, const float* pose, const double* stats,
                       const uint8_t* lut, int32_t n_views, int32_t H, int32_t W, uint8_t* rgb8, uint8_t* normal8, float* normal_cam,
                       uint8_t* depth8, uint8_t* depth_rgb8, void* stream);

int i2sdf_linear_to_srgb(const float* src, float* dst, int64_t n, int32_t clamp01, void* stream);

int i2sdf_pdf_update(const float* pred, const float* target, int32_t channels, const int64_t* pixel_idx, int64_t first_pixel,
                     int64_t n, const int64_t* pointlinks, int64_t n_links, double pdf_max, double pdf_prune, float* pdf,
                     int64_t n_pdf, int32_t* n_bad, void* stream);

int i2sdf_training_draws(uint64_t seed, int64_t B, int32_t n_eval, int32_t n_samples, int32_t n_extra, int32_t max_iters,
                         int32_t n_z, float eik_radius, float nbr_half_width, float* strat_u, float* cdf_u,
                         int32_t* extra_idx, int32_t* eik_idx, float* eik_pts, float* nbr_off, void* stream);

#define I2SDF_BUBBLE_MAX_K 4096
#define I2SDF_BUBBLE_WS_PASSES_OFFSET 24
int64_t i2sdf_bubble_sample_workspace_bytes(int64_t k);
int i2sdf_bubble_sample(const float* weights, int64_t n, const float* pointcloud, int64_t k, uint64_t seed, uint32_t draw,
                        void* workspace, int64_t* idx, float* points, float* sample_count, int32_t* status, void* stream);
int i2sdf_bubble_keys(const float* weights, int64_t n, uint64_t seed, uint32_t draw, float* keys_out, void* stream);

int64_t i2sdf_depth_unproject_workspace_bytes(int64_t n_img, int32_t H, int32_t W);
int i2sdf_depth_unproject_count(const float* depth, int64_t n_img, int32_t H, int32_t W, float lo, float hi, void* workspace,
                                uint8_t* depth_masks, int64_t* n_points, void* stream);
int i2sdf_depth_unproject_write(const float* depth, const float* intrinsics, const float* pose, int64_t n_img, int32_t H, int32_t W,
                                float lo, float hi, const void* workspace, int64_t n_points, int64_t* pointlinks, int64_t* pixlinks,
                                float* pointcloud, void* stream);

int i2sdf_shade_draws(uint64_t seed, int64_t bn, int32_t spp, float* samples, void* stream);
int i2sdf_shade_sample(const float* surface_points, const float* view_direction, const float* normal, const float* Kd, const float* Ks,
                       const float* rough, const float* samples, const uint64_t* seed, int64_t bn, int32_t spp, float* direction,
                       float* points, uint8_t* wi_mask, void* stream);
int i2sdf_shade_reduce(const float* view_direction, const float* normal, const float* Kd, const float* Ks, const float* rough,
                       const float* samples, const uint64_t* seed, const float* radiance, const float* radiance_scale, int64_t bn,
                       int32_t spp, float* colorDiffuse, float* colorSpec, void* stream);
int64_t i2sdf_shade_backward_workspace_bytes(int64_t bn, int32_t spp);
int i2sdf_shade_backward(const float* view_direction, const float* normal, const float* Kd, const float* Ks, const float* rough,
                         const float* samples, const uint64_t* seed, const float* radiance, const float* radiance_scale,
                         const float* g_colorDiffuse, const float* g_colorSpec, const float* g_direction, const float* g_points,
                         int64_t bn, int32_t spp, void* workspace, float* gKd, float* gKs, float* grough, float* g_radiance,
                         float* g_radiance_scale, void* stream);

#define I2SDF_KMEANS_MAX_K 256
int64_t i2sdf_kmeans_workspace_bytes(int64_t n, int64_t k);
int i2sdf_kmeans_pp(const float* points, int64_t n, int64_t k, uint64_t seed, void* workspace, int64_t* idx_out, float* centroids_out,
                    void* stream);
int i2sdf_kmeans_fit(const float* points, int64_t n, int64_t k, float* centroids, int32_t max_iter, double tol, void* workspace,
                     int64_t* labels, int32_t* n_iter, void* stream);
int i2sdf_kmeans_assign(const float* points, int64_t n, const float* centroids, int64_t k, int64_t* labels, float* dist2, void* stream);

#define I2SDF_DBSCAN_NONFINITE 1
#define I2SDF_DBSCAN_CELLS 2
int64_t i2sdf_dbscan_workspace_bytes(int64_t n);
int i2sdf_dbscan_cell_keys(const float* points, int64_t n, double eps, void* workspace, int64_t* keys, int32_t* status, void* stream);
int i2sdf_dbscan_label(const float* points, int64_t n, double eps, int32_t min_samples, const int64_t* sorted_keys, const int64_t* perm,
                       void* workspace, int64_t* labels, uint8_t* core, int32_t* n_clusters, int32_t* status, void* stream);

#define I2SDF_TRACE_ACTIVE 0
#define I2SDF_TRACE_HIT 1
#define I2SDF_TRACE_MISS 2
#define I2SDF_TRACE_UNRESOLVED 3
#define I2SDF_TRACE_INSIDE 4
#define I2SDF_TRACE_AUTO 0
#define I2SDF_TRACE_STEPWISE 1
#define I2SDF_TRACE_FUSED 2
#define I2SDF_TRACE_MAX_STEPS 1024
typedef struct i2sdf_trace_cfg { float eps, step_scale; int32_t max_steps, route; } i2sdf_trace_cfg;
int64_t i2sdf_trace_workspace_floats(int64_t N);
int i2sdf_trace_rays(const i2sdf_plan* plan, const float* packed, const i2sdf_trace_cfg* cfg, const float* cam, const float* dirs,
                     const float* t_min, const float* t_max, int64_t N, float* t_out, int32_t* status_out, int32_t* steps_out,
                     float* f_trace, float* workspace, void* stream);

#ifdef __cplusplus
}
#endif
#endif
```

Baseline: 20.79 million.

## Tile weight packing through LDS and overlap pack with sampler init

The per-chunk pack kernel with its separate rowscale pass is replaced by a task-based kernel. Each block loads a tile of weight rows once into shared memory, computes the weight-norm scale inline, and emits all split/transposed chunks from that tile, so scattered global reads and the binary search over segments go away. The sampler gets an entry point that takes the pack event and waits on it only after its init kernel, so the pack on another stream can overlap sampler setup. The cost is more complex task scheduling, shared-memory use per block, and a new event-reader bookkeeping path in Python.

New measurement: 20.93 million, median of 5. No clear change (+0.7%).

```diff
diff --git a/i2sdf_amd/csrc/pack.hip b/i2sdf_amd/csrc/pack.hip
--- a/i2sdf_amd/csrc/pack.hip
+++ b/i2sdf_amd/csrc/pack.hip
@@ -6,27 +6,40 @@
 
 namespace {
 
-struct RowTab {
-  int32_t n;
-  int32_t rows[3 * I2SDF_MAX_LAYERS], cols[3 * I2SDF_MAX_LAYERS], scale_off[3 * I2SDF_MAX_LAYERS];
-  int64_t off_v[3 * I2SDF_MAX_LAYERS], off_g[3 * I2SDF_MAX_LAYERS];
-};
-
-__global__ __launch_bounds__(256) void rowscale_kernel(RowTab tab, const float* __restrict__ params, float* __restrict__ scale,
-                                                        int n_rows) {
-  const int row = blockIdx.x * 4 + (threadIdx.x >> 6);
-  const int lane = threadIdx.x & 63;
-  if (row >= n_rows) return;
-  int e = 0;
-  while (e + 1 < tab.n && row >= tab.scale_off[e + 1]) ++e;
-  const int r = row - tab.scale_off[e];
-  const int cols = tab.cols[e];
-  const float* v = params + tab.off_v[e] + (int64_t)r * cols;
+constexpr int TILE_STRIDE = PACK_TILE_MAX_COLS + 4;
+constexpr int TILE_COL_STEPS = PACK_TILE_MAX_COLS / 64;
+constexpr int TILE_ROWS_PER_WAVE = PACK_TILE_ROWS / 4, SCALE_ROWS_PER_WAVE = PACK_SCALE_ROWS / 4;
+
+__device__ __forceinline__ float wave_total(float s) {
+#pragma unroll
+  for (int o = 32; o > 0; o >>= 1) s += __shfl_xor(s, o);
+  return s;
+}
+__device__ __forceinline__ float row_scale(const float* __restrict__ params, int64_t off_v, int64_t off_g, int row, int cols, int lane) {
+  const float* v = params + off_v + (int64_t)row * cols;
   float s = 0.f;
   for (int c = lane; c < cols; c += 64) { float x = v[c]; s = fmaf(x, x, s); }
-#pragma unroll
-  for (int o = 32; o > 0; o >>= 1) s += __shfl_xor(s, o);
-  if (lane == 0) scale[row] = params[tab.off_g[e] + r] / sqrtf(s);
+  return params[off_g + row] / sqrtf(wave_total(s));
+}
+
+template <int R>
+__device__ __forceinline__ void load_rows(float (&x)[R][TILE_COL_STEPS], float (&g)[R], const float* __restrict__ params, int64_t off_v, int64_t off_g,
+                                          int row0, int row_end, int cols, int lane) {
+#pragma unroll
+  for (int q = 0; q < R; ++q) {
+    const int row = row0 + 4 * q;
+    const bool ok = row < row_end;
+    const float* v = params + off_v + (int64_t)(ok ? row : row0) * cols;
+    g[q] = ok ? params[off_g + row] : 0.f;
+#pragma unroll
+    for (int i = 0; i < TILE_COL_STEPS; ++i) x[q][i] = (ok && lane + 64 * i < cols) ? v[lane + 64 * i] : 0.f;
+  }
+}
+__device__ __forceinline__ float sum_squares(const float (&x)[TILE_COL_STEPS]) {
+  float s = 0.f;
+#pragma unroll
+  for (int i = 0; i < TILE_COL_STEPS; ++i) s = fmaf(x[i], x[i], s);
+  return s;
 }
 
 __device__ __forceinline__ int map_col(const ColMap& cm, int kp) {
@@ -35,52 +48,119 @@
   return j < cm.valid1 ? cm.base1 + j : -1;
 }
 
-__global__ __launch_bounds__(256) void pack_kernel(const Seg* __restrict__ segs, int n_segs, const float* __restrict__ params,
-                                                    const float* __restrict__ scale, float* __restrict__ chunks,
-                                                    int64_t total_chunks) {
-  const int64_t gid = (int64_t)blockIdx.x * 256 + threadIdx.x;
-  const int64_t chunk = gid >> 6;
-  const int lane = (int)(gid & 63);
-  if (chunk >= total_chunks) return;
-  int lo = 0, hi_ = n_segs - 1;
-  while (lo < hi_) {
-    const int mid = (lo + hi_ + 1) >> 1;
-    if (segs[mid].chunk0 <= chunk) lo = mid; else hi_ = mid - 1;
-  }
-  const Seg s = segs[lo];
-  const int c = (int)(chunk - s.chunk0);
-  const int i32 = lane & 31, hi = lane >> 5;
+__device__ __forceinline__ void put(float* __restrict__ chunks, int64_t chunk, int lane, f32x4 v) {
+  reinterpret_cast<f32x4*>(chunks)[chunk * 64 + lane] = v;
+}
+__device__ __forceinline__ f32x4 as_f32x4(const unsigned (&q)[4]) { return __builtin_bit_cast(f32x4, u32x4{q[0], q[1], q[2], q[3]}); }
+
+__device__ __forceinline__ f32x4 plain_chunk(const Seg& s, int64_t off_g, int c, int lane, const float* __restrict__ params) {
+  const int hi = lane >> 5;
   f32x4 out = {0.f, 0.f, 0.f, 0.f};
-  if (c < s.used) {
-    if (s.type == SEG_BIAS) {
-      const int nt = c / 4, q = c % 4;
-#pragma unroll
-      for (int t = 0; t < 4; ++t) {
-        const int r = 32 * nt + 8 * q + 4 * hi + t;
-        out[t] = (r < s.nrows) ? params[s.off_bias + s.row_off + r] : 0.f;
-      }
-    } else if (s.type == SEG_WFWD) {
-      const int nt = c / s.KC, kc = c % s.KC;
-      const int r = 32 * nt + i32;
-      if (r < s.nrows) {
-        const int row = s.row_off + r;
-        const float sc = scale[s.scale_off + row] * s.mult;
-        const float* v = params + s.off_v + (int64_t)row * s.cols;
-#pragma unroll
-        for (int t = 0; t < 4; ++t) {
-          const int col = map_col(s.cm, 8 * kc + 4 * hi + t);
-          out[t] = col >= 0 ? v[col] * sc : 0.f;
-        }
-      }
-    } else if (s.type == SEG_WFWD3) {
-      const int G = s.NT / 2, w = c >> 1, e = c & 1;
-      const int kc = w / (3 * G), g = (w / 3) % G, sp = w % 3;
-      const int r = 32 * (2 * g + e) + i32;
-      unsigned q[4] = {0u, 0u, 0u, 0u};
-      if (r < s.nrows) {
-        const int row = s.row_off + r;
-        const float sc = scale[s.scale_off + row] * s.mult;
-        const float* v = params + s.off_v + (int64_t)row * s.cols;
+  if (c >= s.used) return out;
+  if (s.type == SEG_BIAS) {
+    const int nt = c / 4, q = c % 4;
+#pragma unroll
+    for (int t = 0; t < 4; ++t) {
+      const int r = 32 * nt + 8 * q + 4 * hi + t;
+      out[t] = (r < s.nrows) ? params[s.off_bias + s.row_off + r] : 0.f;
+    }
+  } else if (s.type == SEG_BIAS_H) {
+    const int kg = lane >> 4;
+#pragma unroll
+    for (int t = 0; t < 4; ++t) {
+      const int r = 16 * c + 4 * kg + t;
+      out[t] = (r < s.nrows) ? params[s.off_bias + s.row_off + r] : 0.f;
+    }
+  } else if (s.type == SEG_ROWVEC || s.type == SEG_ROWVEC_H) {
+    const int rr = c / s.KC, kc = c % s.KC;
+    const int row = s.row_off + rr;
+    const float sc = row_scale(params, s.off_v, off_g, row, s.cols, lane) * s.mult;
+    const int k0 = s.type == SEG_ROWVEC ? 8 * kc + 4 * hi : 16 * kc + 4 * (lane >> 4);
+#pragma unroll
+    for (int t = 0; t < 4; ++t) {
+      const int col = map_col(s.cm, k0 + t);
+      out[t] = col >= 0 ? params[s.off_v + (int64_t)row * s.cols + col] * sc : 0.f;
+    }
+  } else if (s.type == SEG_SCALAR) {
+#pragma unroll
+    for (int t = 0; t < 4; ++t) out[t] = (t < s.nrows) ? params[s.off_bias + s.row_off + t] : 0.f;
+  }
+  return out;
+}
+
+__global__ __launch_bounds__(256) void pack_kernel(const PackTask* __restrict__ tasks, const Seg* __restrict__ segs, const float* __restrict__ params,
+                                                    float* __restrict__ packed, int64_t scale_floats) {
+  __shared__ float tile[PACK_TILE_ROWS * TILE_STRIDE];
+  const PackTask t = tasks[blockIdx.x];
+  const int lane = threadIdx.x & 63, wv = threadIdx.x >> 6;
+  if (t.kind == PACK_SCALE) {
+    if (t.cols == 0) {
+      for (int i = threadIdx.x; i < t.n; i += 256) packed[t.b + i] = 0.f;
+      return;
+    }
+    if (t.cols <= PACK_TILE_MAX_COLS) {
+      float x[SCALE_ROWS_PER_WAVE][TILE_COL_STEPS], g[SCALE_ROWS_PER_WAVE];
+      load_rows<SCALE_ROWS_PER_WAVE>(x, g, params, t.off_v, t.off_g, t.b + wv, t.b + t.n, t.cols, lane);
+#pragma unroll
+      for (int q = 0; q < SCALE_ROWS_PER_WAVE; ++q) {
+        const float sc = g[q] / sqrtf(wave_total(sum_squares(x[q])));
+        if (lane == 0 && wv + 4 * q < t.n) packed[t.scale_off + t.b + wv + 4 * q] = sc;
+      }
+    } else {
+      for (int i = wv; i < t.n; i += 4) {
+        const float sc = row_scale(params, t.off_v, t.off_g, t.b + i, t.cols, lane);
+        if (lane == 0) packed[t.scale_off + t.b + i] = sc;
+      }
+    }
+    return;
+  }
+  const Seg s = segs[t.seg];
+  float* chunks = packed + scale_floats;
+  if (t.kind == PACK_PLAIN) {
+    for (int i = wv; i < t.n; i += 4) put(chunks, s.chunk0 + t.b + i, lane, plain_chunk(s, t.off_g, t.b + i, lane, params));
+    return;
+  }
+  const bool transposed = s.type == SEG_WBWD || s.type == SEG_WBWD3 || s.type == SEG_WBWD3H;
+  const int r0 = t.b * PACK_TILE_ROWS;
+  {
+    float x[TILE_ROWS_PER_WAVE][TILE_COL_STEPS], g[TILE_ROWS_PER_WAVE];
+    load_rows<TILE_ROWS_PER_WAVE>(x, g, params, s.off_v, t.off_g, s.row_off + r0 + wv, s.row_off + s.nrows, s.cols, lane);
+#pragma unroll
+    for (int q = 0; q < TILE_ROWS_PER_WAVE; ++q) {
+      float* trow = tile + (wv + 4 * q) * TILE_STRIDE;
+      const bool row_ok = r0 + wv + 4 * q < s.nrows;
+      const float scale = g[q] / sqrtf(wave_total(sum_squares(x[q])));
+      const float sc = scale * s.mult;
+#pragma unroll
+      for (int i = 0; i < TILE_COL_STEPS; ++i) {
+        const float w = transposed ? x[q][i] * scale * s.mult : x[q][i] * sc;
+        if (lane + 64 * i < s.cols) trow[lane + 64 * i] = row_ok ? w : 0.f;
+      }
+    }
+  }
+  __syncthreads();
+  auto T = [&](int rl, int col) { return tile[rl * TILE_STRIDE + col]; };
+  const int i32 = lane & 31, hi = lane >> 5, i16 = lane & 15, kg = lane >> 4;
+  const int G = s.NT / 2;
+  if (s.type == SEG_WFWD) {
+    const bool row_ok = r0 + i32 < s.nrows;
+    for (int kc = wv; kc < s.KC; kc += 4) {
+      f32x4 out = {0.f, 0.f, 0.f, 0.f};
+      if (row_ok) {
+#pragma unroll
+        for (int e = 0; e < 4; ++e) {
+          const int col = map_col(s.cm, 8 * kc + 4 * hi + e);
+          out[e] = col >= 0 ? T(i32, col) : 0.f;
+        }
+      }
+      put(chunks, s.chunk0 + t.b * s.KC + kc, lane, out);
+    }
+  } else if (s.type == SEG_WFWD3) {
+    const int g = t.b >> 1, e = t.b & 1;
+    const bool row_ok = r0 + i32 < s.nrows;
+    for (int kc = wv; kc < s.KC; kc += 4) {
+      unsigned q[3][4] = {};
+      if (row_ok) {
 #pragma unroll
         for (int i = 0; i < 4; ++i) {
           float x[2];
@@ -88,121 +168,91 @@
           for (int h2 = 0; h2 < 2; ++h2) {
             const int j = 2 * i + h2;
             const int col = map_col(s.cm, 16 * kc + (j & 3) + 8 * (j >> 2) + 4 * hi);
-            x[h2] = col >= 0 ? v[col] * sc : 0.f;
-          }
-          unsigned p0, p1, p2;
-          split3_pair(x[0], x[1], p0, p1, p2);
-          q[i] = sp == 0 ? p0 : (sp == 1 ? p1 : p2);
-        }
-      }
-      out = __builtin_bit_cast(f32x4, u32x4{q[0], q[1], q[2], q[3]});
-    } else if (s.type == SEG_WBWD3) {
-      const int G = s.NT / 2, w = c >> 1, e = c & 1;
-      const int kc = w / (3 * G), g = (w / 3) % G, sp = w % 3;
-      const int col = map_col(s.cm, 32 * (2 * g + e) + i32);
-      unsigned q[4] = {0u, 0u, 0u, 0u};
+            x[h2] = col >= 0 ? T(i32, col) : 0.f;
+          }
+          split3_pair(x[0], x[1], q[0][i], q[1][i], q[2][i]);
+        }
+      }
+#pragma unroll
+      for (int sp = 0; sp < 3; ++sp) put(chunks, s.chunk0 + 2 * ((kc * G + g) * 3 + sp) + e, lane, as_f32x4(q[sp]));
+    }
+  } else if (s.type == SEG_WFWD3H || s.type == SEG_WFWD2H) {
+    const int PL = s.type == SEG_WFWD2H ? 2 : 3, g = t.b;
+    for (int u = wv; u < 2 * s.KC; u += 4) {
+      const int kc = u >> 1, e = u & 1;
+      const int rl = 16 * e + i16;
+      unsigned q[3][4] = {};
+      if (r0 + rl < s.nrows) {
+#pragma unroll
+        for (int i = 0; i < 4; ++i) {
+          float x[2];
+#pragma unroll
+          for (int h2 = 0; h2 < 2; ++h2) {
+            const int j = 2 * i + h2;
+            const int col = map_col(s.cm, 32 * kc + 16 * (j >> 2) + 4 * kg + (j & 3));
+            x[h2] = col >= 0 ? T(rl, col) : 0.f;
+          }
+          split3_pair(x[0], x[1], q[0][i], q[1][i], q[2][i]);
+        }
+      }
+#pragma unroll
+      for (int sp = 0; sp < 3; ++sp)
+        if (sp < PL) put(chunks, s.chunk0 + 2 * ((kc * G + g) * PL + sp) + e, lane, as_f32x4(q[sp]));
+    }
+  } else if (s.type == SEG_WBWD) {
+    for (int u = wv; u < 4 * s.NT; u += 4) {
+      const int kt = u >> 2, ncl = u & 3, nc = 4 * t.b + ncl;
+      if (nc >= s.KC) continue;
+      const int col = map_col(s.cm, 32 * kt + i32);
+      f32x4 out = {0.f, 0.f, 0.f, 0.f};
       if (col >= 0) {
 #pragma unroll
-        for (int i = 0; i < 4; ++i) {
-          float x[2];
-#pragma unroll
-          for (int h2 = 0; h2 < 2; ++h2) {
-            const int j = 2 * i + h2;
-            const int r = 16 * kc + (j & 3) + 8 * (j >> 2) + 4 * hi;
-            x[h2] = 0.f;
-            if (r < s.nrows) {
-              const int row = s.row_off + r;
-              x[h2] = params[s.off_v + (int64_t)row * s.cols + col] * scale[s.scale_off + row] * s.mult;
-            }
-          }
-          unsigned p0, p1, p2;
-          split3_pair(x[0], x[1], p0, p1, p2);
-          q[i] = sp == 0 ? p0 : (sp == 1 ? p1 : p2);
-        }
-      }
-      out = __builtin_bit_cast(f32x4, u32x4{q[0], q[1], q[2], q[3]});
-    } else if (s.type == SEG_BIAS_H) {
-      const int kg = lane >> 4;
-#pragma unroll
-      for (int t = 0; t < 4; ++t) {
-        const int r = 16 * c + 4 * kg + t;
-        out[t] = (r < s.nrows) ? params[s.off_bias + s.row_off + r] : 0.f;
-      }
-    } else if (s.type == SEG_WFWD3H || s.type == SEG_WBWD3H || s.type == SEG_WFWD2H) {
-      const int G = s.NT / 2, w = c >> 1, e = c & 1, PL = s.type == SEG_WFWD2H ? 2 : 3;
-      const int kc = w / (PL * G), g = (w / PL) % G, sp = w % PL;
-      const int i16 = lane & 15, kg = lane >> 4;
-      const int arow = 16 * (2 * g + e) + i16;
-      const bool fwd = s.type != SEG_WBWD3H;
-      const int acol = fwd ? -1 : map_col(s.cm, arow);
-      unsigned q[4] = {0u, 0u, 0u, 0u};
-      if (fwd ? (arow < s.nrows) : (acol >= 0)) {
-#pragma unroll
-        for (int i = 0; i < 4; ++i) {
-          float x[2];
-#pragma unroll
-          for (int h2 = 0; h2 < 2; ++h2) {
-            const int j = 2 * i + h2;
-            const int k = 32 * kc + 16 * (j >> 2) + 4 * kg + (j & 3);
-            x[h2] = 0.f;
-            if (fwd) {
-              const int row = s.row_off + arow, col = map_col(s.cm, k);
-              if (col >= 0) x[h2] = params[s.off_v + (int64_t)row * s.cols + col] * (scale[s.scale_off + row] * s.mult);
-            } else if (k < s.nrows) {
-              const int row = s.row_off + k;
-              x[h2] = params[s.off_v + (int64_t)row * s.cols + acol] * scale[s.scale_off + row] * s.mult;
-            }
-          }
-          unsigned p0, p1, p2;
-          split3_pair(x[0], x[1], p0, p1, p2);
-          q[i] = sp == 0 ? p0 : (sp == 1 ? p1 : p2);
-        }
-      }
-      out = __builtin_bit_cast(f32x4, u32x4{q[0], q[1], q[2], q[3]});
-    } else if (s.type == SEG_ROWVEC_H) {
-      const int rr = c / s.KC, nt = c % s.KC, kg = lane >> 4;
-      const int row = s.row_off + rr;
-      const float sc = scale[s.scale_off + row] * s.mult;
-#pragma unroll
-      for (int t = 0; t < 4; ++t) {
-        const int col = map_col(s.cm, 16 * nt + 4 * kg + t);
-        out[t] = col >= 0 ? params[s.off_v + (int64_t)row * s.cols + col] * sc : 0.f;
-      }
-    } else if (s.type == SEG_WBWD) {
-      const int kt = c / s.KC, nc = c % s.KC;
-      const int col = map_col(s.cm, 32 * kt + i32);
+        for (int e = 0; e < 4; ++e) out[e] = T(8 * ncl + 4 * hi + e, col);
+      }
+      put(chunks, s.chunk0 + kt * s.KC + nc, lane, out);
+    }
+  } else if (s.type == SEG_WBWD3) {
+    for (int u = wv; u < 2 * s.NT; u += 4) {
+      const int kcl = u / s.NT, tl = u % s.NT, g = tl >> 1, e = tl & 1, kc = 2 * t.b + kcl;
+      if (kc >= s.KC) continue;
+      const int col = map_col(s.cm, 32 * tl + i32);
+      unsigned q[3][4] = {};
       if (col >= 0) {
 #pragma unroll
-        for (int t = 0; t < 4; ++t) {
-          const int r = 8 * nc + 4 * hi + t;
-          if (r < s.nrows) {
-            const int row = s.row_off + r;
-            out[t] = params[s.off_v + (int64_t)row * s.cols + col] * scale[s.scale_off + row] * s.mult;
-          }
-        }
-      }
-    } else if (s.type == SEG_ROWVEC) {
-      const int rr = c / s.KC, kc = c % s.KC;
-      const int row = s.row_off + rr;
-      const float sc = scale[s.scale_off + row] * s.mult;
-#pragma unroll
-      for (int t = 0; t < 4; ++t) {
-        const int col = map_col(s.cm, 8 * kc + 4 * hi + t);
-        out[t] = col >= 0 ? params[s.off_v + (int64_t)row * s.cols + col] * sc : 0.f;
-      }
-    } else if (s.type == SEG_SCALAR) {
-#pragma unroll
-      for (int t = 0; t < 4; ++t) out[t] = (t < s.nrows) ? params[s.off_bias + s.row_off + t] : 0.f;
-    }
-  }
-  reinterpret_cast<f32x4*>(chunks)[chunk * 64 + lane] = out;
-}
-
-void fill_tab(RowTab& tab, const NetPlan& np) {
-  for (int l = 0; l < np.d.n_lin; ++l) {
-    const int e = tab.n++;
-    tab.rows[e] = np.d.out_dim[l]; tab.cols[e] = np.d.in_dim[l]; tab.scale_off[e] = np.scale_off[l];
-    tab.off_v[e] = np.d.off_v[l]; tab.off_g[e] = np.d.off_g[l];
+        for (int i = 0; i < 4; ++i) {
+          float x[2];
+#pragma unroll
+          for (int h2 = 0; h2 < 2; ++h2) {
+            const int j = 2 * i + h2;
+            x[h2] = T(16 * kcl + (j & 3) + 8 * (j >> 2) + 4 * hi, col);
+          }
+          split3_pair(x[0], x[1], q[0][i], q[1][i], q[2][i]);
+        }
+      }
+#pragma unroll
+      for (int sp = 0; sp < 3; ++sp) put(chunks, s.chunk0 + 2 * ((kc * G + g) * 3 + sp) + e, lane, as_f32x4(q[sp]));
+    }
+  } else {
+    const int kc = t.b;
+    for (int tl = wv; tl < s.NT; tl += 4) {
+      const int g = tl >> 1, e = tl & 1;
+      const int col = map_col(s.cm, 16 * tl + i16);
+      unsigned q[3][4] = {};
+      if (col >= 0) {
+#pragma unroll
+        for (int i = 0; i < 4; ++i) {
+          float x[2];
+#pragma unroll
+          for (int h2 = 0; h2 < 2; ++h2) {
+            const int j = 2 * i + h2;
+            x[h2] = T(16 * (j >> 2) + 4 * kg + (j & 3), col);
+          }
+          split3_pair(x[0], x[1], q[0][i], q[1][i], q[2][i]);
+        }
+      }
+#pragma unroll
+      for (int sp = 0; sp < 3; ++sp) put(chunks, s.chunk0 + 2 * ((kc * G + g) * 3 + sp) + e, lane, as_f32x4(q[sp]));
+    }
   }
 }
 
@@ -210,14 +260,8 @@
 
 extern "C" int i2sdf_pack_weights(const i2sdf_plan* p, const float* params, float* packed, void* stream) {
   if (!p || !params || !packed) return I2SDF_EINVAL;
-  if (!p->d_segs) return I2SDF_EHIP;
-  hipStream_t st = (hipStream_t)stream;
-  RowTab tab{};
-  fill_tab(tab, p->sdf); fill_tab(tab, p->rgb);
-  if (p->light.d.n_lin) fill_tab(tab, p->light);
-  rowscale_kernel<<<cdiv(p->n_scale, 4), 256, 0, st>>>(tab, params, packed, p->n_scale);
-  const int64_t threads = p->total_chunks * 64;
-  pack_kernel<<<(unsigned)((threads + 255) / 256), 256, 0, st>>>(p->d_segs, p->n_segs, params, packed, packed + p->scale_floats,
-                                                                 p->total_chunks);
+  if (!p->d_segs || !p->d_pack_tasks) return I2SDF_EHIP;
+  static_assert(PACK_TILE_MAX_COLS % 64 == 0, "a staged row is read in whole lane strides");
+  pack_kernel<<<(unsigned)p->pack_tasks.size(), 256, 0, (hipStream_t)stream>>>(p->d_pack_tasks, p->d_segs, params, packed, p->scale_floats);
   return i2sdf_hip_check(hipGetLastError(), "pack_weights launch");
 }
diff --git a/i2sdf_amd/csrc/plan.cpp b/i2sdf_amd/csrc/plan.cpp
--- a/i2sdf_amd/csrc/plan.cpp
+++ b/i2sdf_amd/csrc/plan.cpp
@@ -292,6 +292,56 @@
   }
 }
 
+int pack_tile_blocks(const Seg& s) {
+  if (s.cols > PACK_TILE_MAX_COLS) return 0;
+  const bool pairs = s.NT % 2 == 0;
+  switch (s.type) {
+    case SEG_WFWD: return s.used == s.NT * s.KC ? s.NT : 0;
+    case SEG_WFWD3: return pairs && s.used == s.NT * s.KC * 3 ? s.NT : 0;
+    case SEG_WFWD3H: return pairs && s.used == s.NT * s.KC * 3 ? s.NT / 2 : 0;
+    case SEG_WFWD2H: return pairs && s.used == s.NT * s.KC * 2 ? s.NT / 2 : 0;
+    case SEG_WBWD: return s.used == s.NT * s.KC ? cdiv(s.KC, 4) : 0;
+    case SEG_WBWD3: return pairs && s.used == s.NT * s.KC * 3 ? cdiv(s.KC, 2) : 0;
+    case SEG_WBWD3H: return pairs && s.used == s.NT * s.KC * 3 ? s.KC : 0;
+    default: return 0;
+  }
+}
+bool pack_weight_type(int32_t t) {
+  return t == SEG_WFWD || t == SEG_WFWD3 || t == SEG_WFWD3H || t == SEG_WFWD2H || t == SEG_WBWD || t == SEG_WBWD3 || t == SEG_WBWD3H;
+}
+
+int build_pack_tasks(i2sdf_plan* p) {
+  std::vector<PackTask> tiles, plain, scales;
+  std::vector<int64_t> off_g(p->n_scale, -1);
+  for (const NetPlan* np : {&p->sdf, &p->rgb, &p->light})
+    for (int l = 0; l < np->d.n_lin; ++l) {
+      off_g[np->scale_off[l]] = np->d.off_g[l];
+      for (int r = 0; r < np->d.out_dim[l]; r += PACK_SCALE_ROWS) {
+        const int n = np->d.out_dim[l] - r < PACK_SCALE_ROWS ? np->d.out_dim[l] - r : PACK_SCALE_ROWS;
+        scales.push_back(PackTask{PACK_SCALE, -1, r, n, np->d.in_dim[l], np->scale_off[l], np->d.off_v[l], np->d.off_g[l]});
+      }
+    }
+  if (p->scale_floats > p->n_scale) scales.push_back(PackTask{PACK_SCALE, -1, p->n_scale, (int32_t)(p->scale_floats - p->n_scale), 0, 0, 0, 0});
+  for (int i = 0; i < (int)p->segs.size(); ++i) {
+    const Seg& s = p->segs[i];
+    const int64_t g = s.type == SEG_ZERO ? 0 : off_g[s.scale_off];
+    int plain0 = 0;
+    if (pack_weight_type(s.type)) {
+      const int nb = pack_tile_blocks(s);
+      if (nb == 0) return i2sdf_refuse("i2sdf_plan_create: a weight segment of this shape has no row-block walk in the packing kernel");
+      for (int b = 0; b < nb; ++b) tiles.push_back(PackTask{PACK_TILE, i, b, 0, 0, 0, 0, g});
+      plain0 = s.used;
+    }
+    for (int c = plain0; c < s.nchunks; c += PACK_PLAIN_CHUNKS)
+      plain.push_back(PackTask{PACK_PLAIN, i, c, s.nchunks - c < PACK_PLAIN_CHUNKS ? s.nchunks - c : PACK_PLAIN_CHUNKS, 0, 0, 0, g});
+  }
+  std::vector<PackTask>& out = p->pack_tasks;
+  out = tiles;
+  out.insert(out.end(), plain.begin(), plain.end());
+  out.insert(out.end(), scales.begin(), scales.end());
+  return I2SDF_OK;
+}
+
 }
 
 extern "C" int i2sdf_plan_create(const i2sdf_net_desc* desc, i2sdf_plan** out) {
@@ -363,12 +413,16 @@
   { Seg z{}; z.type = SEG_ZERO; z.nchunks = SC > SCH ? SC : SCH; b.add(z); }
   p->total_chunks = b.chunk;
   p->n_segs = (int32_t)p->segs.size();
+  if (build_pack_tasks(p)) { delete p; return I2SDF_EINVAL; }
   hipError_t e = hipMalloc((void**)&p->d_segs, sizeof(Seg) * p->segs.size());
   if (e == hipSuccess) e = hipMemcpy(p->d_segs, p->segs.data(), sizeof(Seg) * p->segs.size(), hipMemcpyHostToDevice);
+  if (e == hipSuccess) e = hipMalloc((void**)&p->d_pack_tasks, sizeof(PackTask) * p->pack_tasks.size());
+  if (e == hipSuccess) e = hipMemcpy(p->d_pack_tasks, p->pack_tasks.data(), sizeof(PackTask) * p->pack_tasks.size(), hipMemcpyHostToDevice);
   if (e != hipSuccess) {
     (void)i2sdf_hip_check(e, "plan table upload");
     if (p->d_segs) (void)hipFree(p->d_segs);
-    p->d_segs = nullptr;
+    if (p->d_pack_tasks) (void)hipFree(p->d_pack_tasks);
+    p->d_segs = nullptr; p->d_pack_tasks = nullptr;
     (void)hipGetLastError();
   }
   {
@@ -387,6 +441,7 @@
 extern "C" void i2sdf_plan_destroy(i2sdf_plan* p) {
   if (!p) return;
   if (p->d_segs) (void)hipFree(p->d_segs);
+  if (p->d_pack_tasks) (void)hipFree(p->d_pack_tasks);
   if (p->ev_fork) (void)hipEventDestroy(p->ev_fork);
   if (p->ev_join) (void)hipEventDestroy(p->ev_join);
   if (p->side) (void)hipStreamDestroy(p->side);
diff --git a/i2sdf_amd/csrc/plan.h b/i2sdf_amd/csrc/plan.h
--- a/i2sdf_amd/csrc/plan.h
+++ b/i2sdf_amd/csrc/plan.h
@@ -27,6 +27,17 @@
   int32_t used;
   ColMap cm;
   float mult;
+};
+
+enum PackKind : int32_t { PACK_SCALE = 0, PACK_TILE = 1, PACK_PLAIN = 2 };
+constexpr int PACK_TILE_ROWS = 32;
+constexpr int PACK_TILE_MAX_COLS = 320;
+constexpr int PACK_PLAIN_CHUNKS = 4;
+constexpr int PACK_SCALE_ROWS = 16;
+struct PackTask {
+  int32_t kind, seg, b, n;
+  int32_t cols, scale_off;
+  int64_t off_v, off_g;
 };
 
 enum Mark : int {
@@ -86,6 +97,8 @@
   std::vector<i2sdf::Seg> segs;
   i2sdf::Seg* d_segs = nullptr;
   int32_t n_segs = 0;
+  std::vector<i2sdf::PackTask> pack_tasks;
+  i2sdf::PackTask* d_pack_tasks = nullptr;
   int32_t n_scale = 0;
   int64_t scale_floats = 0;
   int64_t total_chunks = 0;
diff --git a/i2sdf_amd/csrc/sampler.hip b/i2sdf_amd/csrc/sampler.hip
--- a/i2sdf_amd/csrc/sampler.hip
+++ b/i2sdf_amd/csrc/sampler.hip
@@ -519,11 +519,12 @@
 }
 
 
-extern "C" int i2sdf_sample_rays(const i2sdf_plan* p, const float* packed, const float* params, const i2sdf_sampler_cfg* sc,
-                                 const float* cam, const float* dirs, int64_t B, int32_t training, const float* t_lin, const float* u_more,
-                                 const float* u_final, int64_t ldu_final, const int32_t* extra_tab, const float* strat_u,
-                                 const int32_t* extra_idx, const int32_t* eik_idx, int32_t force_iters, float* workspace, float* z_out,
-                                 int64_t ldz, float* z_eik, int32_t* iters_out, void* stream) {
+extern "C" int i2sdf_sample_rays_after_pack(const i2sdf_plan* p, const float* packed, const float* params, const i2sdf_sampler_cfg* sc,
+                                            const float* cam, const float* dirs, int64_t B, int32_t training, const float* t_lin,
+                                            const float* u_more, const float* u_final, int64_t ldu_final, const int32_t* extra_tab,
+                                            const float* strat_u, const int32_t* extra_idx, const int32_t* eik_idx, int32_t force_iters,
+                                            float* workspace, float* z_out, int64_t ldz, float* z_eik, int32_t* iters_out, void* pack_event,
+                                            void* stream) {
   if (B == 0) return I2SDF_OK;
   if (!p || !packed || !params || !sc || !cam || !dirs || !t_lin || !u_more || !u_final || !workspace || !z_out || B < 0) return I2SDF_EINVAL;
   if (sc->N_samples_eval > NNEW || sc->N_samples > NNEW || sc->N_samples_eval * sc->max_total_iters > NMAX || sc->max_total_iters > 12)
@@ -547,6 +548,9 @@
   const unsigned grid = (unsigned)((B + 3) / 4);
   const i2sdf_exchange* gcomm = (training && p->exchange.allreduce && (p->dp_flags & I2SDF_DP_GLOBAL_SAMPLER) && force_iters <= 0) ? &p->exchange : nullptr;
   sampler_init_kernel<<<grid, 256, 0, st>>>(B, sc->N_samples_eval, t_lin, training ? strat_u : nullptr, near, far, sc->eps, zA, samples, beta, state);
+  if (pack_event) {
+    if (int rc = i2sdf_hip_check(hipStreamWaitEvent(st, (hipEvent_t)pack_event, 0), "sample_rays: wait for the pack event")) return rc;
+  }
   const int n_it = (force_iters > 0 && force_iters < sc->max_total_iters) ? force_iters : sc->max_total_iters;
   for (int it = 0; it < n_it; ++it) {
     const int n_new = sc->N_samples_eval;
@@ -586,3 +590,12 @@
                                              z_eik, iters_out);
   return i2sdf_hip_check(hipGetLastError(), "sample_rays launch");
 }
+
+extern "C" int i2sdf_sample_rays(const i2sdf_plan* p, const float* packed, const float* params, const i2sdf_sampler_cfg* sc,
+                                 const float* cam, const float* dirs, int64_t B, int32_t training, const float* t_lin, const float* u_more,
+                                 const float* u_final, int64_t ldu_final, const int32_t* extra_tab, const float* strat_u,
+                                 const int32_t* extra_idx, const int32_t* eik_idx, int32_t force_iters, float* workspace, float* z_out,
+                                 int64_t ldz, float* z_eik, int32_t* iters_out, void* stream) {
+  return i2sdf_sample_rays_after_pack(p, packed, params, sc, cam, dirs, B, training, t_lin, u_more, u_final, ldu_final, extra_tab, strat_u, extra_idx,
+                                      eik_idx, force_iters, workspace, z_out, ldz, z_eik, iters_out, nullptr, stream);
+}
diff --git a/i2sdf_amd/engine.py b/i2sdf_amd/engine.py
--- a/i2sdf_amd/engine.py
+++ b/i2sdf_amd/engine.py
@@ -88,6 +88,8 @@
                         "i2sdf_weight_grads", "i2sdf_sample_rays", "i2sdf_composite_forward", "i2sdf_composite_backward", "i2sdf_pack_weights",
                         "i2sdf_ray_setup", "i2sdf_light_forward", "i2sdf_light_backward"):
                 fn = _Timed(fn, name)
+            elif name == "i2sdf_sample_rays_after_pack":
+                fn = _Timed(fn, "i2sdf_sample_rays")
             setattr(self._timed_lib, name, fn)
         self._real_lib, self._lib = self._lib, self._timed_lib
 
@@ -137,6 +139,16 @@
                 cur.wait_event(ev)
                 readers[cur] = True
         return L.ptr(self.packed)
+
+    def _pack_event_to_wait(self):
+        ev = self._pack_event
+        if ev is None:
+            return None, lambda: None
+        cur = torch.cuda.current_stream(self.packed.device)
+        readers = self.__dict__.setdefault("_pack_readers", {})
+        if cur in readers:
+            return None, lambda: None
+        return C.c_void_p(ev.cuda_event), lambda: readers.__setitem__(cur, True)
 
     def set_sdf_forward_bf16x3(self, on: bool):
         L.check(self._lib.i2sdf_plan_set_option(self._plan, L.OPT_SDF_FWD_BF16X3, int(bool(on))), "i2sdf_plan_set_option")
@@ -507,11 +519,16 @@
             u_final, ldu = self.u_final, 0
         ex, ek = i32(extra_idx), i32(eik_idx)
         su = None if strat_u is None else strat_u.contiguous()
-        L.check(self._lib.i2sdf_sample_rays(self._plan, self._pk(), L.ptr(flat_params), C.byref(self._scfg), L.ptr(cam.contiguous()),
-                                             L.ptr(dirs.contiguous()), B, 1 if training else 0, L.ptr(self.t_lin), L.ptr(self.u_more),
-                                             L.ptr(u_final), ldu, L.ptr(self.extra_tab), L.ptr(su), L.ptr(ex), L.ptr(ek), force_iters,
-                                             L.ptr(ws), L.ptr(z_out), self.n_z, L.ptr(z_eik), L.ptr(iters), L.stream_ptr()),
-                 "i2sdf_sample_rays")
+        pack_ev, waited = self._pack_event_to_wait() if B > 0 else (None, lambda: None)
+        if pack_ev is None:
+            self._pk()
+        L.check(self._lib.i2sdf_sample_rays_after_pack(self._plan, L.ptr(self.packed), L.ptr(flat_params), C.byref(self._scfg),
+                                                        L.ptr(cam.contiguous()), L.ptr(dirs.contiguous()), B, 1 if training else 0,
+                                                        L.ptr(self.t_lin), L.ptr(self.u_more), L.ptr(u_final), ldu, L.ptr(self.extra_tab),
+                                                        L.ptr(su), L.ptr(ex), L.ptr(ek), force_iters, L.ptr(ws), L.ptr(z_out), self.n_z,
+                                                        L.ptr(z_eik), L.ptr(iters), pack_ev, L.stream_ptr()),
+                 "i2sdf_sample_rays_after_pack")
+        waited()
         self._last_sampler_ws = ws
         return z_out, z_eik, iters
 
diff --git a/i2sdf_amd/lib.py b/i2sdf_amd/lib.py
--- a/i2sdf_amd/lib.py
+++ b/i2sdf_amd/lib.py
@@ -142,6 +142,8 @@
     "i2sdf_sampler_workspace_floats": (_I64, [_I64]),
     "i2sdf_sample_rays": (C.c_int, [_P, _P, _P, C.POINTER(SamplerCfg), _P, _P, _I64, _I32, _P, _P, _P, _I64, _P, _P, _P, _P, _I32, _P, _P,
                                     _I64, _P, _P, _P]),
+    "i2sdf_sample_rays_after_pack": (C.c_int, [_P, _P, _P, C.POINTER(SamplerCfg), _P, _P, _I64, _I32, _P, _P, _P, _I64, _P, _P, _P, _P, _I32, _P,
+                                               _P, _I64, _P, _P, _P, _P]),
     "i2sdf_render_image_workspace_floats": (_I64, [_P, C.POINTER(SamplerCfg), _I64]),
     "i2sdf_render_image": (C.c_int, [_P, _P, _P, C.POINTER(SamplerCfg), _P, _P, _I32, _P, _I64, _I64] + [_P] * 13),
     "i2sdf_sdf_grid_workspace_floats": (_I64, [_I64]),
diff --git a/include/i2sdf.h b/include/i2sdf.h
--- a/include/i2sdf.h
+++ b/include/i2sdf.h
@@ -226,6 +226,11 @@
                       const float* u_final, int64_t ldu_final, const int32_t* extra_tab, const float* strat_u,
                       const int32_t* extra_idx, const int32_t* eik_idx, int32_t force_iters, float* workspace, float* z_out,
                       int64_t ldz, float* z_eik, int32_t* iters_out, void* stream);
+int i2sdf_sample_rays_after_pack(const i2sdf_plan* plan, const float* packed, const float* params, const i2sdf_sampler_cfg* cfg,
+                                 const float* cam, const float* dirs, int64_t B, int32_t training, const float* t_lin, const float* u_more,
+                                 const float* u_final, int64_t ldu_final, const int32_t* extra_tab, const float* strat_u,
+                                 const int32_t* extra_idx, const int32_t* eik_idx, int32_t force_iters, float* workspace, float* z_out,
+                                 int64_t ldz, float* z_eik, int32_t* iters_out, void* pack_event, void* stream);
 
 
 int i2sdf_light_forward(const i2sdf_plan* plan, const float* packed, const float* feat, int64_t M, int64_t Mp, float* lm, float* hl,
```
